# LanceZPF/loongx

Measured on AMD Instinct MI355X. Metric: edited images/s @512x512, 28-step Flux denoise, higher is better.
Workload: dtype bf16

## Files before the change

### include/lx.h

```cpp
#ifndef LX_H_
#define LX_H_
#include <stddef.h>
#include <stdint.h>
#ifdef __cplusplus
extern "C" {
#endif

#define LX_VERSION 404

typedef enum lx_status {
  LX_OK = 0,
  LX_ERR_INVALID = -1,
  LX_ERR_UNSUPPORTED = -2,
  LX_ERR_LAUNCH = -3,
  LX_ERR_NO_DEVICE = -4
} lx_status;

int lx_version(void);
const char* lx_last_error(void);
int lx_device_arch(char* name, size_t n);

enum {
  LX_EPI_STORE_BF16 = 0,
  LX_EPI_STORE_F32 = 1,
  LX_EPI_RESID_F32 = 2,
  LX_EPI_GELU = 0x100,
  LX_W_TILED = 0x200,
  LX_EPI_SPLIT_BF16 = 0x400,
  LX_EPI_STORE_FP8 = 3,
  LX_EPI_QKV = 0x1000,
  LX_OPERANDS_FP8 = 0x800,
  LX_OPERANDS_F16 = 0x2000
};

typedef struct lx_gemm_desc {
  const void* A;
  const void* W;
  const float* bias;
  void* C;
  const float* gate;
  const float* lora_t;
  const float* lora_up;
  int32_t M, N, K;
  int32_t lda, ldw, ldc;
  int32_t rows_per_batch, gate_ld;
  int32_t lora_r, lora_ldt, lora_mod_cols, lora_toff_max;
  int32_t epilogue;
  int32_t gelu_col_start;
  int32_t lora_nsplit;
  int32_t lora_split_stride;
  int32_t k_segs, a_lo_off;
  int32_t c_lo_off;
  float out_scale;
  union {
    const float* col_scale;
    int32_t* f16_ovf;
  };
  const float* qkv_norm_q;
  const float* qkv_norm_k;
  const float* qkv_rope;
  void* qkv_vt;
  void* qkv_k;
  int32_t qkv_d, qkv_vt_ld, qkv_vt_pos0;
  int32_t qkv_k_ld;
  void* qkv_q8;
  void* qkv_k8;
  void* qkv_vt8;
  int32_t qkv_ld8;
  float qkv_q_scale, qkv_k_scale, qkv_v_scale;
} lx_gemm_desc;

#define LX_GEMM_MAX_GROUP 4
int lx_gemm_bf16(const lx_gemm_desc* problems, int n, void* stream);
void lx_gemm_reload_env(void);

size_t lx_gemm_workspace_bytes(void);
int lx_gemm_bf16_ws(const lx_gemm_desc* problems, int n, void* workspace, size_t ws_bytes, void* stream);
int lx_gemm_workspace_status(void* workspace, void* stream);
enum { LX_GEMM_PLAN_NONE = 0, LX_GEMM_PLAN_8WAVE_256 = 1, LX_GEMM_PLAN_8WAVE_128 = 2, LX_GEMM_PLAN_MIXED = 3, LX_GEMM_PLAN_MIXED_2L = 4,
       LX_GEMM_PLAN_G4 = 5, LX_GEMM_PLAN_G4_SPLIT2 = 6, LX_GEMM_PLAN_G4_SPLIT3 = 7 };
int lx_gemm_last_plan(void);

int lx_lora_down(const void* X, int ldx, const void* Adown, float* T, int ldt, int M, int K, int R, int n_split,
                 int split_stride, void* stream);
int lx_lora_down_f16(const void* X, int ldx, const void* Adown, float* T, int ldt, int M, int K, int R, int n_split,
                     int split_stride, void* stream);
int lx_lora_down_terms(const void* const* X, const int* ldx, const void* const* Adown, int n_terms, float* T, int ldt, int M, int K, int R,
                       int slab_stride, void* stream);

int lx_linear_skinny(const float* X, int ldx, const void* W, int ldw, const float* bias, float* Y, int ldy,
                     int M, int N, int K, int act_in, int act_out, int accumulate, void* stream);

int lx_timestep_embed(const float* t, float* out, int B, int dim, void* stream);

int lx_rope_table(const float* ids, int L, int a0, int a1, int a2, double theta, float* cos_t, float* sin_t, void* stream);

int lx_ln_modulate(const float* X, int ldx, const float* shift, const float* scale, int mod_ld, void* Y, int ldy,
                   int M, int D, int rows_per_batch, float eps, void* stream);
typedef struct lx_ln_seg { int32_t row0, n_rows, rows_per_batch, _pad; const float* shift; const float* scale; } lx_ln_seg;
int lx_ln_modulate_segs(const float* X, int ldx, const lx_ln_seg* seg, int n_seg, int mod_ld, void* Y, int ldy, int D,
                        float eps, void* stream);
int lx_ln_modulate_f16_segs(const float* X, int ldx, const lx_ln_seg* seg, int n_seg, int mod_ld, void* Y, int ldy, int D,
                            float eps, int32_t* f16_ovf, void* stream);
int lx_ln_modulate_lora_segs(const float* X, int ldx, const lx_ln_seg* seg, int n_seg, int mod_ld, void* Y, int ldy, int D,
                             float eps, const void* Adown, int R, float* T, int ldt, int lora_row0, int lora_rows, void* stream);
int lx_ln_modulate_lora_f16_segs(const float* X, int ldx, const lx_ln_seg* seg, int n_seg, int mod_ld, void* Y, int ldy, int D,
                                 float eps, const void* Adown, int R, float* T, int ldt, int lora_row0, int lora_rows,
                                 int32_t* f16_ovf, void* stream);

int lx_qkv_prep(void* QKV, int ld, int q_col, int k_col, int v_col, int row0, int n_rows, int rows_per_batch,
                int H, const float* wq, const float* wk, float eps, const float* cos_tab, const float* sin_tab,
                void* VT, int vt_ld, int vt_pos0, void* stream);

typedef struct lx_qkv_seg {
  int32_t row0, rows_per_batch, vt_pos0, _pad;
  const float* wq; const float* wk; const float* cos_tab; const float* sin_tab;
} lx_qkv_seg;
int lx_qkv_prep_segs(void* QKV, int ld, int q_col, int k_col, int v_col, const lx_qkv_seg* seg, int n_seg, int n_batches,
                     int H, float eps, void* VT, int vt_ld, void* stream);
int lx_qkv_prep_f16in_segs(void* QKV, int ld, int q_col, int k_col, int v_col, const lx_qkv_seg* seg, int n_seg, int n_batches,
                           int H, float eps, void* VT, int vt_ld, void* stream);

typedef struct lx_attn_desc {
  const void* Q; const void* K; const void* VT; void* O;
  int32_t ldq, ldk, ldo, vt_ld;
  int32_t q_col, k_col, o_col;
  int32_t B, H;
  int32_t n_seg;
  int32_t seg_row0[3], seg_len[3], seg_vt0[3];
  float bias[3][3];
  float scale;
  int32_t n_qseg;
  int32_t flags;
  int32_t qseg_mask;
  int32_t* f16_ovf;
} lx_attn_desc;
enum { LX_ATTN_Q_LOG2 = 1, LX_ATTN_BOUNDED = 2, LX_ATTN_INVARIANT = 4, LX_ATTN_O_F16 = 8, LX_ATTN_PREFER_4WAVE = 16, LX_ATTN_P_EXP2 = 32 };
int lx_attn_fwd(const lx_attn_desc* d, void* stream);
enum { LX_ATTN_KERNEL_NONE = 0, LX_ATTN_KERNEL_8WAVE = 1, LX_ATTN_KERNEL_4WAVE = 2 };
int lx_attn_last_kernel(void);

enum { LX_ATTN_MASK_BOOL = 0, LX_ATTN_MASK_F32 = 1, LX_ATTN_MASK_BF16 = 2, LX_ATTN_MASK_F16 = 3 };
typedef struct lx_attn_mask_desc {
  const void* mask;
  int32_t dtype;
  int32_t dims[4];
  int32_t _pad;
  int64_t strides[4];
  void* workspace;
  size_t workspace_bytes;
} lx_attn_mask_desc;
int lx_attn_mask_workspace(const lx_attn_desc* d, const lx_attn_mask_desc* m, size_t* bytes);
int lx_attn_mask_prep(const lx_attn_desc* d, const lx_attn_mask_desc* m, void* stream);
int lx_attn_fwd_masked(const lx_attn_desc* d, const lx_attn_mask_desc* m, void* stream);

int lx_qkv_prep_fp8_segs(const void* QKV, int ld, int q_col, int k_col, int v_col, const lx_qkv_seg* seg, int n_seg,
                         int n_batches, int H, float eps, void* Q8, void* K8, int ld8, void* VT8, int vt8_ld,
                         float q_scale, float k_scale, float v_scale, void* stream);
int lx_qkv_prep_fp8_f16in_segs(const void* QKV, int ld, int q_col, int k_col, int v_col, const lx_qkv_seg* seg, int n_seg,
                               int n_batches, int H, float eps, void* Q8, void* K8, int ld8, void* VT8, int vt8_ld,
                               float q_scale, float k_scale, float v_scale, void* stream);
int lx_attn_fwd_fp8(const lx_attn_desc* d, float qk_descale, float v_descale, void* stream);

int lx_split_bf16(const float* src, int lds, void* dst, int ldd, int lo_off, int M, int K, void* stream);
int lx_ln_modulate_split_segs(const float* X, int ldx, const lx_ln_seg* seg, int n_seg, int mod_ld, void* Y, int ldy, int y_lo_off,
                              int D, float eps, void* stream);
int lx_qkv_prep_f32_segs(float* QKV, int ld, int q_col, int k_col, const lx_qkv_seg* seg, int n_seg, int n_batches, int H, float eps,
                         void* stream);
typedef struct lx_attn_f32_desc {
  const float* QKV; int32_t ld, q_col, k_col, v_col;
  void* O; int32_t ldo, o_col, o_lo_off;
  int32_t B, H, n_seg;
  int32_t seg_row0[3], seg_len[3];
  float bias[3][3];
  float scale;
} lx_attn_f32_desc;
int lx_attn_fwd_f32(const lx_attn_f32_desc* d, void* stream);

int lx_qkv_prep_split_segs(const float* QKV, int ld, int q_col, int k_col, int v_col, const lx_qkv_seg* seg, int n_seg, int n_batches, int H,
                           float eps, void* QK2, int ld2, int q2_col, int k2_col, int lo_off, void* VT2, int vt_ld, long long vt_lo_off,
                           void* stream);
int lx_attn_fwd_split(const lx_attn_desc* d, int qk_lo_off, long long vt_lo_off, int o_lo_off, void* stream);

int lx_ln_modulate_fp8_segs(const float* X, int ldx, const lx_ln_seg* seg, int n_seg, int mod_ld, void* Y, int ldy, void* Y8, int ldy8,
                            float y8_scale, int D, float eps, void* stream);
int lx_convert_fp8(const void* src, int src_is_bf16, int lds, void* dst, int ldd, float scale, int M, int K, void* stream);
int lx_lora_down_fp8(const void* X8, int ldx, float x_descale, const void* Adown, float* T, int ldt, int M, int K, int R, int n_split,
                     int split_stride, void* stream);

int lx_euler_step(float* x, const void* v, int v_is_bf16, float dsigma, size_t n, void* stream);
int lx_convert(void* dst, int dst_bf16, const void* src, int src_bf16, size_t n, void* stream);

int lx_s4_scan(const float* u, const double* lam, const double* w, const float* Dskip, float* y,
               int B, int H, int L, int N, void* stream);
int lx_s4_conv(const float* u, const float* Kker, const float* Dskip, float* y, int B, int H, int L, void* stream);
int lx_chanmix(const float* x, const float* W, const float* bias, const float* resid, const float* ln_g,
               const float* ln_b, float* y, int B, int Hin, int Hout, int L, int act, void* stream);
int lx_pyramid_pool(const float* x, float* y, int B, int C, int L, const int* sizes, int n_sizes, int ldy, int y_col0,
                    void* stream);
int lx_layernorm_relu(float* x, const float* g, const float* b, int M, int D, float eps, void* stream);
int lx_linear_f32(const float* X, int ldx, int x_trans, const float* W, int ldw, const float* bias, float* Y, int ldy,
                  int y_trans, int M, int N, int K, int accumulate, void* stream);

int lx_chan_gemm_f32(const float* X, long x_bstride, int ldx, const float* W, int ldw, const float* bias, float* Y, long y_bstride,
                     int ldy, int B, int N, int K, int L, int epilogue, float* part, void* stream);

size_t lx_duan_workspace_bytes(int B, int C, int L, int Hd);
int lx_duan_fwd(const float* x, const float* c, const float* gw1, const float* gb1, const float* gw2, const float* gb2,
                const float* mw1, const float* mb1, const float* mw2, const float* mb2, float* y,
                int B, int C, int L, int Hd, float eps, int keep_k, void* ws, size_t ws_bytes, void* stream);

size_t lx_groupnorm_workspace_bytes(int B, int P, int G);
int lx_groupnorm_silu(const void* x, int x_is_bf16, int B, int P, int C, int G, const float* gamma, const float* beta, float eps,
                      int silu, void* y, void* ws, size_t ws_bytes, void* stream);
int lx_im2col3x3(const void* x, int B, int H, int W, int C, int mode, void* out, int Kpad, void* stream);
int lx_softmax_rows(const float* S, int lds, float scale, void* P, int ldp, int M, int N, void* stream);

#ifdef __cplusplus
}
#endif
#endif
```

### loongx_amd/_lib.py

```python
from __future__ import annotations

import ctypes as C
import os

import torch

_HERE = os.path.dirname(os.path.abspath(__file__))
LIB_PATH = os.environ.get("LX_AMD_LIB", os.path.join(_HERE, "lib", "liblx_amd.so"))

LX_EPI_STORE_BF16, LX_EPI_STORE_F32, LX_EPI_RESID_F32, LX_EPI_GELU, LX_W_TILED, LX_EPI_SPLIT_BF16 = 0, 1, 2, 0x100, 0x200, 0x400
LX_EPI_STORE_FP8, LX_OPERANDS_FP8, LX_EPI_QKV, LX_OPERANDS_F16 = 3, 0x800, 0x1000, 0x2000
LX_GEMM_MAX_GROUP = 4
(LX_GEMM_PLAN_NONE, LX_GEMM_PLAN_8WAVE_256, LX_GEMM_PLAN_8WAVE_128, LX_GEMM_PLAN_MIXED, LX_GEMM_PLAN_MIXED_2L, LX_GEMM_PLAN_G4,
 LX_GEMM_PLAN_G4_SPLIT2, LX_GEMM_PLAN_G4_SPLIT3) = range(8)


class GemmDesc(C.Structure):
    _fields_ = [("A", C.c_void_p), ("W", C.c_void_p), ("bias", C.c_void_p), ("C", C.c_void_p),
                ("gate", C.c_void_p), ("lora_t", C.c_void_p), ("lora_up", C.c_void_p),
                ("M", C.c_int32), ("N", C.c_int32), ("K", C.c_int32),
                ("lda", C.c_int32), ("ldw", C.c_int32), ("ldc", C.c_int32),
                ("rows_per_batch", C.c_int32), ("gate_ld", C.c_int32),
                ("lora_r", C.c_int32), ("lora_ldt", C.c_int32), ("lora_mod_cols", C.c_int32),
                ("lora_toff_max", C.c_int32), ("epilogue", C.c_int32), ("gelu_col_start", C.c_int32),
                ("lora_nsplit", C.c_int32), ("lora_split_stride", C.c_int32),
                ("k_segs", C.c_int32), ("a_lo_off", C.c_int32), ("c_lo_off", C.c_int32), ("out_scale", C.c_float),
                ("col_scale", C.c_void_p),
                ("qkv_norm_q", C.c_void_p), ("qkv_norm_k", C.c_void_p), ("qkv_rope", C.c_void_p), ("qkv_vt", C.c_void_p),
                ("qkv_k", C.c_void_p),
                ("qkv_d", C.c_int32), ("qkv_vt_ld", C.c_int32), ("qkv_vt_pos0", C.c_int32), ("qkv_k_ld", C.c_int32),
                ("qkv_q8", C.c_void_p), ("qkv_k8", C.c_void_p), ("qkv_vt8", C.c_void_p),
                ("qkv_ld8", C.c_int32), ("qkv_q_scale", C.c_float), ("qkv_k_scale", C.c_float), ("qkv_v_scale", C.c_float)]


class AttnDesc(C.Structure):
    _fields_ = [("Q", C.c_void_p), ("K", C.c_void_p), ("VT", C.c_void_p), ("O", C.c_void_p),
                ("ldq", C.c_int32), ("ldk", C.c_int32), ("ldo", C.c_int32), ("vt_ld", C.c_int32),
                ("q_col", C.c_int32), ("k_col", C.c_int32), ("o_col", C.c_int32),
                ("B", C.c_int32), ("H", C.c_int32), ("n_seg", C.c_int32),
                ("seg_row0", C.c_int32 * 3), ("seg_len", C.c_int32 * 3), ("seg_vt0", C.c_int32 * 3),
                ("bias", (C.c_float * 3) * 3), ("scale", C.c_float), ("n_qseg", C.c_int32), ("flags", C.c_int32),
                ("qseg_mask", C.c_int32), ("f16_ovf", C.c_void_p)]


LX_ATTN_Q_LOG2, LX_ATTN_BOUNDED, LX_ATTN_INVARIANT, LX_ATTN_O_F16, LX_ATTN_PREFER_4WAVE, LX_ATTN_P_EXP2 = 1, 2, 4, 8, 16, 32
LX_ATTN_MASK_BOOL, LX_ATTN_MASK_F32, LX_ATTN_MASK_BF16, LX_ATTN_MASK_F16 = 0, 1, 2, 3


class AttnMaskDesc(C.Structure):
    _fields_ = [("mask", C.c_void_p), ("dtype", C.c_int32), ("dims", C.c_int32 * 4), ("_pad", C.c_int32),
                ("strides", C.c_int64 * 4), ("workspace", C.c_void_p), ("workspace_bytes", C.c_size_t)]


class AttnF32Desc(C.Structure):
    _fields_ = [("QKV", C.c_void_p), ("ld", C.c_int32), ("q_col", C.c_int32), ("k_col", C.c_int32), ("v_col", C.c_int32),
                ("O", C.c_void_p), ("ldo", C.c_int32), ("o_col", C.c_int32), ("o_lo_off", C.c_int32),
                ("B", C.c_int32), ("H", C.c_int32), ("n_seg", C.c_int32),
                ("seg_row0", C.c_int32 * 3), ("seg_len", C.c_int32 * 3),
                ("bias", (C.c_float * 3) * 3), ("scale", C.c_float)]


class LnSeg(C.Structure):
    _fields_ = [("row0", C.c_int32), ("n_rows", C.c_int32), ("rows_per_batch", C.c_int32), ("_pad", C.c_int32),
                ("shift", C.c_void_p), ("scale", C.c_void_p)]


class QkvSeg(C.Structure):
    _fields_ = [("row0", C.c_int32), ("rows_per_batch", C.c_int32), ("vt_pos0", C.c_int32), ("_pad", C.c_int32),
                ("wq", C.c_void_p), ("wk", C.c_void_p), ("cos_tab", C.c_void_p), ("sin_tab", C.c_void_p)]


_P, _I, _F, _Z = C.c_void_p, C.c_int, C.c_float, C.c_size_t
_SIGS = {
    "lx_version": (C.c_int, []),
    "lx_last_error": (C.c_char_p, []),
    "lx_device_arch": (C.c_int, [C.c_char_p, _Z]),
    "lx_gemm_bf16": (C.c_int, [C.POINTER(GemmDesc), _I, _P]),
    "lx_gemm_reload_env": (None, []),
    "lx_gemm_workspace_bytes": (_Z, []),
    "lx_gemm_bf16_ws": (C.c_int, [C.POINTER(GemmDesc), _I, _P, _Z, _P]),
    "lx_gemm_workspace_status": (C.c_int, [_P, _P]),
    "lx_gemm_last_plan": (C.c_int, []),
    "lx_lora_down": (C.c_int, [_P, _I, _P, _P, _I, _I, _I, _I, _I, _I, _P]),
    "lx_lora_down_f16": (C.c_int, [_P, _I, _P, _P, _I, _I, _I, _I, _I, _I, _P]),
    "lx_lora_down_terms": (C.c_int, [C.POINTER(C.c_void_p), C.POINTER(C.c_int), C.POINTER(C.c_void_p), _I, _P, _I, _I, _I, _I, _I, _P]),
    "lx_linear_skinny": (C.c_int, [_P, _I, _P, _I, _P, _P, _I, _I, _I, _I, _I, _I, _I, _P]),
    "lx_timestep_embed": (C.c_int, [_P, _P, _I, _I, _P]),
    "lx_rope_table": (C.c_int, [_P, _I, _I, _I, _I, C.c_double, _P, _P, _P]),
    "lx_ln_modulate": (C.c_int, [_P, _I, _P, _P, _I, _P, _I, _I, _I, _I, _F, _P]),
    "lx_ln_modulate_segs": (C.c_int, [_P, _I, C.POINTER(LnSeg), _I, _I, _P, _I, _I, _F, _P]),
    "lx_ln_modulate_f16_segs": (C.c_int, [_P, _I, C.POINTER(LnSeg), _I, _I, _P, _I, _I, _F, _P, _P]),
    "lx_ln_modulate_lora_segs": (C.c_int, [_P, _I, C.POINTER(LnSeg), _I, _I, _P, _I, _I, _F, _P, _I, _P, _I, _I, _I, _P]),
    "lx_ln_modulate_lora_f16_segs": (C.c_int, [_P, _I, C.POINTER(LnSeg), _I, _I, _P, _I, _I, _F, _P, _I, _P, _I, _I, _I, _P, _P]),
    "lx_qkv_prep_segs": (C.c_int, [_P, _I, _I, _I, _I, C.POINTER(QkvSeg), _I, _I, _I, _F, _P, _I, _P]),
    "lx_qkv_prep_f16in_segs": (C.c_int, [_P, _I, _I, _I, _I, C.POINTER(QkvSeg), _I, _I, _I, _F, _P, _I, _P]),
    "lx_qkv_prep": (C.c_int, [_P, _I, _I, _I, _I, _I, _I, _I, _I, _P, _P, _F, _P, _P, _P, _I, _I, _P]),
    "lx_attn_fwd": (C.c_int, [C.POINTER(AttnDesc), _P]),
    "lx_attn_last_kernel": (C.c_int, []),
    "lx_attn_mask_workspace": (C.c_int, [C.POINTER(AttnDesc), C.POINTER(AttnMaskDesc), C.POINTER(C.c_size_t)]),
    "lx_attn_mask_prep": (C.c_int, [C.POINTER(AttnDesc), C.POINTER(AttnMaskDesc), _P]),
    "lx_attn_fwd_masked": (C.c_int, [C.POINTER(AttnDesc), C.POINTER(AttnMaskDesc), _P]),
    "lx_qkv_prep_fp8_segs": (C.c_int, [_P, _I, _I, _I, _I, C.POINTER(QkvSeg), _I, _I, _I, _F, _P, _P, _I, _P, _I, _F, _F, _F, _P]),
    "lx_qkv_prep_fp8_f16in_segs": (C.c_int, [_P, _I, _I, _I, _I, C.POINTER(QkvSeg), _I, _I, _I, _F, _P, _P, _I, _P, _I, _F, _F, _F, _P]),
    "lx_attn_fwd_fp8": (C.c_int, [C.POINTER(AttnDesc), _F, _F, _P]),
    "lx_split_bf16": (C.c_int, [_P, _I, _P, _I, _I, _I, _I, _P]),
    "lx_ln_modulate_split_segs": (C.c_int, [_P, _I, C.POINTER(LnSeg), _I, _I, _P, _I, _I, _I, _F, _P]),
    "lx_qkv_prep_f32_segs": (C.c_int, [_P, _I, _I, _I, C.POINTER(QkvSeg), _I, _I, _I, _F, _P]),
    "lx_attn_fwd_f32": (C.c_int, [C.POINTER(AttnF32Desc), _P]),
    "lx_qkv_prep_split_segs": (C.c_int, [_P, _I, _I, _I, _I, C.POINTER(QkvSeg), _I, _I, _I, _F, _P, _I, _I, _I, _I, _P, _I, C.c_longlong, _P]),
    "lx_attn_fwd_split": (C.c_int, [C.POINTER(AttnDesc), _I, C.c_longlong, _I, _P]),
    "lx_groupnorm_workspace_bytes": (_Z, [_I, _I, _I]),
    "lx_groupnorm_silu": (C.c_int, [_P, _I, _I, _I, _I, _I, _P, _P, _F, _I, _P, _P, _Z, _P]),
    "lx_im2col3x3": (C.c_int, [_P, _I, _I, _I, _I, _I, _P, _I, _P]),
    "lx_softmax_rows": (C.c_int, [_P, _I, _F, _P, _I, _I, _I, _P]),
    "lx_ln_modulate_fp8_segs": (C.c_int, [_P, _I, C.POINTER(LnSeg), _I, _I, _P, _I, _P, _I, _F, _I, _F, _P]),
    "lx_convert_fp8": (C.c_int, [_P, _I, _I, _P, _I, _F, _I, _I, _P]),
    "lx_lora_down_fp8": (C.c_int, [_P, _I, _F, _P, _P, _I, _I, _I, _I, _I, _I, _P]),
    "lx_euler_step": (C.c_int, [_P, _P, _I, _F, _Z, _P]),
    "lx_convert": (C.c_int, [_P, _I, _P, _I, _Z, _P]),
    "lx_s4_scan": (C.c_int, [_P, _P, _P, _P, _P, _I, _I, _I, _I, _P]),
    "lx_s4_conv": (C.c_int, [_P, _P, _P, _P, _I, _I, _I, _P]),
    "lx_chanmix": (C.c_int, [_P, _P, _P, _P, _P, _P, _P, _I, _I, _I, _I, _I, _P]),
    "lx_pyramid_pool": (C.c_int, [_P, _P, _I, _I, _I, C.POINTER(C.c_int), _I, _I, _I, _P]),
    "lx_layernorm_relu": (C.c_int, [_P, _P, _P, _I, _I, _F, _P]),
    "lx_linear_f32": (C.c_int, [_P, _I, _I, _P, _I, _P, _P, _I, _I, _I, _I, _I, _I, _P]),
    "lx_chan_gemm_f32": (C.c_int, [_P, C.c_long, _I, _P, _I, _P, _P, C.c_long, _I, _I, _I, _I, _I, _I, _P, _P]),
    "lx_duan_workspace_bytes": (_Z, [_I, _I, _I, _I]),
    "lx_duan_fwd": (C.c_int, [_P] * 11 + [_I, _I, _I, _I, _F, _I, _P, _Z, _P]),
}

EXPORTS = tuple(_SIGS)


class LxError(RuntimeError):
    pass


def _load():
    if not os.path.exists(LIB_PATH):
        raise ImportError(f"liblx_amd.so not found at {LIB_PATH}: build it with `python -c 'import __graft_entry__ as g; "
                          f"g.build()'` or loongx_amd/csrc/build.sh -- there is no CPU/torch fallback for the hot path")
    lib = C.CDLL(LIB_PATH)
    for name, (res, args) in _SIGS.items():
        fn = getattr(lib, name)
        fn.restype, fn.argtypes = res, args
    return lib


lib = _load()


def check(status: int, what: str = "") -> None:
    if status != 0:
        raise LxError(f"{what or 'lx call'} failed ({status}): {lib.lx_last_error().decode()}")
```

### loongx_amd/csrc/gemm.hip

```cpp
#include "gemm8.h"


static double round_us(int bm, int K) { return bm == 256 ? 15.0 + 1.81 * (K / 64) : 10.5 + 1.06 * (K / 64); }

struct GemmEnv { int bm, g4, sk, g4_fault; };
static int env_int(const char* name, int dflt) {
  const char* s = getenv(name);
  return s ? atoi(s) : dflt;
}
static GemmEnv read_gemm_env() { return GemmEnv{env_int("LX_GEMM_BM", 0), env_int("LX_GEMM4", 1), env_int("LX_GEMM4_SK", 1), env_int("LX_GEMM4_FAULT", 0)}; }
static GemmEnv g_gemm_env = read_gemm_env();
static const GemmEnv& gemm_env() { return g_gemm_env; }
extern "C" void lx_gemm_reload_env(void) { g_gemm_env = read_gemm_env(); }

namespace {
constexpr size_t SK_FLAGS_OFF = (size_t)256 * SK_SLOT_FLOATS * sizeof(float);
constexpr size_t SK_WS_BYTES = SK_FLAGS_OFF + (256 + 64) * sizeof(int);
static_assert(SK_WS_BYTES % 256 == 0, "workspace size keeps the 256-byte alignment contract");
constexpr int SK_MIN_KT_ALL = 96;
constexpr int SK_MAX_ROUNDS = 16;

int device_cus() {
  static int n = -1;
  if (n < 0) {
    int dev = 0;
    hipDeviceProp_t pr;
    n = (hipGetDevice(&dev) == hipSuccess && hipGetDeviceProperties(&pr, dev) == hipSuccess) ? pr.multiProcessorCount : 0;
  }
  return n;
}
}

static long tiles_of(const lx_gemm_desc& p, int bm) { return (long)((p.M + bm - 1) / bm) * ((p.N + BN - 1) / BN); }

static lx_gemm_desc sub_rows(const lx_gemm_desc& p, int r0, int rows) {
  lx_gemm_desc q = p;
  q.A = (const uint16_t*)p.A + (size_t)r0 * p.lda;
  const int epi = p.epilogue & 0xff;
  q.C = epi == LX_EPI_STORE_BF16 ? (void*)((uint16_t*)p.C + (size_t)r0 * p.ldc) : (void*)((float*)p.C + (size_t)r0 * p.ldc);
  if (p.lora_t) q.lora_t = p.lora_t + (size_t)r0 * p.lora_ldt;
  if (p.qkv_k) q.qkv_k = (uint16_t*)p.qkv_k + (size_t)r0 * p.qkv_k_ld;
  if (p.qkv_q8) {
    q.qkv_q8 = (uint8_t*)p.qkv_q8 + (size_t)r0 * p.qkv_ld8;
    q.qkv_k8 = (uint8_t*)p.qkv_k8 + (size_t)r0 * p.qkv_ld8;
  }
  q.M = rows;
  return q;
}

static int launch_plan(const GemmArgs& a, int bm, hipStream_t s, int variant = LX_GV_BF16) {
  if (a.n == 0) return LX_OK;
  if (variant == LX_GV_SPLIT) lx_gemm8_launch_split(bm, a, s);
  else if (variant == LX_GV_F16) lx_gemm8_launch_f16(bm, a, s);
  else if (variant == LX_GV_FP8) lx_gemm8_launch_fp8(bm, a, s);
  else lx_gemm8_launch_bf16(bm, a, s);
  LX_LAUNCH_CHECK("lx_gemm_bf16");
  return LX_OK;
}

void lx_gemm8_launch_bf16(int bm, const GemmArgs& a, hipStream_t s) {
  const int t = a.tile_start[a.n];
  if (bm == 256) hipLaunchKernelGGL((lx_gemm_kernel<256, false>), dim3(t), dim3(NTHREADS), 0, s, a);
  else hipLaunchKernelGGL((lx_gemm_kernel<128, false>), dim3(t), dim3(NTHREADS), 0, s, a);
}
void lx_gemm8_mixed_launch_bf16(const GemmArgs& big, const GemmArgs& tail, int n_big_pad, hipStream_t s) {
  hipLaunchKernelGGL(lx_gemm_mixed_kernel<false>, dim3(n_big_pad + tail.tile_start[tail.n]), dim3(NTHREADS), 0, s, big, tail, n_big_pad);
}

static void plan_add(GemmArgs& a, const lx_gemm_desc& p, int m_base, int bm) {
  a.p[a.n] = p;
  a.m_base[a.n] = m_base;
  a.tile_start[a.n + 1] = a.tile_start[a.n] + (int)tiles_of(p, bm);
  ++a.n;
  for (int i = a.n + 1; i <= MAX_SUB; ++i) a.tile_start[i] = a.tile_start[a.n];
}

static thread_local int lx_gemm_last = LX_GEMM_PLAN_NONE;
extern "C" int lx_gemm_last_plan(void) { return lx_gemm_last; }
static int planned(int rc, int plan) {
  if (rc == LX_OK) lx_gemm_last = plan;
  return rc;
}

extern "C" size_t lx_gemm_workspace_bytes(void) { return SK_WS_BYTES; }

extern "C" int lx_gemm_workspace_status(void* workspace, void* stream) {
  LX_CHECK_ARG(workspace, "lx_gemm_workspace_status: NULL workspace");
  int* err = (int*)((char*)workspace + SK_FLAGS_OFF) + 256;
  int v = 0;
  hipStream_t s = (hipStream_t)stream;
  if (hipMemcpyAsync(&v, err, sizeof(int), hipMemcpyDeviceToHost, s) != hipSuccess || hipStreamSynchronize(s) != hipSuccess) {
    lx_set_error("lx_gemm_workspace_status: reading the error word failed: %s", hipGetErrorString(hipGetLastError()));
    return LX_ERR_LAUNCH;
  }
  if (v == 0) return LX_OK;
  (void)hipMemsetAsync((char*)workspace + SK_FLAGS_OFF, 0, (256 + 64) * sizeof(int), s);
  (void)hipStreamSynchronize(s);
  lx_set_error("lx_gemm_bf16_ws: a split-K pair workgroup timed out waiting for its partner (CUs held by other work?); the results "
               "of that launch are invalid. Re-run with the workspace omitted (lx_gemm_bf16) or LX_GEMM4_SK=0");
  return LX_ERR_LAUNCH;
}

extern "C" int lx_gemm_bf16(const lx_gemm_desc* problems, int n, void* stream) { return lx_gemm_bf16_ws(problems, n, nullptr, 0, stream); }

extern "C" int lx_gemm_bf16_ws(const lx_gemm_desc* problems, int n, void* workspace, size_t ws_bytes, void* stream) {
  LX_CHECK_ARG(problems && n >= 1 && n <= LX_GEMM_MAX_GROUP, "lx_gemm_bf16: n=%d out of range [1,%d]", n, LX_GEMM_MAX_GROUP);
  long t256 = 0, t128 = 0;
  int kmax = 0;
  bool split = false, fp8 = false, f16 = false, qkv = false;
  for (int i = 0; i < n; ++i) fp8 = fp8 || (problems[i].epilogue & LX_OPERANDS_FP8) != 0;
  for (int i = 0; i < n; ++i) f16 = f16 || (problems[i].epilogue & LX_OPERANDS_F16) != 0;
  for (int i = 0; i < n; ++i) {
    const lx_gemm_desc& p = problems[i];
    if (f16) {
      LX_CHECK_ARG((p.epilogue & LX_OPERANDS_F16) != 0 && !(p.epilogue & LX_OPERANDS_FP8) && p.k_segs <= 1 && !(p.epilogue & LX_EPI_SPLIT_BF16),
                   "lx_gemm_bf16[%d]: LX_OPERANDS_F16 must be set on every problem of a launch and excludes the e4m3 and split-bf16 modes", i);
      if (p.f16_ovf) LX_CHECK_ARG(((uintptr_t)p.f16_ovf & 3) == 0, "lx_gemm_bf16[%d]: f16_ovf must be 4-byte aligned", i);
    }
    if (fp8) {
      LX_CHECK_ARG((p.epilogue & LX_OPERANDS_FP8) != 0 && p.k_segs <= 1 && !(p.epilogue & LX_EPI_SPLIT_BF16), "lx_gemm_bf16[%d]: LX_OPERANDS_FP8 must be set on every problem of a launch and excludes the split-bf16 mode", i);
      LX_CHECK_ARG(p.K % 128 == 0 && p.lda % 16 == 0 && p.ldw % 16 == 0, "lx_gemm_bf16[%d]: fp8 operands need K %% 128 == 0 and lda / ldw %% 16 == 0 (K=%d)", i, p.K);
      if (p.col_scale) LX_CHECK_ARG(((uintptr_t)p.col_scale & 15) == 0, "lx_gemm_bf16[%d]: col_scale must be 16-byte aligned", i);
      if (p.lora_t) LX_CHECK_ARG(p.lora_r <= 4 && p.lora_nsplit <= 4, "lx_gemm_bf16[%d]: the fp8 path applies LoRA in the tile prologue only (rank <= 4, <= 4 slabs)", i);
      if ((p.epilogue & 0xff) == LX_EPI_STORE_FP8) LX_CHECK_ARG(p.out_scale > 0.f && p.ldc % 8 == 0, "lx_gemm_bf16[%d]: LX_EPI_STORE_FP8 needs out_scale > 0 and ldc %% 8 == 0", i);
    }
    LX_CHECK_ARG(p.k_segs >= 0 && p.k_segs <= 3, "lx_gemm_bf16[%d]: k_segs=%d must be 0..3", i, p.k_segs);
    const int segs = p.k_segs > 1 ? p.k_segs : 1;
    if (segs > 1 || (p.epilogue & LX_EPI_SPLIT_BF16)) split = true;
    if (segs > 1) LX_CHECK_ARG(p.a_lo_off >= p.K && p.a_lo_off % 8 == 0 && p.lda >= p.a_lo_off + p.K, "lx_gemm_bf16[%d]: a_lo_off=%d needs K <= a_lo_off, a_lo_off + K <= lda, multiple of 8", i, p.a_lo_off);
    if (segs == 3) LX_CHECK_ARG(p.ldw >= 2 * p.K, "lx_gemm_bf16[%d]: k_segs = 3 reads W as [N, 2K] = [W_hi | W_lo]: ldw=%d < 2K", i, p.ldw);
    if (p.epilogue & LX_EPI_SPLIT_BF16) LX_CHECK_ARG((p.epilogue & 0xff) == LX_EPI_STORE_BF16 && p.c_lo_off >= p.N && p.c_lo_off % 8 == 0 && p.ldc >= p.c_lo_off + p.N,
                                                     "lx_gemm_bf16[%d]: LX_EPI_SPLIT_BF16 needs a bf16 store and N <= c_lo_off, c_lo_off + N <= ldc, multiple of 8", i);
    LX_CHECK_ARG(p.A && p.W && p.C, "lx_gemm_bf16[%d]: NULL operand", i);
    LX_CHECK_ARG(p.M > 0 && p.N > 0 && p.K > 0, "lx_gemm_bf16[%d]: bad shape M=%d N=%d K=%d", i, p.M, p.N, p.K);
    LX_CHECK_ARG(p.K % BK == 0, "lx_gemm_bf16[%d]: K=%d must be a multiple of %d", i, p.K, BK);
    LX_CHECK_ARG(p.N % 8 == 0, "lx_gemm_bf16[%d]: N=%d must be a multiple of 8", i, p.N);
    LX_CHECK_ARG(p.lda % 8 == 0 && p.ldw % 8 == 0 && p.lda >= p.K && p.ldw >= p.K, "lx_gemm_bf16[%d]: lda/ldw must be >= K and multiples of 8", i);
    LX_CHECK_ARG(((uintptr_t)p.A & 15) == 0 && ((uintptr_t)p.W & 15) == 0 && ((uintptr_t)p.C & 15) == 0, "lx_gemm_bf16[%d]: operands must be 16-byte aligned", i);
    LX_CHECK_ARG(p.ldc % 8 == 0 && p.ldc >= p.N, "lx_gemm_bf16[%d]: ldc=%d must be >= N and a multiple of 8", i, p.ldc);
    const int epi = p.epilogue & 0xff;
    LX_CHECK_ARG(epi >= LX_EPI_STORE_BF16 && (epi <= LX_EPI_RESID_F32 || (fp8 && epi == LX_EPI_STORE_FP8)), "lx_gemm_bf16[%d]: unknown epilogue %d", i, p.epilogue);
    LX_CHECK_ARG(p.rows_per_batch > 0, "lx_gemm_bf16[%d]: rows_per_batch must be > 0", i);
    if (p.epilogue & LX_W_TILED) LX_CHECK_ARG(p.N % BN == 0 && p.ldw == (segs == 3 ? 2 * p.K : p.K), "lx_gemm_bf16[%d]: LX_W_TILED needs N %% 256 == 0 and ldw == K (2K with k_segs = 3)", i);
    if (p.gate) LX_CHECK_ARG(p.gate_ld >= p.N && p.gate_ld % 4 == 0, "lx_gemm_bf16[%d]: gate_ld=%d", i, p.gate_ld);
    if (p.lora_t) {
      LX_CHECK_ARG(p.lora_up && p.lora_r >= 1 && p.lora_r <= 16, "lx_gemm_bf16[%d]: LoRA needs lora_up and 1 <= r <= 16", i);
      LX_CHECK_ARG(p.lora_mod_cols <= 0 || p.lora_mod_cols % BN == 0, "lx_gemm_bf16[%d]: lora_mod_cols must be a multiple of %d", i, BN);
    }
    if (p.epilogue & LX_EPI_QKV) {
      LX_CHECK_ARG(!fp8 && segs == 1 && !(p.epilogue & LX_EPI_SPLIT_BF16) && epi == LX_EPI_STORE_BF16, "lx_gemm_bf16[%d]: LX_EPI_QKV goes with plain bf16 operands and LX_EPI_STORE_BF16", i);
      LX_CHECK_ARG(p.qkv_d > 0 && p.qkv_d % BN == 0 && (p.N >= 3 * p.qkv_d || p.N % BN == 0), "lx_gemm_bf16[%d]: LX_EPI_QKV needs qkv_d %% 256 == 0 and whole projection tiles (qkv_d=%d N=%d)", i, p.qkv_d, p.N);
      LX_CHECK_ARG(p.rows_per_batch % 32 == 0 && p.M % 32 == 0, "lx_gemm_bf16[%d]: LX_EPI_QKV needs rows_per_batch %% 32 == 0 and M %% 32 == 0 (%d, %d)", i, p.rows_per_batch, p.M);
      const bool q8 = p.qkv_q8 != nullptr;
      LX_CHECK_ARG(p.qkv_norm_q && p.qkv_norm_k && (p.qkv_vt || q8) && p.qkv_rope && ((uintptr_t)p.qkv_norm_q & 15) == 0 && ((uintptr_t)p.qkv_norm_k & 15) == 0 && ((uintptr_t)p.qkv_vt & 15) == 0 &&
                   ((uintptr_t)p.qkv_rope & 15) == 0, "lx_gemm_bf16[%d]: LX_EPI_QKV needs 16-byte aligned qkv_norm_q / qkv_norm_k / qkv_rope / qkv_vt", i);
      if (q8) {
        LX_CHECK_ARG(p.qkv_k8 && p.qkv_vt8 && (((uintptr_t)p.qkv_q8 | (uintptr_t)p.qkv_k8 | (uintptr_t)p.qkv_vt8) & 15) == 0 && p.qkv_ld8 % 16 == 0 && p.qkv_ld8 >= p.qkv_d,
                     "lx_gemm_bf16[%d]: LX_EPI_QKV e4m3 outputs need 16-byte aligned qkv_q8 / qkv_k8 / qkv_vt8 and qkv_ld8 %% 16 == 0, >= qkv_d", i);
        LX_CHECK_ARG(p.qkv_q_scale > 0.f && p.qkv_k_scale > 0.f && p.qkv_v_scale > 0.f && !p.qkv_k, "lx_gemm_bf16[%d]: LX_EPI_QKV e4m3 outputs need positive scales and no separate bf16 key image", i);
      }
      LX_CHECK_ARG(p.qkv_vt_ld > 0 && p.qkv_vt_ld % 64 == 0 && p.qkv_vt_pos0 >= 0 && p.qkv_vt_pos0 % 64 == 0 && p.qkv_vt_pos0 + p.rows_per_batch <= p.qkv_vt_ld,
                   "lx_gemm_bf16[%d]: qkv_vt_ld / qkv_vt_pos0 must be multiples of 64 with the stream inside a V^T row", i);
      if (p.qkv_k) LX_CHECK_ARG(((uintptr_t)p.qkv_k & 15) == 0 && p.qkv_k_ld % 8 == 0 && p.qkv_k_ld >= p.qkv_d, "lx_gemm_bf16[%d]: qkv_k must be 16-byte aligned with qkv_k_ld %% 8 == 0, >= qkv_d", i);
      qkv = true;
    }
    if (p.bias) LX_CHECK_ARG(((uintptr_t)p.bias & 15) == 0, "lx_gemm_bf16[%d]: bias must be 16-byte aligned", i);
    t256 += tiles_of(p, 256);
    t128 += tiles_of(p, 128);
    kmax = p.K * segs > kmax ? p.K * segs : kmax;
  }
  hipStream_t s = (hipStream_t)stream;
  if (fp8) {
    const int ncu = device_cus() > 0 ? device_cus() : 256;
    const double ca = (double)((t256 + ncu - 1) / ncu) * round_us(256, kmax / 4), cb = (double)((t128 + ncu - 1) / ncu) * round_us(128, kmax / 4);
    const int bm = gemm_env().bm ? gemm_env().bm : (cb < ca ? 128 : 256);
    GemmArgs all;
    all.n = 0;
    all.tile_start[0] = 0;
    for (int i = 1; i <= MAX_SUB; ++i) all.tile_start[i] = 0;
    for (int i = 0; i < n; ++i) plan_add(all, problems[i], 0, bm);
    return planned(launch_plan(all, bm, s, LX_GV_FP8), bm == 256 ? LX_GEMM_PLAN_8WAVE_256 : LX_GEMM_PLAN_8WAVE_128);
  }
  const int NCU = device_cus() > 0 ? device_cus() : 256;
  const GemmEnv& env = gemm_env();
  const int forced = env.bm;
  if (env.g4 && forced == 0 && (workspace || env.g4 == 2)) {
    bool ok = true;
    for (int i = 0; i < n; ++i) {
      const lx_gemm_desc& p = problems[i];
      ok = ok && (p.epilogue & 0xff) <= LX_EPI_RESID_F32 && p.K / BK >= 2 && !((p.epilogue & LX_EPI_QKV) && p.qkv_q8);
      if (p.lora_t)
        ok = ok && p.lora_r <= 8 && p.lora_r % 2 == 0 && p.lora_nsplit >= 1 && p.lora_nsplit <= 4 && p.lora_ldt % 2 == 0 && p.lora_split_stride % 2 == 0 &&
             ((((uintptr_t)p.lora_t) | ((uintptr_t)p.lora_up)) & 7) == 0;
    }
    const long rounds = (t256 + NCU - 1) / NCU;
    bool fills = env.g4 == 2 || (t256 >= NCU && (rounds * NCU - t256 <= NCU / 4 || rounds >= 8));
    bool uniform_k4 = true;
    for (int i = 1; i < n; ++i) uniform_k4 = uniform_k4 && problems[i].K == problems[0].K;
    const long tail = t256 % NCU, full = t256 - tail;
    for (int i = 1; i < n; ++i) uniform_k4 = uniform_k4 && problems[i].k_segs == problems[0].k_segs;
    const int kt_all = kmax / BK;
    const bool can_split = env.sk && workspace && ws_bytes >= SK_WS_BYTES && ((uintptr_t)workspace & 255) == 0 && uniform_k4 && kt_all >= 16 &&
                           tail > 0 && tail * 2 <= 256 && tail * 2 <= NCU && rounds <= SK_MAX_ROUNDS;
    bool split_all = can_split && full == 0 && kt_all >= SK_MIN_KT_ALL;
    const int tail_div = !qkv && kt_all >= 96 ? 2 : 3;
    bool split_tail = can_split && full > 0 && tail * tail_div <= NCU;
    int np = 2;
    if (!split && env.sk != 2 && kt_all >= 24 && tail * 3 <= 256 && tail * 3 <= NCU && (split_all || split_tail) && (kt_all >= 96 || tail * 6 <= NCU)) np = 3;
    if (split) {
      const double r4 = 8.9 + 1.31 * kt_all;
      const bool sk_tail = can_split && tail > 0;
      const double c4 = (double)(full / NCU) * r4 + (tail == 0 ? 0.0 : sk_tail ? 8.9 + 1.31 * (kt_all - kt_all / 2) + 6.0 : r4);
      const double c8a = (double)((t256 + NCU - 1) / NCU) * (5.8 + 1.55 * kt_all), c8b = (double)((t128 + NCU - 1) / NCU) * (10.5 + 1.06 * kt_all);
      fills = env.g4 == 2 || c4 < (c8a < c8b ? c8a : c8b);
      split_all = fills && sk_tail && full == 0;
      split_tail = fills && sk_tail && full > 0;
      if (!fills) split_all = split_tail = false;
    }
    if (ok && (fills || split_all || split_tail)) {
      GemmArgs all;
      all.n = 0;
      all.tile_start[0] = 0;
      for (int i = 1; i <= MAX_SUB; ++i) all.tile_start[i] = 0;
      for (int i = 0; i < n; ++i) plan_add(all, problems[i], 0, 256);
      float* slots = nullptr;
      int *flags = nullptr, *err = nullptr;
      unsigned grid = (unsigned)t256;
      int sk_full = (int)t256, sk_parts = 1;
      if (split_all || split_tail) {
        slots = (float*)workspace;
        flags = (int*)((char*)workspace + SK_FLAGS_OFF);
        err = flags + 256;
        grid = (unsigned)(full + np * tail);
        sk_full = (int)full;
        sk_parts = env.g4_fault ? 3 : 2;
      }
      if (split) lx_gemm4_launch_split(all, grid, sk_full, sk_parts, slots, flags, err, s);
      else if (f16) lx_gemm4_launch_f16(all, grid, sk_full, sk_parts, slots, flags, err, s, np);
      else lx_gemm4_launch_bf16(all, grid, sk_full, sk_parts, slots, flags, err, s, np);
      LX_LAUNCH_CHECK("lx_gemm_bf16");
      return planned(LX_OK, !(split_all || split_tail) ? LX_GEMM_PLAN_G4 : np == 3 ? LX_GEMM_PLAN_G4_SPLIT3 : LX_GEMM_PLAN_G4_SPLIT2);
    }
  }
  if (split) {
    const double ca = (double)((t256 + NCU - 1) / NCU) * round_us(256, kmax), cb = (double)((t128 + NCU - 1) / NCU) * round_us(128, kmax);
    const int bm = forced ? forced : (cb < ca ? 128 : 256);
    GemmArgs all;
    all.n = 0;
    all.tile_start[0] = 0;
    for (int i = 1; i <= MAX_SUB; ++i) all.tile_start[i] = 0;
    for (int i = 0; i < n; ++i) plan_add(all, problems[i], 0, bm);
    return planned(launch_plan(all, bm, s, LX_GV_SPLIT), bm == 256 ? LX_GEMM_PLAN_8WAVE_256 : LX_GEMM_PLAN_8WAVE_128);
  }
  if (workspace) LX_CHECK_ARG(ws_bytes >= SK_WS_BYTES && ((uintptr_t)workspace & 255) == 0, "lx_gemm_bf16_ws: workspace needs %zu bytes (lx_gemm_workspace_bytes()), 256-byte aligned", SK_WS_BYTES);
  const int variant = f16 ? LX_GV_F16 : LX_GV_BF16;
  const double c_a = (double)((t256 + NCU - 1) / NCU) * round_us(256, kmax);
  const double c_b = (double)((t128 + NCU - 1) / NCU) * round_us(128, kmax);
  GemmArgs big, tail;
  big.n = tail.n = 0;
  big.tile_start[0] = tail.tile_start[0] = 0;
  for (int i = 1; i <= MAX_SUB; ++i) big.tile_start[i] = tail.tile_start[i] = 0;
  double c_c = 1e30;
  const long full = (t256 / NCU) * NCU;
  if (forced == 0 && full > 0 && t256 > full) {
    long remain = t256;
    int keep_rows[LX_GEMM_MAX_GROUP];
    for (int i = 0; i < n; ++i) keep_rows[i] = problems[i].M;
    for (int i = n - 1; i >= 0 && remain > full; --i) {
      const int tn = (problems[i].N + BN - 1) / BN;
      while (remain > full && keep_rows[i] > 0) {
        const int last_rows = keep_rows[i] % 256 ? keep_rows[i] % 256 : 256;
        keep_rows[i] -= last_rows;
        remain -= tn;
      }
    }
    long tail_tiles = 0;
    for (int i = 0; i < n; ++i) {
      if (keep_rows[i] > 0) plan_add(big, sub_rows(problems[i], 0, keep_rows[i]), 0, 256);
      if (keep_rows[i] < problems[i].M) {
        const lx_gemm_desc q = sub_rows(problems[i], keep_rows[i], problems[i].M - keep_rows[i]);
        plan_add(tail, q, keep_rows[i], 128);
        tail_tiles += tiles_of(q, 128);
      }
    }
    c_c = (double)((remain + NCU - 1) / NCU) * round_us(256, kmax) + (double)((tail_tiles + NCU - 1) / NCU) * round_us(128, kmax) + 2.0;
  }
  int choice = forced == 256 ? 0 : forced == 128 ? 1 : (c_c < c_a && c_c < c_b) ? 2 : (c_b < c_a ? 1 : 0);
  if (choice == 2) {
    if (big.n > 0 && tail.n > 0) {
      const int n_big = big.tile_start[big.n], n_big_pad = (n_big + 7) & ~7;
      if (f16) lx_gemm8_mixed_launch_f16(big, tail, n_big_pad, s);
      else lx_gemm8_mixed_launch_bf16(big, tail, n_big_pad, s);
      LX_LAUNCH_CHECK("lx_gemm_bf16");
      return planned(LX_OK, LX_GEMM_PLAN_MIXED);
    }
    const int rc = launch_plan(big, 256, s, variant);
    if (rc != LX_OK) return rc;
    return planned(launch_plan(tail, 128, s, variant), LX_GEMM_PLAN_MIXED_2L);
  }
  GemmArgs all;
  all.n = 0;
  all.tile_start[0] = 0;
  for (int i = 1; i <= MAX_SUB; ++i) all.tile_start[i] = 0;
  for (int i = 0; i < n; ++i) plan_add(all, problems[i], 0, choice == 0 ? 256 : 128);
  return planned(launch_plan(all, choice == 0 ? 256 : 128, s, variant), choice == 0 ? LX_GEMM_PLAN_8WAVE_256 : LX_GEMM_PLAN_8WAVE_128);
}
```

### loongx_amd/csrc/gemm4.h

```cpp
#pragma once
#include "gemm_common.h"

namespace {

constexpr int G4_STAGE = 256 * BK * 2 + BN * BK * 2;
constexpr int G4_LDS = 2 * G4_STAGE;
constexpr int G4_PLD = 132;
static_assert(G4_LDS <= 160 * 1024 && 4 * 2 * 16 * G4_PLD * 4 <= G4_LDS, "LDS budget / epilogue patches");

#ifdef LX_G4_PROBE
__device__ unsigned long long lx_g4_probe_buf[8192 * 8];
#define G4_STAMP(k) if (threadIdx.x == 0 && blockIdx.x < 8192) { asm volatile("s_waitcnt lgkmcnt(0)" ::: "memory"); lx_g4_probe_buf[blockIdx.x * 8 + (k)] = __builtin_amdgcn_s_memtime(); }
#else
#define G4_STAMP(k)
#endif


template <bool SPLIT, bool F16 = false, int NP = 2>
__global__ __launch_bounds__(G4_THREADS) void lx_gemm4_kernel(const GemmArgs args, const int sk_full, const int sk_parts, float* __restrict__ sk_slots,
                                                              int* __restrict__ sk_flags, int* __restrict__ sk_err) {
#if defined(__HIP_DEVICE_COMPILE__)
  __shared__ __attribute__((aligned(1024))) char smem[G4_LDS];
  constexpr int BM = 256, A_BYTES = BM * BK * 2;
  const int pid = blockIdx.x;
  G4_STAMP(0)
  const int total = args.tile_start[MAX_SUB];
  int lid, part = 0;
  if (pid < sk_full) {
    const int q = sk_full >> 3, r = sk_full & 7;
    const int xcd = pid & 7, inx = pid >> 3;
    lid = (xcd < r ? xcd * (q + 1) : r * (q + 1) + (xcd - r) * q) + inx;
  } else {
    const int r = pid - sk_full;
    lid = sk_full + r / NP;
    part = r % NP;
  }
  (void)total;
  const bool split_tile = pid >= sk_full && sk_parts >= 2;
  const int g = tile_group(args, lid);
  lx_gemm_desc P = args.p[g];
  int tm, tn;
  tile_coords<BM>(P, lid - args.tile_start[g], tm, tn);
  const int tid = threadIdx.x, lane = tid & 63;
  const int wave = __builtin_amdgcn_readfirstlane(tid >> 6);
  const int wm = wave >> 1, wn = wave & 1, l15 = lane & 15, lq = lane >> 4;
  int m0 = tm * BM, n0 = tn * BN;
  int M = P.M, N = P.N;
  const int K = P.K;
  const bool w_tiled = (P.epilogue & LX_W_TILED) != 0;
  const int nk1 = K / BK;
  const int nkt = SPLIT ? nk1 * max(P.k_segs, 1) : nk1;
  const int kt_begin = !split_tile ? 0 : NP == 2 ? (part ? nkt >> 1 : 0) : (part * nkt) / NP;
  const int kt_end = !split_tile ? nkt : NP == 2 ? (part ? nkt : nkt >> 1) : ((part + 1) * nkt) / NP;

  uint32_t aoff[8], woff[8];
  {
    const int rsub = lane >> 3, pslot = lane & 7;
#pragma unroll
    for (int j = 0; j < 8; ++j) {
      const int row = (j * 4 + wave) * 8 + rsub;
      const int lslot = pslot ^ ((row >> 1) & 7);
      aoff[j] = (uint32_t)((min(m0 + row, M - 1) - m0) * P.lda + lslot * 8) * 2u;
      woff[j] = w_tiled ? (uint32_t)((j * 4 + wave) * 512 + lane * 8) * 2u : (uint32_t)((min(n0 + row, N - 1) - n0) * P.ldw + lslot * 8) * 2u;
    }
  }
  const __bf16* a_org = (const __bf16*)P.A + (size_t)m0 * P.lda;
  const int kw_tiles = SPLIT && P.k_segs == 3 ? 2 * nk1 : nk1;
  const __bf16* w_org = w_tiled ? (const __bf16*)P.W + ((size_t)tn * kw_tiles) * (BN * BK) : (const __bf16*)P.W + (size_t)n0 * P.ldw;
  const lx_rsrc_t rs_a = lx_make_rsrc(a_org), rs_w = lx_make_rsrc(w_org);
  const int w_kstride_b = (w_tiled ? BN * BK : BK) * 2;
  const int a_lo_b = SPLIT ? P.a_lo_off * 2 : 0;
  auto a_soff = [&](int t) -> int {
    if constexpr (!SPLIT) return t * (BK * 2);
    else {
      const int seg = t >= 2 * nk1 ? 2 : (t >= nk1 ? 1 : 0);
      return (t - seg * nk1) * (BK * 2) + (seg == 1 ? a_lo_b : 0);
    }
  };
  auto w_soff = [&](int t) -> int {
    if constexpr (!SPLIT) return t * w_kstride_b;
    else {
      const int seg = t >= 2 * nk1 ? 2 : (t >= nk1 ? 1 : 0);
      return (t - seg * nk1 + (seg == 2 ? nk1 : 0)) * w_kstride_b;
    }
  };
  auto piece = [&](int p_, int a_so, int w_so, int stage) {
    if (p_ < 8) lx_buf_to_lds(rs_a, (lptr_t)(smem + stage * G4_STAGE + (p_ * 4 + wave) * 1024), aoff[p_], a_so);
    else lx_buf_to_lds(rs_w, (lptr_t)(smem + stage * G4_STAGE + A_BYTES + ((p_ - 8) * 4 + wave) * 1024), woff[p_ - 8], w_so);
  };
  int a_ad[2], w_ad[2];
  {
    const int ar = wm * 128 + l15, wr = wn * 128 + l15;
#pragma unroll
    for (int ks = 0; ks < 2; ++ks) {
      a_ad[ks] = ar * 128 + (((ks * 4 + lq) ^ ((ar >> 1) & 7)) * 16);
      w_ad[ks] = A_BYTES + wr * 128 + (((ks * 4 + lq) ^ ((wr >> 1) & 7)) * 16);
    }
  }
  f32x4 acc[8][8];
#pragma unroll
  for (int i = 0; i < 8; ++i)
#pragma unroll
    for (int j = 0; j < 8; ++j) acc[i][j] = f32x4{0.f, 0.f, 0.f, 0.f};
  bf16x8 af[2][8], wf[2][8];
  auto rd = [&](int stage, int ks, int idx) {
    const char* base = smem + stage * G4_STAGE;
    if (idx < 8) wf[ks][idx] = *(const bf16x8*)(base + w_ad[ks] + idx * 2048);
    else af[ks][idx - 8] = *(const bf16x8*)(base + a_ad[ks] + (idx - 8) * 2048);
  };
  auto mm = [&](int ks, int n_) {
    const int j = n_ >> 3, i = n_ & 7;
    if constexpr (F16) asm volatile("v_mfma_f32_16x16x32_f16 %0, %1, %2, %0" : "+a"(acc[i][j]) : "v"(wf[ks][j]), "v"(af[ks][i]));
    else asm volatile("v_mfma_f32_16x16x32_bf16 %0, %1, %2, %0" : "+a"(acc[i][j]) : "v"(wf[ks][j]), "v"(af[ks][i]));
  };
#define G4_SB() __builtin_amdgcn_sched_barrier(0)
  const bool has_lora = P.lora_t != nullptr && kt_begin == 0;
  u32x2 lu[8], lt[8][4];
  if (has_lora) {
    const int R = P.lora_r, nsplit = P.lora_nsplit;
    const int toff = R * min(n0 / max(P.lora_mod_cols, 1), P.lora_toff_max);
    const int rk = min(2 * lq, R - 2);
#pragma unroll
    for (int j = 0; j < 8; ++j) lu[j] = *(const u32x2*)(P.lora_up + (size_t)min(n0 + wn * 128 + j * 16 + l15, N - 1) * R + rk);
#pragma unroll
    for (int i = 0; i < 8; ++i) {
      const float* tp = P.lora_t + (size_t)min(m0 + wm * 128 + i * 16 + l15, M - 1) * P.lora_ldt + toff + rk;
#pragma unroll
      for (int q = 0; q < 4; ++q) lt[i][q] = *(const u32x2*)(tp + (size_t)min(q, nsplit - 1) * P.lora_split_stride);
    }
  }
  {
    const int t1 = min(kt_begin + 1, kt_end - 1);
    const int a0 = a_soff(kt_begin), w0 = w_soff(kt_begin), a1 = a_soff(t1), w1 = w_soff(t1);
#pragma unroll
    for (int p_ = 0; p_ < 16; ++p_) piece(p_, a0, w0, 0);
#pragma unroll
    for (int p_ = 0; p_ < 16; ++p_) piece(p_, a1, w1, 1);
  }
  asm volatile("s_waitcnt vmcnt(16)" ::: "memory");
  __builtin_amdgcn_s_barrier();
  G4_SB();
  G4_STAMP(1)
#pragma unroll
  for (int x = 0; x < 16; ++x) rd(0, 0, x);
  if (has_lora) {
    const int R = P.lora_r, nsplit = P.lora_nsplit;
    const bool live = 2 * lq < R;
    auto frag_u = [&](u32x2 v) {
      const float a = live ? __uint_as_float(v[0]) : 0.f, b = live ? __uint_as_float(v[1]) : 0.f;
      const uint16_t ah = f32_to_bf16(a), bh = f32_to_bf16(b);
      const uint16_t al = f32_to_bf16(a - bf16_to_f32(ah)), bl = f32_to_bf16(b - bf16_to_f32(bh));
      const u32x4 w = {(uint32_t)ah * 0x10001u, (uint32_t)al * 0x10001u, (uint32_t)bh * 0x10001u, (uint32_t)bl * 0x10001u};
      return __builtin_bit_cast(bf16x8, w);
    };
    auto frag_t = [&](float a, float b) {
      a = live ? a : 0.f; b = live ? b : 0.f;
      const uint16_t ah = f32_to_bf16(a), bh = f32_to_bf16(b);
      const uint32_t pa = (uint32_t)ah | ((uint32_t)f32_to_bf16(a - bf16_to_f32(ah)) << 16);
      const uint32_t pb = (uint32_t)bh | ((uint32_t)f32_to_bf16(b - bf16_to_f32(bh)) << 16);
      const u32x4 w = {pa, pa, pb, pb};
      return __builtin_bit_cast(bf16x8, w);
    };
    bf16x8 uf[8], tf[8];
#pragma unroll
    for (int j = 0; j < 8; ++j) uf[j] = frag_u(lu[j]);
#pragma unroll
    for (int i = 0; i < 8; ++i) {
      float a = __uint_as_float(lt[i][0][0]), b = __uint_as_float(lt[i][0][1]);
#pragma unroll
      for (int q = 1; q < 4; ++q)
        if (q < nsplit) { a += __uint_as_float(lt[i][q][0]); b += __uint_as_float(lt[i][q][1]); }
      tf[i] = frag_t(a, b);
    }
#pragma unroll
    for (int j = 0; j < 8; ++j)
#pragma unroll
      for (int i = 0; i < 8; ++i) acc[i][j] = __builtin_amdgcn_mfma_f32_16x16x32_bf16(uf[j], tf[i], acc[i][j], 0, 0, 0);
    asm volatile("s_nop 15\n s_nop 7" ::: "memory");
  }
  asm volatile("s_waitcnt lgkmcnt(0)" ::: "memory");
  G4_STAMP(2)
  int c = 0;
  for (int kt = kt_begin; kt < kt_end; ++kt) {
    const int n = c ^ 1;
    const int kt2 = min(kt + 2, kt_end - 1);
    const int a_so2 = a_soff(kt2), w_so2 = w_soff(kt2);
#pragma unroll
    for (int m = 0; m < 64; ++m) {
      if (m == 16) {
        G4_SB();
        asm volatile("s_waitcnt lgkmcnt(0)" ::: "memory");
        __builtin_amdgcn_s_barrier();
        G4_SB();
      }
      mm(0, m); G4_SB();
      if (m < 16) { rd(c, 1, m); G4_SB(); }
      if (m >= 16 && (m - 16) % 6 == 0) { piece((m - 16) / 6, a_so2, w_so2, c); G4_SB(); }
    }
#pragma unroll
    for (int m = 0; m < 64; ++m) {
      if (m == 43) {
        G4_SB();
        asm volatile("s_waitcnt vmcnt(16)" ::: "memory");
        __builtin_amdgcn_s_barrier();
        G4_SB();
      }
      mm(1, m); G4_SB();
      if (m < 40 && m % 5 == 0) { piece(8 + m / 5, a_so2, w_so2, c); G4_SB(); }
      if (m >= 43 && m < 59) { rd(n, 0, m - 43); G4_SB(); }
    }
    asm volatile("s_waitcnt lgkmcnt(0)" ::: "memory");
    c = n;
  }
#undef G4_SB
  G4_STAMP(3)
  asm volatile("s_nop 15\n s_nop 7\n s_waitcnt vmcnt(0)" ::: "memory");
  __syncthreads();
  G4_STAMP(4)

  const float* partner = nullptr;
  const float* partner2 = nullptr;
  float* my_slot = nullptr;
  if (split_tile) {
    my_slot = sk_slots + (size_t)(pid - sk_full) * SK_SLOT_FLOATS;
    if constexpr (NP == 2) {
      partner = sk_slots + (size_t)((pid - sk_full) ^ 1) * SK_SLOT_FLOATS;
    } else {
      const int gb = (pid - sk_full) - part;
      partner = sk_slots + (size_t)(gb + (part + 1) % NP) * SK_SLOT_FLOATS;
      partner2 = sk_slots + (size_t)(gb + (part + 2) % NP) * SK_SLOT_FLOATS;
    }
  }
  auto pld4 = [&](size_t off_floats, const float* from) {
    const u32x4 v = __builtin_amdgcn_raw_buffer_load_b128(lx_make_rsrc(from), (int)(off_floats * 4), 0, PAIR_AUX_SC1);
    return f32x4{__uint_as_float(v[0]), __uint_as_float(v[1]), __uint_as_float(v[2]), __uint_as_float(v[3])};
  };
  const int lm0 = wm * 128, ln0 = wn * 128;
  auto exchange = [&]() {
    asm volatile("s_waitcnt vmcnt(0)" ::: "memory");
    __syncthreads();
    __builtin_amdgcn_fence(__ATOMIC_RELEASE, "workgroup");
    if (tid == 0) {
      const int me = pid - sk_full, other = NP == 2 ? (me ^ 1) : (me - part + (part + 1) % NP), other2 = me - part + (part + 2) % NP;
      bool ok = __hip_atomic_load(sk_err, __ATOMIC_RELAXED, __HIP_MEMORY_SCOPE_AGENT) == 0;
      if (ok) {
        if (!(sk_parts == 3 && part == 1))
          __hip_atomic_store(sk_flags + me, NP - 1, __ATOMIC_RELAXED, __HIP_MEMORY_SCOPE_AGENT);
        int spins = 0;
        while (__hip_atomic_load(sk_flags + other, __ATOMIC_RELAXED, __HIP_MEMORY_SCOPE_AGENT) == 0) {
          __builtin_amdgcn_s_sleep(1);
          if (++spins > (1 << 20)) { ok = false; break; }
        }
        if constexpr (NP == 3) {
          while (ok && __hip_atomic_load(sk_flags + other2, __ATOMIC_RELAXED, __HIP_MEMORY_SCOPE_AGENT) == 0) {
            __builtin_amdgcn_s_sleep(1);
            if (++spins > (1 << 20)) { ok = false; break; }
          }
        }
        if (ok) {
          if constexpr (NP == 2) __hip_atomic_store(sk_flags + other, 0, __ATOMIC_RELAXED, __HIP_MEMORY_SCOPE_AGENT);
          else {
            __hip_atomic_fetch_add(sk_flags + other, -1, __ATOMIC_RELAXED, __HIP_MEMORY_SCOPE_AGENT);
            __hip_atomic_fetch_add(sk_flags + other2, -1, __ATOMIC_RELAXED, __HIP_MEMORY_SCOPE_AGENT);
          }
        } else __hip_atomic_store(sk_err, 1, __ATOMIC_RELAXED, __HIP_MEMORY_SCOPE_AGENT);
      }
    }
    __syncthreads();
    G4_STAMP(6)
    __builtin_amdgcn_fence(__ATOMIC_ACQUIRE, "workgroup");
  };

  const int epi = P.epilogue & 0xff;
  const bool do_gelu = (P.epilogue & LX_EPI_GELU) != 0;
  const int mw0 = m0 + wm * 128, nw0 = n0 + wn * 128;
  float* patch = (float*)smem + wave * (2 * 16 * G4_PLD);
  const bool bf16_out = epi == LX_EPI_STORE_BF16;
  const int c8 = (lane & 15) * 8, c4 = (lane & 31) * 4;
  const int ncol = nw0 + (bf16_out ? c8 : c4);
  const bool col_ok = ncol < N;
  f32x4 bias0 = {0.f, 0.f, 0.f, 0.f}, bias1 = {0.f, 0.f, 0.f, 0.f};
  if (P.bias && col_ok) {
    bias0 = *(const f32x4*)(P.bias + ncol);
    if (bf16_out) bias1 = *(const f32x4*)(P.bias + ncol + 4);
  }
  asm volatile("s_waitcnt vmcnt(0)" : "+v"(bias0), "+v"(bias1)::"memory");
  const bool gelu0 = do_gelu && ncol >= P.gelu_col_start;
  const int m_base = args.m_base[g];
  static_assert(!(F16 && SPLIT), "fp16 operands exclude the split-bf16 mode");
  float f16_mx = 0.f;
  const bool qkv_tile = (P.epilogue & LX_EPI_QKV) != 0 && n0 < 3 * P.qkv_d;
  const int qkind = qkv_tile ? n0 / P.qkv_d : -1;
  f32x4 nw0v = {1.f, 1.f, 1.f, 1.f}, nw1v = {1.f, 1.f, 1.f, 1.f};
  if (qkv_tile && qkind != 1) {
    const float* nwp = (qkind == 2 ? P.qkv_norm_q : P.qkv_norm_k) + c8;
    nw0v = *(const f32x4*)nwp; nw1v = *(const f32x4*)(nwp + 4);
    asm volatile("s_waitcnt vmcnt(0)" : "+v"(nw0v), "+v"(nw1v)::"memory");
  }
  auto put = [&](auto ic_) {
    constexpr int i = decltype(ic_)::value;
    float* pt = patch + (i & 1) * (16 * G4_PLD);
    asm volatile("" : "+a"(acc[i][0]), "+a"(acc[i][1]), "+a"(acc[i][2]), "+a"(acc[i][3]), "+a"(acc[i][4]), "+a"(acc[i][5]), "+a"(acc[i][6]), "+a"(acc[i][7]));
#pragma unroll
    for (int j = 0; j < 8; ++j) *(f32x4*)(pt + l15 * G4_PLD + j * 16 + 4 * lq) = acc[i][j];
  };
  auto park = [&](auto ic_, auto nx_) {
    constexpr int i = decltype(ic_)::value, nx = decltype(nx_)::value;
    const float* pt = patch + (i & 1) * (16 * G4_PLD);
    __builtin_amdgcn_wave_barrier();
    if constexpr (nx >= 0) { if (mw0 + nx * 16 < M) put(std::integral_constant<int, nx>{}); }
    __builtin_amdgcn_sched_barrier(0);
    if (mw0 + i * 16 >= M) return;
    const lx_rsrc_t rs_slot = lx_make_rsrc(my_slot);
#pragma unroll
    for (int t = 0; t < 8; ++t) {
      const int row = t * 2 + (lane >> 5);
      const f32x4 v = *(const f32x4*)(pt + row * G4_PLD + c4);
      __builtin_amdgcn_raw_buffer_store_b128(u32x4{__float_as_uint(v[0]), __float_as_uint(v[1]), __float_as_uint(v[2]), __float_as_uint(v[3])}, rs_slot,
                                             (int)(((size_t)(wm * 128 + i * 16 + row) * 256 + wn * 128 + c4) * 4), 0, PAIR_AUX_SC1);
    }
  };
  auto block = [&](auto ic_, auto nx_) {
    constexpr int i = decltype(ic_)::value, nx = decltype(nx_)::value;
    const int mb = mw0 + i * 16;
    if (mb >= M) return;
    const float* pt = patch + (i & 1) * (16 * G4_PLD);
    f32x4 res[8], gat[8];
    if (epi == LX_EPI_RESID_F32 && !qkv_tile) {
      const int rpb = P.rows_per_batch;
#pragma unroll
      for (int t = 0; t < 8; ++t) {
        const int m = mb + t * 2 + (lane >> 5);
        if (m < M && col_ok) {
          res[t] = *(const f32x4*)((const float*)P.C + (size_t)m * P.ldc + ncol);
          if (P.gate) gat[t] = *(const f32x4*)(P.gate + (size_t)((m_base + m) / rpb) * P.gate_ld + ncol);
        }
      }
    }
    __builtin_amdgcn_wave_barrier();
    if constexpr (nx >= 0) { if (mw0 + nx * 16 < M) put(std::integral_constant<int, nx>{}); }
    __builtin_amdgcn_sched_barrier(0);
    if (partner) {
      f32x4 pa[4][2], pb[4][2];
#pragma unroll
      for (int t = 0; t < 4; ++t) {
        const size_t po = (size_t)(lm0 + i * 16 + t * 4 + (lane >> 4)) * 256 + ln0 + c8;
        pa[t][0] = pld4(po, partner); pa[t][1] = pld4(po + 4, partner);
        if constexpr (NP == 3) { pb[t][0] = pld4(po, partner2); pb[t][1] = pld4(po + 4, partner2); }
      }
      float* pw = patch + (i & 1) * (16 * G4_PLD);
#pragma unroll
      for (int t = 0; t < 4; ++t) {
        float* q_ = pw + (t * 4 + (lane >> 4)) * G4_PLD + c8;
        f32x4 v0 = *(const f32x4*)q_, v1 = *(const f32x4*)(q_ + 4);
#pragma unroll
        for (int c_ = 0; c_ < 4; ++c_) { v0[c_] += pa[t][0][c_]; v1[c_] += pa[t][1][c_]; }
        if constexpr (NP == 3) {
#pragma unroll
          for (int c_ = 0; c_ < 4; ++c_) { v0[c_] += pb[t][0][c_]; v1[c_] += pb[t][1][c_]; }
        }
        *(f32x4*)q_ = v0; *(f32x4*)(q_ + 4) = v1;
      }
      __builtin_amdgcn_wave_barrier();
    }
    if (qkv_tile) {
      const int D = P.qkv_d, L = P.rows_per_batch, H = D >> 7;
      const int gm = m_base + mb, b = gm / L, p0 = gm - b * L;
      const int h = (nw0 - qkind * D) >> 7;
      if (qkind == 1) {
        const int gk = lane & 1;
        float e[4][8];
#pragma unroll
        for (int t = 0; t < 4; ++t)
#pragma unroll
          for (int k = 0; k < 8; ++k) {
            const int rk = qkv_vt_interleave(gk * 8 + k), dk = t * 32 + (lane >> 1);
            e[t][k] = pt[rk * G4_PLD + dk];
          }
#pragma unroll
        for (int t = 0; t < 4; ++t) {
          const int d = t * 32 + (lane >> 1);
          const float bd = P.bias ? P.bias[nw0 + d] : 0.f;
          u32x4 o = {pack_bf16x2(e[t][0] + bd, e[t][1] + bd), pack_bf16x2(e[t][2] + bd, e[t][3] + bd), pack_bf16x2(e[t][4] + bd, e[t][5] + bd),
                     pack_bf16x2(e[t][6] + bd, e[t][7] + bd)};
          *(u32x4*)((uint16_t*)P.qkv_vt + ((size_t)(b * H + h) * 128 + d) * P.qkv_vt_ld + P.qkv_vt_pos0 + p0 + gk * 8) = o;
        }
      } else {
        uint16_t* const out = (qkind == 0 && P.qkv_k) ? (uint16_t*)P.qkv_k : (uint16_t*)P.C;
        const int out_ld = (qkind == 0 && P.qkv_k) ? P.qkv_k_ld : P.ldc;
        f32x4 cs[4][2], pv[4][2];
#pragma unroll
        for (int t = 0; t < 4; ++t) {
          const float* rp = P.qkv_rope + (size_t)(p0 + t * 4 + (lane >> 4)) * 128 + c8;
          cs[t][0] = *(const f32x4*)rp; cs[t][1] = *(const f32x4*)(rp + 4);
        }
#pragma unroll
        for (int t = 0; t < 4; ++t) {
          const int row = t * 4 + (lane >> 4);
          pv[t][0] = *(const f32x4*)(pt + row * G4_PLD + c8); pv[t][1] = *(const f32x4*)(pt + row * G4_PLD + c8 + 4);
        }
        float yy[4][8];
#pragma unroll
        for (int t = 0; t < 4; ++t) {
          f32x4 v0 = pv[t][0], v1 = pv[t][1];
          float ss = 0.f;
#pragma unroll
          for (int c_ = 0; c_ < 4; ++c_) { v0[c_] += bias0[c_]; v1[c_] += bias1[c_]; ss = __builtin_fmaf(v0[c_], v0[c_], ss); ss = __builtin_fmaf(v1[c_], v1[c_], ss); }
#ifdef LX_G4_ROW16_SHFL
          ss += __shfl_xor(ss, 1, 64); ss += __shfl_xor(ss, 2, 64); ss += __shfl_xor(ss, 4, 64); ss += __shfl_xor(ss, 8, 64);
#else
          ss = row16_sum(ss);
#endif
          const float r = rsqrtf(ss * (1.0f / 128.0f) + 1e-6f);
          float x[8];
          float (&y)[8] = yy[t];
#pragma unroll
          for (int c_ = 0; c_ < 4; ++c_) { x[c_] = v0[c_] * r * nw0v[c_]; x[4 + c_] = v1[c_] * r * nw1v[c_]; }
#pragma unroll
          for (int q = 0; q < 4; ++q) {
            const float co = q < 2 ? cs[t][0][2 * q] : cs[t][1][2 * q - 4], si = q < 2 ? cs[t][0][2 * q + 1] : cs[t][1][2 * q - 3];
            y[2 * q] = x[2 * q] * co - x[2 * q + 1] * si;
            y[2 * q + 1] = x[2 * q + 1] * co + x[2 * q] * si;
          }
        }
#pragma unroll
        for (int t = 0; t < 4; ++t) {
          const int m = mb + t * 4 + (lane >> 4);
          const float (&y)[8] = yy[t];
          u32x4 o = {pack_bf16x2(y[0], y[1]), pack_bf16x2(y[2], y[3]), pack_bf16x2(y[4], y[5]), pack_bf16x2(y[6], y[7])};
          if (m < M) *(u32x4*)(out + (size_t)m * out_ld + ncol) = o;
        }
      }
      return;
    }
    if (bf16_out) {
      f32x4 pv[4][2];
#pragma unroll
      for (int t = 0; t < 4; ++t) {
        const int row = t * 4 + (lane >> 4);
        pv[t][0] = *(const f32x4*)(pt + row * G4_PLD + c8); pv[t][1] = *(const f32x4*)(pt + row * G4_PLD + c8 + 4);
      }
#pragma unroll
      for (int t = 0; t < 4; ++t) {
        const int row = t * 4 + (lane >> 4), m = mb + row;
        f32x4 v0 = pv[t][0], v1 = pv[t][1];
        if (m < M && col_ok) {
#pragma unroll
          for (int c_ = 0; c_ < 4; ++c_) { v0[c_] += bias0[c_]; v1[c_] += bias1[c_]; }
          if (gelu0) { v0 = gelu_tanh4(v0); v1 = gelu_tanh4(v1); }
          u32x4 o = {pack_op16x2<F16>(v0[0], v0[1], f16_mx), pack_op16x2<F16>(v0[2], v0[3], f16_mx), pack_op16x2<F16>(v1[0], v1[1], f16_mx),
                     pack_op16x2<F16>(v1[2], v1[3], f16_mx)};
          *(u32x4*)((uint16_t*)P.C + (size_t)m * P.ldc + ncol) = o;
          if constexpr (SPLIT) {
            if (P.epilogue & LX_EPI_SPLIT_BF16) {
              float r[8];
#pragma unroll
              for (int c_ = 0; c_ < 4; ++c_) {
                r[c_] = v0[c_] - bf16_to_f32(f32_to_bf16(v0[c_]));
                r[4 + c_] = v1[c_] - bf16_to_f32(f32_to_bf16(v1[c_]));
              }
              u32x4 ol = {pack_bf16x2(r[0], r[1]), pack_bf16x2(r[2], r[3]), pack_bf16x2(r[4], r[5]), pack_bf16x2(r[6], r[7])};
              *(u32x4*)((uint16_t*)P.C + (size_t)m * P.ldc + ncol + P.c_lo_off) = ol;
            }
          }
        }
      }
    } else {
      f32x4 pv[8];
#pragma unroll
      for (int t = 0; t < 8; ++t) pv[t] = *(const f32x4*)(pt + (t * 2 + (lane >> 5)) * G4_PLD + c4);
      if (epi == LX_EPI_RESID_F32) {
        asm volatile("s_waitcnt vmcnt(0)" ::: "memory");
#pragma unroll
        for (int t = 0; t < 8; ++t) asm volatile("" : "+v"(res[t]), "+v"(gat[t]));
      }
#pragma unroll
      for (int t = 0; t < 8; ++t) {
        const int row = t * 2 + (lane >> 5), m = mb + row;
        f32x4 v = pv[t];
        if (m < M && col_ok) {
#pragma unroll
          for (int c_ = 0; c_ < 4; ++c_) v[c_] += bias0[c_];
          if (gelu0) v = gelu_tanh4(v);
          if (epi == LX_EPI_RESID_F32) {
            f32x4 o = res[t];
            if (P.gate) {
#pragma unroll
              for (int c_ = 0; c_ < 4; ++c_) o[c_] = __builtin_fmaf(gat[t][c_], v[c_], o[c_]);
            } else {
#pragma unroll
              for (int c_ = 0; c_ < 4; ++c_) o[c_] += v[c_];
            }
            v = o;
          }
          *(f32x4*)((float*)P.C + (size_t)m * P.ldc + ncol) = v;
        }
      }
    }
  };
#define G4_B(I, NX) block(std::integral_constant<int, I>{}, std::integral_constant<int, NX>{})
#define G4_K(I, NX) park(std::integral_constant<int, I>{}, std::integral_constant<int, NX>{})
  if (!split_tile) {
    if (mw0 < M) put(std::integral_constant<int, 0>{});
    G4_B(0, 1); G4_B(1, 2); G4_B(2, 3); G4_B(3, 4); G4_B(4, 5); G4_B(5, 6); G4_B(6, 7); G4_B(7, -1);
  } else if constexpr (NP == 2) {
    if (part == 0) {
      if (mw0 + 64 < M) put(std::integral_constant<int, 4>{});
      G4_K(4, 5); G4_K(5, 6); G4_K(6, 7); G4_K(7, 0);
      exchange();
      G4_B(0, 1); G4_B(1, 2); G4_B(2, 3); G4_B(3, -1);
    } else {
      if (mw0 < M) put(std::integral_constant<int, 0>{});
      G4_K(0, 1); G4_K(1, 2); G4_K(2, 3); G4_K(3, 4);
      exchange();
      G4_B(4, 5); G4_B(5, 6); G4_B(6, 7); G4_B(7, -1);
    }
  } else {
    if (part == 0) {
      if (mw0 + 48 < M) put(std::integral_constant<int, 3>{});
      G4_K(3, 4); G4_K(4, 5); G4_K(5, 6); G4_K(6, 7); G4_K(7, 0);
      exchange();
      G4_B(0, 1); G4_B(1, 2); G4_B(2, -1);
    } else if (part == 1) {
      if (mw0 < M) put(std::integral_constant<int, 0>{});
      G4_K(0, 1); G4_K(1, 2); G4_K(2, 7); G4_K(7, 6); G4_K(6, 3);
      exchange();
      G4_B(3, 4); G4_B(4, 5); G4_B(5, -1);
    } else {
      if (mw0 < M) put(std::integral_constant<int, 0>{});
      G4_K(0, 1); G4_K(1, 2); G4_K(2, 3); G4_K(3, 4); G4_K(4, 5); G4_K(5, 6);
      exchange();
      G4_B(6, 7); G4_B(7, -1);
    }
  }
#undef G4_B
#undef G4_K
  if constexpr (F16) { if (bf16_out && !qkv_tile) report_f16_overflow(f16_mx, P.f16_ovf); }
  asm volatile("s_waitcnt vmcnt(0)" ::: "memory");
  G4_STAMP(5)
#endif
}


}
```

### loongx_amd/csrc/gemm_common.h

```cpp
#pragma once
#include "common.h"
#include <type_traits>

constexpr int MAX_SUB = 2 * LX_GEMM_MAX_GROUP;

struct GemmArgs {
  lx_gemm_desc p[MAX_SUB];
  int tile_start[MAX_SUB + 1];
  int m_base[MAX_SUB];
  int n;
};
static_assert(2 * sizeof(GemmArgs) + 16 <= 4096, "lx_gemm_mixed_kernel takes two plans by value: the kernarg segment is 4 KiB");

namespace {

constexpr int BN = 256;
constexpr int BK = 64;
constexpr int NTHREADS = 512;
#ifndef LX_GROUP_M
#define LX_GROUP_M 4
#endif
constexpr int GROUP_M = LX_GROUP_M;

typedef const __attribute__((address_space(1))) void* gptr_t;
typedef __attribute__((address_space(3))) void* lptr_t;

constexpr int PAIR_AUX_SC1 = 16;

__device__ __forceinline__ float clamp_e4m3(float x) { return fminf(fmaxf(x, -448.f), 448.f); }
__device__ __forceinline__ uint32_t pack_fp8x4(float a, float b, float c, float d) {
  int w = __builtin_amdgcn_cvt_pk_fp8_f32(clamp_e4m3(a), clamp_e4m3(b), 0, false);
  w = __builtin_amdgcn_cvt_pk_fp8_f32(clamp_e4m3(c), clamp_e4m3(d), w, true);
  return (uint32_t)w;
}

__device__ __forceinline__ int qkv_vt_interleave(int key) {
  return (key & ~15) | (((key >> 2) & 1) << 3) | (((key >> 3) & 1) << 2) | (key & 3);
}

__device__ __forceinline__ int tile_group(const GemmArgs& args, const int lid) {
  int g = 0;
#pragma unroll
  for (int i = 1; i < MAX_SUB; ++i)
    if (lid >= args.tile_start[i]) g = i;
  return g;
}

template <int BM>
__device__ __forceinline__ void tile_coords(const lx_gemm_desc& P, const int local, int& tm, int& tn) {
  const int tiles_m = (P.M + BM - 1) / BM;
  const int tiles_n = (P.N + BN - 1) / BN;
  const int gs = GROUP_M * tiles_n;
  const int gi = local / gs, in_g = local - gi * gs;
  const int first_m = gi * GROUP_M;
  const int gm = min(tiles_m - first_m, GROUP_M);
  tm = first_m + in_g % gm;
  tn = in_g / gm;
}

constexpr int G4_THREADS = 256;
constexpr int SK_SLOT_FLOATS = 256 * 256;

}

enum { LX_GV_BF16 = 0, LX_GV_F16 = 1, LX_GV_SPLIT = 2, LX_GV_FP8 = 3 };

void lx_gemm8_launch_bf16(int bm, const GemmArgs& a, hipStream_t s);
void lx_gemm8_launch_f16(int bm, const GemmArgs& a, hipStream_t s);
void lx_gemm8_launch_split(int bm, const GemmArgs& a, hipStream_t s);
void lx_gemm8_launch_fp8(int bm, const GemmArgs& a, hipStream_t s);
void lx_gemm8_mixed_launch_bf16(const GemmArgs& big, const GemmArgs& tail, int n_big_pad, hipStream_t s);
void lx_gemm8_mixed_launch_f16(const GemmArgs& big, const GemmArgs& tail, int n_big_pad, hipStream_t s);
void lx_gemm4_launch_bf16(const GemmArgs& a, unsigned grid, int sk_full, int sk_parts, float* slots, int* flags, int* err, hipStream_t s, int np = 2);
void lx_gemm4_launch_f16(const GemmArgs& a, unsigned grid, int sk_full, int sk_parts, float* slots, int* flags, int* err, hipStream_t s, int np = 2);
void lx_gemm4_launch_split(const GemmArgs& a, unsigned grid, int sk_full, int sk_parts, float* slots, int* flags, int* err, hipStream_t s);
```

### loongx_amd/flux/engine.py

```python
from __future__ import annotations

import math
import os
from typing import Dict, List, Optional, Sequence

import torch

from .. import ops
from ..ops import LX_EPI_GELU, LX_EPI_RESID_F32, LX_EPI_STORE_BF16, LX_EPI_STORE_F32
from .weights import FluxConfig, PackedWeights

NEG_INF = float("-inf")


def _pad64(n: int) -> int:
    return (n + 63) // 64 * 64


def mask_argument(attention_mask) -> None:
    if not isinstance(attention_mask, torch.Tensor) or attention_mask.dim() < 2:
        raise NotImplementedError("attention_mask must be a tensor of rank 2..4 over the concatenated [text | image | condition] sequence")


def refuse_masked_modes(model_config: Optional[Dict], precise_default: bool) -> None:
    mc = model_config or {}
    if bool(mc.get("precise", precise_default)):
        raise NotImplementedError("attention_mask is not supported in precise mode")
    if mc.get("attn_fp8", False):
        raise NotImplementedError("attention_mask is not supported in attn_fp8 mode")


class DiTEngine:
    def __init__(self, weights: PackedWeights, device="cuda"):
        self.w = weights
        self.cfg: FluxConfig = weights.cfg
        self.device = torch.device(device)
        if self.cfg.attention_head_dim != 128:
            raise ValueError("the gfx950 attention kernel is specialised for head_dim 128 (FLUX.1)")
        self.shape = None
        self.cond_ready = False
        self.sched = None
        self.graphs: Dict = {}
        self._warmed = set()
        import os
        self.use_graph = os.environ.get("LX_GRAPH", "1") != "0"
        self.qkv_epilogue = True
        self.ln_lora = True
        self.model_config: Dict = {}
        self.c_factor: Optional[float] = None
        self.attn_mask: Optional[torch.Tensor] = None
        self.cond_mask: Optional[torch.Tensor] = None
        self._mask_ws: Optional[torch.Tensor] = None
        self.pair_plan = os.environ.get("LX_PAIR_PLAN", "1") != "0"
        self.lora_scale = 1.0
        self.precise_default = False
        self.attn_nomax = False
        self.precise = False
        self.gemm_fp8 = False
        self.w8: Dict[str, torch.Tensor] = {}
        self.operands_default = "bf16"
        self.f16 = False
        self.w16: Dict[str, torch.Tensor] = {}
        self.f16_ovf: Optional[torch.Tensor] = None
        self._gemm_ws: Optional[torch.Tensor] = None
        self.cond_cache_enabled = os.environ.get("LX_COND_CACHE", "1") != "0"
        self.cond_cache = False
        self.cond_cached = False
        self.cond_skip = False
        self.KC = self.VTC = None

    def setup(self, B: int, T: int, N: int, C: int) -> None:
        if self.shape == (B, T, N, C):
            return
        cfg, dev = self.cfg, self.device
        D, H = cfg.inner_dim, cfg.num_attention_heads
        self.B, self.T, self.N, self.C = B, T, N, C
        self.r_txt, self.r_img, self.r_cond = 0, B * T, B * (T + N)
        self.M = B * (T + N + C)
        M = self.M
        f32, bf16 = torch.float32, torch.bfloat16
        self.X = torch.zeros(M, D, dtype=f32, device=dev)
        self.XN = torch.zeros(M, D, dtype=bf16, device=dev)
        self.Y = torch.zeros(M, 7 * D, dtype=bf16, device=dev)
        self.XN16, self.Y16 = self.XN.view(torch.float16), self.Y.view(torch.float16)
        self.vt0 = {"txt": 0, "img": _pad64(T), "cond": _pad64(T) + _pad64(N)}
        self.VT = torch.zeros(B, H, 128, _pad64(T) + _pad64(N) + _pad64(C), dtype=bf16, device=dev)
        self.Q8 = self.K8 = self.VT8 = None
        self.TL_SPLIT = 4
        self.TLs = torch.zeros(max(self.TL_SPLIT, 3), M, 16, dtype=f32, device=dev)
        self.TL = self.TLs[0]
        self.lat16 = torch.zeros(B * N, cfg.in_channels, dtype=bf16, device=dev)
        self.lat16h = self.lat16.view(torch.float16)
        self.out = torch.zeros(B * N, cfg.in_channels, dtype=f32, device=dev)
        self.temb = torch.zeros(B, D, dtype=f32, device=dev)
        self.temb_base = torch.zeros(B, D, dtype=f32, device=dev)
        self.cond_temb = torch.zeros(B, D, dtype=f32, device=dev)
        self.tproj = torch.zeros(B, 256, dtype=f32, device=dev)
        self.thid = torch.zeros(B, D, dtype=f32, device=dev)
        self.t1000 = torch.zeros(B, dtype=f32, device=dev)
        self.mods = torch.zeros(B, cfg.n_mod, dtype=f32, device=dev)
        self.cmods = torch.zeros(B, cfg.n_mod, dtype=f32, device=dev)
        nb = cfg.num_layers + cfg.num_single_layers
        self.tmod = torch.zeros(B, max(nb * cfg.lora_r, 4), dtype=f32, device=dev)
        self.X_txt_init = torch.zeros(max(B * T, 1), D, dtype=f32, device=dev)
        self.X_cond_init = torch.zeros(max(B * C, 1), D, dtype=f32, device=dev)
        rd = sum(cfg.axes_dims_rope)
        self.rope_main = torch.zeros(2, T + N, rd, dtype=f32, device=dev)
        self.rope_cond = torch.zeros(2, max(C, 1), rd, dtype=f32, device=dev)
        self.rope_cs_main = torch.zeros(T + N, rd, dtype=f32, device=dev)
        self.rope_cs_cond = torch.zeros(max(C, 1), rd, dtype=f32, device=dev)
        self.qkv_fused = False
        self.g_lat = torch.zeros(B, N, cfg.in_channels, dtype=f32, device=dev)
        self.g_t = torch.zeros(B, dtype=f32, device=dev)
        self.graphs = {}
        self.shape = (B, T, N, C)
        self.cond_ready = False
        self.KC = self.VTC = None
        self.cond_cache = self.cond_cached = False
        self.XN2 = self.Y32 = self.YA = self.lat2 = None
        self.XN8 = self.Y8 = None

    def _setup_precise(self) -> None:
        if self.XN2 is not None:
            return
        if not self.w.precise_ready:
            raise ValueError("precise mode needs weights packed with precise=True (pack_state_dict / LxFluxTransformer.from_state_dict): "
                             "the bf16 rounding residuals of the weights were not kept")
        D, dev, bf16 = self.cfg.inner_dim, self.device, torch.bfloat16
        self.XN2 = torch.zeros(self.M, 2 * D, dtype=bf16, device=dev)
        self.Y32 = torch.zeros(self.M, 3 * D, dtype=torch.float32, device=dev)
        self.YA = torch.zeros(self.M, 10 * D, dtype=bf16, device=dev)
        self.lat2 = torch.zeros(self.B * self.N, 2 * self.cfg.in_channels, dtype=bf16, device=dev)
        self.precise_attn_split = os.environ.get("LX_PRECISE_ATTN", "split") != "f32"
        if self.precise_attn_split:
            self.QK2 = torch.zeros(self.M, 4 * D, dtype=bf16, device=dev)
            self.VT2 = torch.zeros((2,) + tuple(self.VT.shape), dtype=bf16, device=dev)

    def _fp8_images(self) -> None:
        if self.Q8 is None:
            u8, D = torch.uint8, self.cfg.inner_dim
            self.Q8 = torch.zeros(self.M, D, dtype=u8, device=self.device)
            self.K8 = torch.zeros(self.M, D, dtype=u8, device=self.device)
            self.VT8 = torch.zeros(self.VT.shape, dtype=u8, device=self.device)

    def _setup_f16(self) -> None:
        if self.f16_ovf is None:
            self.f16_ovf = torch.zeros(1, dtype=torch.int32, device=self.device)
        key = (id(self.w), getattr(self.w, "weights_version", 0), getattr(self.w, "lora_version", 0), len(self.w.lora))
        if self.w16 and self._w16_key == key:
            return
        self.w16 = {}
        self._w16_gen = getattr(self, "_w16_gen", 0) + 1
        stat = torch.zeros(2, dtype=torch.int64, device=self.device)
        total = 0

        def image(W):
            h = W.float().clamp_(-65504.0, 65504.0).to(torch.float16)
            back = h.to(W.dtype)
            stat[0] += (back != W).sum()
            stat[1] += (W.float().abs() > 65504.0).sum()
            return h

        for name, W in self.w.t.items():
            if not name.endswith(".w") or name.startswith("mod.") or name.startswith("tte.") or W.dtype != torch.bfloat16:
                continue
            h = image(W)
            if getattr(W, "lx_tiled", False):
                h.lx_tiled = True
            total += W.numel()
            self.w16[name[:-2]] = h
        for name, lo in self.w.lora.items():
            self.w16[name + ".down"] = image(lo.down)
        lost, clipped = (int(v) for v in stat.tolist())
        self.w16_inexact_share = lost / max(total, 1)
        self.w16_clipped = clipped
        self._w16_key = key

    def f16_overflow_count(self, reset: bool = True) -> int:
        if self.f16_ovf is None:
            return 0
        n = int(self.f16_ovf.item())
        if reset:
            self._ovf_event, self._ovf_seen = None, 0
            if n:
                self.f16_ovf.zero_()
        return n

    def f16_overflow_poll(self, sync: bool = False) -> int:
        if not self.f16 or self.f16_ovf is None:
            return 0
        wclip = int(getattr(self, "w16_clipped", 0))
        if sync:
            return self.f16_overflow_count(reset=True) + wclip
        if getattr(self, "_ovf_host", None) is None:
            self._ovf_host = torch.zeros(1, dtype=torch.int32).pin_memory()
            self._ovf_event, self._ovf_seen = None, 0
        n = 0
        if self._ovf_event is not None and self._ovf_event.query():
            self._ovf_event = None
            total = int(self._ovf_host[0])
            n, self._ovf_seen = max(total - self._ovf_seen, 0), total
        if self._ovf_event is None:
            self._ovf_host.copy_(self.f16_ovf, non_blocking=True)
            self._ovf_event = torch.cuda.Event()
            self._ovf_event.record()
        return n + wclip

    def set_lora_scale(self, s: float) -> None:
        s = float(s)
        if s != self.lora_scale:
            self.lora_scale = s
            self.graphs = {}
            self.cond_ready = False
            self.sched = None

    def gemm_ws(self) -> Optional[torch.Tensor]:
        if not self.pair_plan:
            return None
        if self._gemm_ws is None:
            if torch.cuda.is_current_stream_capturing():
                return None
            self._gemm_ws = ops.gemm_workspace(self.device)
        return self._gemm_ws

    def check_status(self, sync: bool = True) -> None:
        if self._gemm_ws is None:
            return
        if sync:
            try:
                ops.gemm_workspace_status(self._gemm_ws)
            except Exception:
                self.pair_plan, self.graphs, self._err_event = False, {}, None
                raise
            return
        n = self._gemm_ws.numel()
        if getattr(self, "_err_host", None) is None:
            self._err_host = torch.zeros(1, dtype=torch.int32).pin_memory()
            self._err_event = None
        if self._err_event is not None and self._err_event.query():
            self._err_event = None
            if int(self._err_host[0]) != 0:
                self.check_status(sync=True)
        if self._err_event is None:
            word = self._gemm_ws[n - 64 * 4: n - 63 * 4].view(torch.int32)
            self._err_host.copy_(word, non_blocking=True)
            self._err_event = torch.cuda.Event()
            self._err_event.record()

    def rows(self, buf: torch.Tensor, stream: str) -> torch.Tensor:
        if stream == "txt":
            return buf[self.r_txt:self.r_img]
        if stream == "img":
            return buf[self.r_img:self.r_cond]
        return buf[self.r_cond:self.M]

    def _streams(self):
        return [(n, l) for n, l in (("txt", self.T), ("img", self.N), ("cond", 0 if self.cond_skip else self.C)) if l > 0]

    def _all_streams(self):
        return [(n, l) for n, l in (("txt", self.T), ("img", self.N), ("cond", self.C)) if l > 0]

    def _lin_skinny(self, x, name, out, act_in=0, act_out=0, accumulate=False):
        lo = self.w.t.get(name + ".w_lo") if self.precise else None
        if lo is None:
            ops.linear_skinny(x, self.w.t[name + ".w"], self.w.t[name + ".b"], out, act_in=act_in, act_out=act_out,
                              accumulate=accumulate)
            return
        ops.linear_skinny(x, self.w.t[name + ".w"], self.w.t[name + ".b"], out, act_in=act_in, accumulate=accumulate)
        ops.linear_skinny(x, lo, None, out, act_in=act_in, accumulate=True)
        if act_out == 1:
            torch.nn.functional.silu(out, inplace=True)

    def _time_text_embed(self, t1000: torch.Tensor, out: torch.Tensor, base: torch.Tensor) -> None:
        ops.timestep_embed(t1000, self.tproj)
        self._lin_skinny(self.tproj, "tte.timestep_embedder.linear_1", self.thid, act_out=1)
        out.copy_(base)
        self._lin_skinny(self.thid, "tte.timestep_embedder.linear_2", out, accumulate=True)

    def _compute_mods(self, temb: torch.Tensor, out: torch.Tensor, lora: bool, lora_only: bool = False) -> None:
        w = self.w
        if not lora_only:
            ops.linear_skinny(temb, w.t["mod.w"], w.t["mod.b"], out, act_in=1)
            if self.precise and "mod.w_lo" in w.t:
                ops.linear_skinny(temb, w.t["mod.w_lo"], None, out, act_in=1, accumulate=True)
        if lora and "mod.lora_down" in w.t and self.lora_scale != 0.0:
            cfg, r, D = self.cfg, self.cfg.lora_r, self.cfg.inner_dim
            nb = cfg.num_layers + cfg.num_single_layers
            rows = temb.shape[0]
            tm = self.tmod[:, : nb * r] if rows == self.B else torch.zeros(rows, nb * r, dtype=torch.float32, device=self.device)
            ops.linear_skinny(temb, w.t["mod.lora_down"], None, tm, act_in=1)
            if self.precise and "mod.lora_down_lo" in w.t:
                ops.linear_skinny(temb, w.t["mod.lora_down_lo"], None, tm, act_in=1, accumulate=True)
            if self.lora_scale != 1.0:
                tm.mul_(self.lora_scale)
            for idx in range(nb):
                if idx < cfg.num_layers:
                    base, width = cfg.mod_base_double(idx), 6 * D
                else:
                    base, width = cfg.mod_base_single(idx - cfg.num_layers), 3 * D
                ops.linear_f32(tm[:, idx * r:], w.t[f"mod.lora_up.{idx}"], None, out[:, base:], M=rows, N=width, K=r,
                               ldx=tm.stride(0), ldy=out.stride(0), accumulate=True)

    def prepare_schedule(self, t_sched) -> None:
        if not self.cond_ready:
            raise RuntimeError("call set_conditioning() before prepare_schedule()")
        cfg, dev, f32 = self.cfg, self.device, torch.float32
        host = None if isinstance(t_sched, torch.Tensor) and t_sched.is_cuda else tuple(float(v) for v in torch.as_tensor(t_sched, dtype=f32).reshape(-1).tolist())
        t = torch.as_tensor(t_sched, dtype=f32).reshape(-1).to(dev)
        n, B, D = t.numel(), self.B, cfg.inner_dim
        if n * B * cfg.n_mod * 4 > (4 << 30):
            self.sched = None
            return
        t1000 = torch.mul(t, 1000.0).repeat_interleave(B).contiguous()
        tproj = torch.empty(n * B, 256, dtype=f32, device=dev)
        thid = torch.empty(n * B, D, dtype=f32, device=dev)
        temb_all = self.temb_base.repeat(n, 1).contiguous()
        ops.timestep_embed(t1000, tproj)
        self._lin_skinny(tproj, "tte.timestep_embedder.linear_1", thid, act_out=1)
        self._lin_skinny(thid, "tte.timestep_embedder.linear_2", temb_all, accumulate=True)
        xs = torch.nn.functional.silu(temb_all)
        hi = xs.to(torch.bfloat16)
        lo = (xs - hi.float()).to(torch.bfloat16)
        acc2 = torch.empty(2 * n * B, cfg.n_mod, dtype=f32, device=dev)
        ops.gemm([ops.gemm_desc(torch.cat([hi, lo], 0).contiguous(), self.w.t["mod.w"], acc2, epilogue=LX_EPI_STORE_F32)])
        mods_all = acc2[: n * B]
        mods_all += acc2[n * B:]
        if self.precise and "mod.w_lo" in self.w.t:
            acc3 = torch.empty(n * B, cfg.n_mod, dtype=f32, device=dev)
            ops.gemm([ops.gemm_desc(hi.contiguous(), self.w.t["mod.w_lo"], acc3, epilogue=LX_EPI_STORE_F32)])
            mods_all += acc3
        mods_all += self.w.t["mod.b"]
        if self.latent_lora and "mod.lora_down" in self.w.t:
            self._compute_mods(temb_all, mods_all, lora=True, lora_only=True)
        self.sched = (host if host is not None else tuple(float(v) for v in t.tolist()), mods_all.view(n, B, cfg.n_mod))

    def _setup_nomax(self) -> None:
        self.attn_nomax = False
        if self.model_config.get("attn_fp8", False) and not self.precise:
            return
        if (self.precise and not getattr(self, "precise_attn_split", False)) or os.environ.get("LX_ATTN_NOMAX", "1") == "0":
            return
        w = self.w
        tab = getattr(w, "q_log2", None)
        if tab is None:
            layers = []
            for n in w.t:
                if n.endswith(".wq"):
                    p = n[:-3]
                    layers.append((w.t[n], w.t[p + ".wk"], w.t.get(p + ".wq_txt", w.t[n]), w.t.get(p + ".wk_txt", w.t[p + ".wk"])))
            if not layers:
                return
            mx = torch.stack([torch.stack([torch.maximum(a.abs().max(), c.abs().max()), torch.maximum(b.abs().max(), d.abs().max())])
                              for a, b, c, d in layers]).tolist()
            tab = {}
            for (a, b, c, d), (qm, km) in zip(layers, mx):
                tab[a.data_ptr()] = {"wq": a, "wk": b, "wq_txt": c, "wk_txt": d, "bound": 128.0 * ops.Q_LOG2_FACTOR * qm * km,
                                     "scaled": {a.data_ptr(): (a * ops.Q_LOG2_FACTOR).contiguous(), c.data_ptr(): (c * ops.Q_LOG2_FACTOR).contiguous()}}
            w.q_log2 = tab
            w.q_log2_version = getattr(w, "q_log2_version", 0)
        fin = [abs(v) for row in self.attn_bias.values() for v in row.values() if v > -1e37]
        self._nomax_room = 100.0 - max(fin, default=0.0) * 1.4426950408889634
        self.attn_nomax = any(e["bound"] <= self._nomax_room for e in tab.values())

    def _layer_nomax(self, wq: torch.Tensor) -> bool:
        if not self.attn_nomax:
            return False
        e = getattr(self.w, "q_log2", {}).get(wq.data_ptr())
        return e is not None and e["wq"] is wq and e["bound"] <= self._nomax_room

    def _qn(self, w_q: torch.Tensor, wq: torch.Tensor) -> torch.Tensor:
        return self.w.q_log2[wq.data_ptr()]["scaled"][w_q.data_ptr()] if self._layer_nomax(wq) else w_q

    def _attn_bias(self) -> Dict[str, Dict[str, float]]:
        names = ("txt", "img", "cond")
        b = {q: {k: 0.0 for k in names} for q in names}
        mc = self.model_config
        if self.C:
            if not mc.get("union_cond_attn", True):
                for o in ("txt", "img"):
                    b[o]["cond"] = NEG_INF
                    b["cond"][o] = NEG_INF
            elif mc.get("independent_condition", False):
                b["cond"]["txt"] = b["cond"]["img"] = NEG_INF
            if self.c_factor is not None:
                lb = math.log(self.c_factor)
                b = {q: {k: 0.0 for k in names} for q in names}
                for o in ("txt", "img"):
                    b[o]["cond"] = lb
                    b["cond"][o] = lb
        return b

    def user_mask(self, mask: torch.Tensor, B: int, S: int, C: int, model_config, c_factor: Optional[float]) -> Optional[torch.Tensor]:
        mc = model_config or {}
        if c_factor is not None or (C and (not mc.get("union_cond_attn", True) or mc.get("independent_condition", False))):
            return None
        if mask.dim() > 4:
            raise ValueError(f"attention_mask: rank {mask.dim()} (expected 2..4)")
        if mask.device.type != self.device.type or (self.device.index is not None and mask.device.index != self.device.index):
            raise ValueError(f"attention_mask: on {mask.device}, the engine runs on {self.device}")
        if mask.dtype not in (torch.bool, torch.float32, torch.bfloat16, torch.float16):
            raise ValueError(f"attention_mask: dtype {mask.dtype} (expected bool, float32, bfloat16 or float16)")
        m = mask
        while m.dim() < 4:
            m = m.unsqueeze(0)
        H = self.cfg.num_attention_heads
        if m.shape[0] not in (1, B) or m.shape[1] not in (1, H) or m.shape[2] not in (1, S) or m.shape[3] != S:
            raise ValueError(f"attention_mask: shape {tuple(mask.shape)} does not broadcast to [B={B}, H={H}, S={S}, S={S}] "
                             "over the concatenated [text | image | condition] sequence")
        return m

    def _mask_segments(self):
        streams = self._all_streams()
        bias = [[0.0] * 3 for _ in range(3)]
        for qi, (qs, _) in enumerate(streams):
            for ki, (ks, _) in enumerate(streams):
                bias[qi][ki] = self.attn_bias[qs][ks]
        return [L for _, L in streams], [self.vt0[s] for s, _ in streams], bias

    def _prep_cond_mask(self) -> None:
        seg_len, seg_vt0, bias = self._mask_segments()
        kw = dict(B=self.B, H=self.cfg.num_attention_heads, seg_len=seg_len, seg_vt0=seg_vt0, bias=bias)
        need = ops.attn_mask_workspace_bytes(self.cond_mask, **kw)
        if self._mask_ws is None or self._mask_ws.numel() < need:
            self._mask_ws = torch.empty(max(need, 1), dtype=torch.uint8, device=self.device)
        ops.attn_mask_prep(self.cond_mask, self._mask_ws, **kw)

    def set_conditioning(self, prompt_embeds, pooled, guidance, txt_ids, img_ids, condition_latents=None,
                         condition_ids=None, c_t: float = 0.0, model_config: Optional[Dict] = None,
                         c_factor: Optional[float] = None, attention_mask: Optional[torch.Tensor] = None) -> None:
        cfg, w, dev = self.cfg, self.w, self.device
        B, T = prompt_embeds.shape[0], prompt_embeds.shape[1]
        N = img_ids.shape[0]
        C = 0 if condition_latents is None else condition_latents.shape[1]
        self.cond_mask, self.cond_ready = None, False
        mask = None
        if attention_mask is not None:
            mask_argument(attention_mask)
            refuse_masked_modes(model_config, self.precise_default)
            mask = self.user_mask(attention_mask, B, T + N + C, C, model_config, c_factor)
        self.setup(B, T, N, C)
        self.gemm_ws()
        self.model_config = dict(model_config or {})
        self.c_factor = c_factor
        self.latent_lora = bool(self.model_config.get("latent_lora", False))
        self.precise = bool(self.model_config.get("precise", self.precise_default))
        if self.precise:
            self._setup_precise()
        self.gemm_fp8 = bool(self.model_config.get("gemm_fp8", False)) and not self.precise
        if self.gemm_fp8:
            self._setup_fp8()
        self._pick_operands()
        if self.model_config.get("attn_fp8", False) and not self.precise:
            self._fp8_images()
        if self.model_config.get("add_cond_attn", False) and C and C != N:
            raise ValueError("add_cond_attn adds the condition attention output onto the image stream: needs C == N")
        f32, bf16 = torch.float32, torch.bfloat16
        if self.precise:
            self._embed_p(prompt_embeds.reshape(B * T, -1), "context_embedder", self.X_txt_init, lora=False)
            if C:
                self._embed_p(condition_latents.reshape(B * C, -1), "x_embedder", self.X_cond_init, lora=True)
        else:
            pe = prompt_embeds.to(device=dev, dtype=self._op_dtype()).reshape(B * T, -1).contiguous()
            ops.gemm([ops.gemm_desc(pe, self._W("context_embedder"), self.X_txt_init, bias=w.t["context_embedder.b"],
                                    epilogue=LX_EPI_STORE_F32, **self._f16_kw())])
        if C and not self.precise:
            cl = condition_latents.to(device=dev, dtype=self._op_dtype()).reshape(B * C, -1).contiguous()
            lo = w.lora.get("x_embedder") if self.lora_scale != 0.0 else None
            tl = None
            if lo is not None:
                tl = self.TL[: B * C, : cfg.lora_r]
                ops.lora_down(cl, self._down("x_embedder", lo), tl)
                if self.lora_scale != 1.0:
                    tl.mul_(self.lora_scale)
            ops.gemm([ops.gemm_desc(cl, self._W("x_embedder"), self.X_cond_init, bias=w.t["x_embedder.b"], epilogue=LX_EPI_STORE_F32,
                                    lora_t=tl, lora_up=lo.up if lo is not None else None, **self._f16_kw())])
        ids = torch.cat([txt_ids.to(dev, f32).reshape(-1, 3), img_ids.to(dev, f32).reshape(-1, 3)], 0)
        self.cos_main, self.sin_main = ops.rope_table(ids, cfg.axes_dims_rope, out=(self.rope_main[0], self.rope_main[1]))
        if C:
            self.cos_cond, self.sin_cond = ops.rope_table(condition_ids.to(dev, f32).reshape(-1, 3), cfg.axes_dims_rope,
                                                          out=(self.rope_cond[0], self.rope_cond[1]))
        self._rope_pairs(check=False)
        pooled = pooled.to(device=dev, dtype=f32).contiguous()
        self._lin_skinny(pooled, "tte.text_embedder.linear_1", self.thid, act_out=1)
        self._lin_skinny(self.thid, "tte.text_embedder.linear_2", self.temb_base)
        if cfg.guidance_embeds:
            if guidance is None:
                raise ValueError("this transformer has guidance_embeds=True: pass `guidance`")
            g1000 = (guidance.to(device=dev, dtype=f32) * 1000.0).contiguous()
            ops.timestep_embed(g1000, self.tproj)
            self._lin_skinny(self.tproj, "tte.guidance_embedder.linear_1", self.thid, act_out=1)
            self._lin_skinny(self.thid, "tte.guidance_embedder.linear_2", self.temb_base, accumulate=True)
        if C:
            ct = torch.full((B,), float(c_t) * 1000.0, dtype=f32, device=dev)
            self._time_text_embed(ct, self.cond_temb, self.temb_base)
            self._compute_mods(self.cond_temb, self.cmods, lora=True)
        self.attn_bias = self._attn_bias()
        self._setup_nomax()
        if mask is not None:
            self.cond_mask = mask
            self._prep_cond_mask()
        self.cond_ready = True
        self.cond_cached = False
        self.sched = None

    def _pick_operands(self) -> None:
        fmt = str(self.model_config.get("operands", self.operands_default)).lower()
        if fmt not in ("bf16", "fp16", "f16", "float16", "bfloat16"):
            raise ValueError(f'model_config["operands"] = {fmt!r}: "bf16" or "fp16"')
        self.f16 = fmt in ("fp16", "f16", "float16") and not self.precise and not self.gemm_fp8
        if self.f16:
            self._setup_f16()
        elif self.w16:
            self.w16, self.graphs = {}, {}

    def _op_dtype(self):
        return torch.float16 if self.f16 else torch.bfloat16

    def _op(self, t: torch.Tensor) -> torch.Tensor:
        return t.view(torch.float16) if self.f16 else t

    def _W(self, name: str) -> torch.Tensor:
        return self.w16[name] if self.f16 else self.w.t[name + ".w"]

    def _down(self, name: str, lo) -> torch.Tensor:
        return self.w16[name + ".down"] if self.f16 else lo.down

    def _f16_kw(self) -> Dict:
        return dict(f16=True, f16_ovf=self.f16_ovf) if self.f16 else {}

    def _ln(self, base_by_stream: Dict[str, int], shift_off: int, scale_off: int, lora_for: Optional[str] = None,
            include_txt: bool = False):
        row0 = {"txt": self.r_txt, "img": self.r_img, "cond": self.r_cond}
        segs = []
        for s, L in self._streams():
            mods = self.cmods if s == "cond" else self.mods
            b0 = base_by_stream[s]
            segs.append((row0[s], self.B * L, L, mods[:, b0 + shift_off:], mods[:, b0 + scale_off:]))
        lora, ready = None, None
        lo = self.w.lora.get(lora_for) if lora_for is not None else None
        if (lo is not None and self.ln_lora and (self.C > 0 or self.latent_lora) and self.lora_scale == 1.0 and lo.down.shape[0] <= 16
                and self.cfg.inner_dim in (3072, 256) and self._lora_rows(include_txt) is not None):
            r0, n = self._lora_rows(include_txt)
            lora = (self._down(lora_for, lo), self.TL[r0:r0 + n, : lo.down.shape[0]], r0, n)
            ready = (lo, r0)
        if self.f16:
            ops.ln_modulate_segs(self.X, segs, self.XN16, self.mods.stride(0), f16_ovf=self.f16_ovf, lora=lora)
        else:
            ops.ln_modulate_segs(self.X, segs, self.XN, self.mods.stride(0), lora=lora)
        return ready

    def _lora_rows(self, include_txt: bool):
        end = self.r_cond if self.cond_skip else self.M
        if self.latent_lora:
            r0 = self.r_txt if include_txt else self.r_img
            return r0, end - r0
        if self.cond_skip:
            return None
        return self.r_cond, self.M - self.r_cond

    def _lora_t(self, A: torch.Tensor, name: str, include_txt: bool = False):
        lo = self.w.lora.get(name)
        if lo is None or (self.C == 0 and not self.latent_lora) or self.lora_scale == 0.0 or self._lora_rows(include_txt) is None:
            return None, None
        r0, n = self._lora_rows(include_txt)
        t = self.TL[r0:r0 + n, : lo.down.shape[0]]
        ops.lora_down(self._op(A[r0:r0 + n]), self._down(name, lo), t, n_split=self.TL_SPLIT, split_stride=self.TLs.stride(0))
        if self.lora_scale != 1.0:
            self.TLs[:, r0:r0 + n, : lo.down.shape[0]].mul_(self.lora_scale)
        return lo, r0

    def _gemm_streams(self, A: torch.Tensor, Cbuf: torch.Tensor, main: str, txt: Optional[str], *, epilogue: int,
                      gate_off: Optional[Dict[str, int]] = None, lora_mod_cols: int = 0, lora_toff_max: int = 0,
                      gelu_col_start: int = 0, only: Optional[Sequence[str]] = None, ncols: Optional[Dict[str, int]] = None,
                      qkv=None, lora_ready=None) -> None:
        w = self.w
        lora_needed = only is None or "cond" in only or self.latent_lora
        nsplit = self.TL_SPLIT
        if lora_ready is not None:
            (lo, lr0), nsplit = lora_ready, 1
        else:
            lo, lr0 = self._lora_t(A, main, include_txt=txt is None) if lora_needed else (None, None)
        probs = []
        for s, L in self._streams():
            if only is not None and s not in only:
                continue
            name = txt if (s == "txt" and txt is not None) else main
            a, c = self._op(self.rows(A, s)), self.rows(Cbuf, s)
            W, bias = self._W(name), w.t[name + ".b"]
            if self.f16 and (epilogue & 0xff) == LX_EPI_STORE_BF16 and qkv is None:
                c = c.view(torch.float16)
            n_out = ncols.get(s) if ncols else None
            if n_out is not None and n_out < W.shape[0]:
                tiled = getattr(W, "lx_tiled", False)
                W, bias, c = W[:n_out], bias[:n_out], c[:, :n_out]
                if tiled:
                    W.lx_tiled = True
            kw = dict(bias=bias, epilogue=epilogue, rows_per_batch=L, gelu_col_start=gelu_col_start, **self._f16_kw())
            if qkv is not None:
                rope = self.rope_cs_cond if s == "cond" else (self.rope_cs_main[: self.T] if s == "txt" else self.rope_cs_main[self.T:])
                kw["qkv"] = dict(norm_q=self._qn(qkv[2] if s == "txt" else qkv[0], qkv[0]), norm_k=qkv[3] if s == "txt" else qkv[1], rope=rope,
                                 vt=self.VT, vt_pos0=self.vt0[s], d=self.cfg.inner_dim)
                if self.model_config.get("attn_fp8", False):
                    self._fp8_images()
                    kw["qkv"].update(q8=self.rows(self.Q8, s), k8=self.rows(self.K8, s), vt=self.VT8)
                elif self.cond_cache and len(qkv) > 4:
                    kw["qkv"].update(k=self.rows(self.KC[qkv[4]], s), vt=self.VTC[qkv[4]])
            if gate_off is not None:
                mods = self.cmods if s == "cond" else self.mods
                kw["gate"] = mods[:, gate_off[s]:]
            if lo is not None and name == main and (s == "cond" or (s == "img" and self.latent_lora) or
                                                    (s == "txt" and self.latent_lora and txt is None)):
                row0 = {"txt": self.r_txt, "img": self.r_img, "cond": self.r_cond}[s]
                if row0 >= lr0:
                    kw.update(lora_t=self.TL[row0:row0 + a.shape[0]], lora_up=lo.up[: W.shape[0]], lora_mod_cols=lora_mod_cols,
                              lora_toff_max=lora_toff_max, lora_nsplit=nsplit, lora_split_stride=self.TLs.stride(0))
            probs.append(ops.gemm_desc(a, W, c, **kw))
        ops.gemm(probs, self.gemm_ws())

    def _rope_pairs(self, check: bool) -> None:
        D, rd = self.cfg.inner_dim, sum(self.cfg.axes_dims_rope)
        ok = (self.qkv_epilogue and D % 256 == 0 and rd == 128 and self.cos_main is not None
              and all(L % 32 == 0 for _, L in self._all_streams()) and (self.C == 0 or self.cos_cond is not None)
              and self.cos_main.shape[0] == self.T + self.N)
        if ok:
            pairs = [(self.rope_cs_main, self.cos_main, self.sin_main)]
            if self.C:
                pairs.append((self.rope_cs_cond, self.cos_cond, self.sin_cond))
            for dst, cos, sin in pairs:
                if check and not (torch.equal(cos[:, 0::2], cos[:, 1::2]) and torch.equal(sin[:, 0::2], sin[:, 1::2])):
                    ok = False
                    break
                dst[:, 0::2].copy_(cos[:, 0::2])
                dst[:, 1::2].copy_(sin[:, 0::2])
        self.qkv_fused = bool(ok)

    def _qkv_epilogue(self) -> bool:
        if not self.qkv_fused or self.precise or self.gemm_fp8:
            return False
        return True

    def _attention(self, wq, wk, wq_txt, wk_txt, prepped: bool = False, layer: Optional[int] = None, img_only: bool = False) -> None:
        cfg = self.cfg
        D, H, B = cfg.inner_dim, cfg.num_attention_heads, self.B
        Y = self.Y
        seg_row0, seg_len, seg_vt0, qsegs = [], [], [], []
        off = 0
        cached = self.cond_cache and layer is not None and prepped
        streams = self._all_streams() if cached else self._streams()
        bias = [[0.0] * 3 for _ in range(3)]
        for qi, (qs, _) in enumerate(streams):
            for ki, (ks, _) in enumerate(streams):
                bias[qi][ki] = self.attn_bias[qs][ks]
        for s, L in streams:
            row0 = {"txt": self.r_txt, "img": self.r_img, "cond": self.r_cond}[s]
            if s == "cond":
                cos, sin = self.cos_cond, self.sin_cond
            elif self.cos_main is None:
                cos = sin = None
            else:
                cos, sin = self.cos_main[off:off + L], self.sin_main[off:off + L]
                off += L
            qsegs.append((row0, L, self.vt0[s], self._qn(wq_txt if s == "txt" else wq, wq), wk_txt if s == "txt" else wk, cos, sin))
            seg_row0.append(row0); seg_len.append(L); seg_vt0.append(self.vt0[s])
        flags = (ops.ATTN_Q_LOG2 | ops.ATTN_BOUNDED) if self._layer_nomax(wq) else 0
        if not self.pair_plan:
            flags |= ops.ATTN_INVARIANT
        okw = dict(f16_ovf=self.f16_ovf) if self.f16 else {}
        if img_only:
            okw["qseg_mask"] = 1 << [s for s, _ in streams].index("img")
        if self.f16:
            flags |= ops.ATTN_O_F16
        mask, mask_ws = (self.attn_mask, None) if self.attn_mask is not None else (self.cond_mask, self._mask_ws)
        if mask is not None:
            if self.model_config.get("attn_fp8", False):
                raise NotImplementedError("attention_mask is not supported in attn_fp8 mode")
            if cached:
                raise NotImplementedError("attention_mask is not supported on condition-cached forwards")
            if not prepped:
                ops.qkv_prep_segs(Y, 2 * D, 0, D, qsegs, B, H, self.VT, in_f16=self.f16)
            mflags = (ops.ATTN_Q_LOG2 if self._layer_nomax(wq) else 0) | (ops.ATTN_O_F16 if self.f16 else 0)
            ops.attn_fwd_masked(Y, Y, self.VT, Y, mask, q_col=2 * D, k_col=0, o_col=2 * D, B=B, H=H, seg_row0=seg_row0,
                                seg_len=seg_len, seg_vt0=seg_vt0, bias=bias, flags=mflags, workspace=mask_ws, prepped=mask_ws is not None,
                                **okw)
            return
        if self.model_config.get("attn_fp8", False):
            self._fp8_images()
            if not prepped:
                ops.qkv_prep_fp8_segs(Y, 2 * D, 0, D, qsegs, B, H, self.Q8, self.K8, self.VT8, in_f16=self.f16)
            f8 = (ops.ATTN_O_F16 if self.f16 else 0) | (ops.ATTN_P_EXP2 if self.model_config.get("attn_fp8_exp2", False) else 0)
            ops.attn_fwd_fp8(self.Q8, self.K8, self.VT8, Y, o_col=2 * D, B=B, H=H, seg_row0=seg_row0, seg_len=seg_len,
                             seg_vt0=seg_vt0, bias=bias, flags=f8, **okw)
            return
        if cached:
            ops.attn_fwd(Y, self.KC[layer], self.VTC[layer], Y, q_col=2 * D, k_col=0, o_col=2 * D, B=B, H=H, seg_row0=seg_row0,
                         seg_len=seg_len, seg_vt0=seg_vt0, bias=bias, n_qseg=(len(self._streams()) if self.cond_skip else 0) if not img_only else 0,
                         flags=flags, **okw)
            return
        if not prepped:
            ops.qkv_prep_segs(Y, 2 * D, 0, D, qsegs, B, H, self.VT, in_f16=self.f16)
        ops.attn_fwd(Y, Y, self.VT, Y, q_col=2 * D, k_col=0, o_col=2 * D, B=B, H=H, seg_row0=seg_row0, seg_len=seg_len,
                     seg_vt0=seg_vt0, bias=bias, flags=flags, **okw)

    def double_block(self, i: int) -> None:
        if self.precise:
            return self._double_block_p(i)
        if self.gemm_fp8:
            return self._double_block_8(i)
        cfg, w = self.cfg, self.w
        D = cfg.inner_dim
        b = cfg.mod_base_double(i)
        base = {"img": b, "cond": b, "txt": b + 6 * D}
        p = f"d{i}"
        Yq, Ya, Yf = self.Y[:, : 3 * D], self.Y[:, 2 * D: 3 * D], self.Y[:, 3 * D:]
        ready = self._ln(base, 0, D, lora_for=p + ".qkv")
        nw = (w.t[p + ".wq"], w.t[p + ".wk"], w.t[p + ".wq_txt"], w.t[p + ".wk_txt"])
        fused = self._qkv_epilogue()
        self._gemm_streams(self.XN, Yq, p + ".qkv", p + ".qkv_txt", epilogue=LX_EPI_STORE_BF16, lora_mod_cols=D, lora_toff_max=2,
                           qkv=nw + (i,) if fused else None, lora_ready=ready)
        self._attention(*nw, prepped=fused, layer=i)
        gate = {s: base[s] + 2 * D for s in base}
        self._gemm_streams(Ya, self.X, p + ".out", p + ".out_txt", epilogue=LX_EPI_RESID_F32, gate_off=gate)
        if self.C and self.model_config.get("add_cond_attn", False):
            lo = w.lora.get(p + ".out") if self.lora_scale != 0.0 else None
            a = self.rows(Ya, "cond")
            kw = dict(lora_t=self.rows(self.TL, "cond"), lora_up=lo.up, lora_nsplit=self.TL_SPLIT,
                      lora_split_stride=self.TLs.stride(0)) if lo is not None else {}
            ops.gemm([ops.gemm_desc(self._op(a), self._W(p + ".out"), self.rows(self.X, "img"), bias=w.t[p + ".out.b"], epilogue=LX_EPI_RESID_F32,
                                    rows_per_batch=self.C, gate=self.cmods[:, gate["cond"]:], **kw, **self._f16_kw())])
        ready = self._ln(base, 3 * D, 4 * D, lora_for=p + ".ff1")
        self._gemm_streams(self.XN, Yf, p + ".ff1", p + ".ff1_txt", epilogue=LX_EPI_STORE_BF16 | LX_EPI_GELU, lora_ready=ready)
        gate = {s: base[s] + 5 * D for s in base}
        self._gemm_streams(Yf, self.X, p + ".ff2", p + ".ff2_txt", epilogue=LX_EPI_RESID_F32, gate_off=gate)

    def single_block(self, j: int, image_out_only: bool = False) -> None:
        if self.precise:
            return self._single_block_p(j, image_out_only)
        if self.gemm_fp8:
            return self._single_block_8(j, image_out_only)
        cfg, w = self.cfg, self.w
        D = cfg.inner_dim
        b = cfg.mod_base_single(j)
        base = {"img": b, "cond": b, "txt": b}
        p = f"s{j}"
        ready = self._ln(base, 0, D, lora_for=p + ".fused", include_txt=True)
        kv_only = {"txt": 2 * D, "cond": 2 * D} if image_out_only else None
        nw = (w.t[p + ".wq"], w.t[p + ".wk"], w.t[p + ".wq"], w.t[p + ".wk"])
        fused = self._qkv_epilogue()
        self._gemm_streams(self.XN, self.Y, p + ".fused", None, epilogue=LX_EPI_STORE_BF16 | LX_EPI_GELU, gelu_col_start=3 * D,
                           lora_mod_cols=D, lora_toff_max=3, ncols=kv_only, qkv=nw + (cfg.num_layers + j,) if fused else None,
                           lora_ready=ready)
        self._attention(*nw, prepped=fused, layer=cfg.num_layers + j, img_only=image_out_only)
        gate = {s: b + 2 * D for s in base}
        self._gemm_streams(self.Y[:, 2 * D:], self.X, p + ".out", None, epilogue=LX_EPI_RESID_F32, gate_off=gate,
                           only=("img",) if image_out_only else None)

    S_X8, S_Y8 = 16.0, 16.0

    def _setup_fp8(self) -> None:
        if self.XN8 is None:
            D = self.cfg.inner_dim
            self.XN8 = torch.zeros(self.M, D, dtype=torch.uint8, device=self.device)
            self.Y8 = torch.zeros(self.M, 5 * D, dtype=torch.uint8, device=self.device)
        if self.w8:
            return
        names = []
        for i in range(self.cfg.num_layers):
            names += [f"d{i}.{n}" for n in ("qkv", "qkv_txt", "out", "out_txt", "ff1", "ff1_txt", "ff2", "ff2_txt")]
        for j in range(self.cfg.num_single_layers):
            names += [f"s{j}.fused", f"s{j}.out"]
        for n in names:
            W = self.w.t[n + ".w"]
            W = ops.untile_weight(W) if getattr(W, "lx_tiled", False) else W
            W8, rs = ops.quantize_weight_fp8(W)
            self.w8[n] = ops.tile_weight(W8) if (W8.shape[0] % 256 == 0 and W8.shape[1] % 128 == 0) else W8
            self.w8[n + ".rs"] = rs

    def _cs(self, name: str, act_scale: float, rows: Optional[slice] = None) -> torch.Tensor:
        key = f"{name}.cs{act_scale:g}"
        t = self.w8.get(key)
        if t is None:
            t = self.w8[key] = (self.w8[name + ".rs"] / act_scale).contiguous()
        return t if rows is None else t[rows]

    def _gemm_streams_8(self, A8: torch.Tensor, act_scale: float, Cbuf: torch.Tensor, main: str, txt: Optional[str], *, epilogue: int,
                        w_rows: Optional[slice] = None, t_col0: int = 0, gate_off: Optional[Dict[str, int]] = None, lora_mod_cols: int = 0,
                        lora_toff_max: int = 0, gelu: bool = False, only: Optional[Sequence[str]] = None, lora=None, out_scale: float = 0.0):
        w = self.w
        row0 = {"txt": self.r_txt, "img": self.r_img, "cond": self.r_cond}
        lo, lr0 = lora if lora is not None else (None, 0)
        probs = []
        for s_, L in self._streams():
            if only is not None and s_ not in only:
                continue
            name = txt if (s_ == "txt" and txt is not None) else main
            a, c = self.rows(A8, s_), self.rows(Cbuf, s_)
            W8, bias = self.w8[name], w.t[name + ".b"]
            if w_rows is not None:
                tiled = getattr(W8, "lx_tiled", False)
                W8, bias = W8[w_rows], bias[w_rows]
                if tiled:
                    W8.lx_tiled = True
            kw = dict(bias=bias, epilogue=epilogue | (LX_EPI_GELU if gelu else 0), rows_per_batch=L, fp8=True, col_scale=self._cs(name, act_scale, w_rows),
                      out_scale=out_scale)
            if gate_off is not None:
                mods = self.cmods if s_ == "cond" else self.mods
                kw["gate"] = mods[:, gate_off[s_]:]
            if lo is not None and name == main and row0[s_] >= lr0 and (s_ == "cond" or (s_ == "img" and self.latent_lora) or
                                                                         (s_ == "txt" and self.latent_lora and txt is None)):
                up = lo.up[w_rows] if w_rows is not None else lo.up
                kw.update(lora_t=self.TL[row0[s_]:row0[s_] + a.shape[0], t_col0:], lora_up=up, lora_mod_cols=lora_mod_cols,
                          lora_toff_max=lora_toff_max, lora_nsplit=self.TL_SPLIT, lora_split_stride=self.TLs.stride(0))
            probs.append(ops.gemm_desc(a, W8, c, **kw))
        ops.gemm(probs)

    def _lora_t8(self, X8: torch.Tensor, act_scale: float, name: str, include_txt: bool = False):
        lo = self.w.lora.get(name)
        if lo is None or (self.C == 0 and not self.latent_lora) or self.lora_scale == 0.0 or self._lora_rows(include_txt) is None:
            return None
        r0, n = self._lora_rows(include_txt)
        t = self.TL[r0:r0 + n, : lo.down.shape[0]]
        ops.lora_down_fp8(X8[r0:r0 + n], self.lora_scale / act_scale, lo.down, t, n_split=self.TL_SPLIT, split_stride=self.TLs.stride(0))
        return lo, r0

    def _ln8(self, base_by_stream: Dict[str, int], shift_off: int, scale_off: int) -> None:
        row0 = {"txt": self.r_txt, "img": self.r_img, "cond": self.r_cond}
        segs = []
        for s_, L in self._streams():
            mods = self.cmods if s_ == "cond" else self.mods
            b0 = base_by_stream[s_]
            segs.append((row0[s_], self.B * L, L, mods[:, b0 + shift_off:], mods[:, b0 + scale_off:]))
        ops.ln_modulate_fp8_segs(self.X, segs, self.XN, self.XN8, self.mods.stride(0), self.S_X8)

    def _lora_pair(self, A: torch.Tensor, name: str, include_txt: bool = False):
        lo, r0 = self._lora_t(A, name, include_txt=include_txt)
        return None if lo is None else (lo, r0)

    def _double_block_8(self, i: int) -> None:
        cfg, w = self.cfg, self.w
        D = cfg.inner_dim
        b = cfg.mod_base_double(i)
        base = {"img": b, "cond": b, "txt": b + 6 * D}
        p = f"d{i}"
        Y, Y8 = self.Y, self.Y8
        self._ln8(base, 0, D)
        self._gemm_streams_8(self.XN8, self.S_X8, Y[:, : 3 * D], p + ".qkv", p + ".qkv_txt", epilogue=LX_EPI_STORE_BF16, lora_mod_cols=D,
                             lora_toff_max=2, lora=self._lora_pair(self.XN, p + ".qkv"))
        self._attention(w.t[p + ".wq"], w.t[p + ".wk"], w.t[p + ".wq_txt"], w.t[p + ".wk_txt"])
        Ya = Y[:, 2 * D: 3 * D]
        ops.convert_fp8(Ya, Y8[:, :D], self.S_Y8)
        gate = {s_: base[s_] + 2 * D for s_ in base}
        self._gemm_streams_8(Y8[:, :D], self.S_Y8, self.X, p + ".out", p + ".out_txt", epilogue=LX_EPI_RESID_F32, gate_off=gate,
                             lora=self._lora_pair(Ya, p + ".out"))
        if self.C and self.model_config.get("add_cond_attn", False):
            raise NotImplementedError("add_cond_attn is not wired into the fp8 GEMM path (use the bf16 or the precise mode)")
        self._ln8(base, 3 * D, 4 * D)
        self._gemm_streams_8(self.XN8, self.S_X8, Y8[:, D:], p + ".ff1", p + ".ff1_txt", epilogue=ops.LX_EPI_STORE_FP8, gelu=True, out_scale=self.S_Y8)
        gate = {s_: base[s_] + 5 * D for s_ in base}
        self._gemm_streams_8(Y8[:, D:], self.S_Y8, self.X, p + ".ff2", p + ".ff2_txt", epilogue=LX_EPI_RESID_F32, gate_off=gate,
                             lora=self._lora_t8(Y8[:, D:], self.S_Y8, p + ".ff2"))

    def _single_block_8(self, j: int, image_out_only: bool = False) -> None:
        cfg, w = self.cfg, self.w
        D, r = cfg.inner_dim, cfg.lora_r
        b = cfg.mod_base_single(j)
        base = {"img": b, "cond": b, "txt": b}
        p = f"s{j}"
        Y, Y8 = self.Y, self.Y8
        self._ln8(base, 0, D)
        lora = self._lora_pair(self.XN, p + ".fused", include_txt=True)
        only = ("img",) if image_out_only else None
        self._gemm_streams_8(self.XN8, self.S_X8, Y[:, : 3 * D], p + ".fused", None, epilogue=LX_EPI_STORE_BF16, w_rows=slice(0, 3 * D),
                             lora_mod_cols=D, lora_toff_max=2, lora=lora)
        self._gemm_streams_8(self.XN8, self.S_X8, Y8[:, D:], p + ".fused", None, epilogue=ops.LX_EPI_STORE_FP8, gelu=True, out_scale=self.S_Y8,
                             w_rows=slice(3 * D, 7 * D), t_col0=3 * r, only=only, lora=lora)
        self._attention(w.t[p + ".wq"], w.t[p + ".wk"], w.t[p + ".wq"], w.t[p + ".wk"])
        ops.convert_fp8(Y[:, 2 * D: 3 * D], Y8[:, :D], self.S_Y8)
        gate = {s_: b + 2 * D for s_ in base}
        self._gemm_streams_8(Y8, self.S_Y8, self.X, p + ".out", None, epilogue=LX_EPI_RESID_F32, gate_off=gate, only=only,
                             lora=self._lora_t8(Y8, self.S_Y8, p + ".out", include_txt=True))

    def _desc_p(self, A2: torch.Tensor, name: str, Cbuf: torch.Tensor, *, K: int, a_lo_off: int, w_rows: Optional[slice] = None, **kw):
        w2 = self.w.t.get(name + ".w2")
        W = w2 if w2 is not None else self.w.t[name + ".w"]
        if w_rows is not None:
            tiled = getattr(W, "lx_tiled", False)
            W = W[w_rows]
            if tiled:
                W.lx_tiled = True
        return ops.gemm_desc(A2, W, Cbuf, K=K, N=W.shape[0], k_segs=3 if w2 is not None else 2, a_lo_off=a_lo_off, **kw)

    def _lora_t_p(self, A2: torch.Tensor, name: str, K: int, a_lo_off: int, r0: int, n: int):
        lo = self.w.lora.get(name)
        if lo is None or self.lora_scale == 0.0:
            return None, 0
        R = lo.down.shape[0]
        terms = [(A2[r0:r0 + n, :K], lo.down), (A2[r0:r0 + n, a_lo_off:a_lo_off + K], lo.down)]
        if lo.down_lo is not None:
            terms.append((A2[r0:r0 + n, :K], lo.down_lo))
        ops.lora_down_terms(terms, self.TLs[0, r0:r0 + n, :R], self.TLs.stride(0))
        if self.lora_scale != 1.0:
            self.TLs[: len(terms), r0:r0 + n, :R].mul_(self.lora_scale)
        return lo, len(terms)

    def _embed_p(self, x32: torch.Tensor, name: str, out: torch.Tensor, lora: bool, pair: Optional[torch.Tensor] = None) -> None:
        x32 = x32.to(device=self.device, dtype=torch.float32).contiguous()
        rows, K = x32.shape
        if pair is None:
            pair = torch.empty(rows, 2 * K, dtype=torch.bfloat16, device=self.device)
        ops.split_bf16(x32, pair, K)
        kw = {}
        if lora:
            lo, ns = self._lora_t_p(pair, name, K, K, 0, rows) if rows <= self.TLs.shape[1] else (None, 0)
            if lo is not None:
                kw = dict(lora_t=self.TL[:rows], lora_up=lo.up, lora_nsplit=ns, lora_split_stride=self.TLs.stride(0))
        ops.gemm([self._desc_p(pair, name, out, K=K, a_lo_off=K, bias=self.w.t[name + ".b"], epilogue=LX_EPI_STORE_F32, **kw)], self.gemm_ws())

    def _ln_p(self, base_by_stream: Dict[str, int], shift_off: int, scale_off: int) -> None:
        row0 = {"txt": self.r_txt, "img": self.r_img, "cond": self.r_cond}
        segs = []
# ... 310 lines not shown
```

### loongx_amd/ops.py

```python
from __future__ import annotations

import ctypes as C
import math
from typing import Optional, Sequence

import torch

from . import _lib as L
from ._lib import (LX_EPI_QKV, LX_EPI_GELU, LX_EPI_RESID_F32, LX_EPI_SPLIT_BF16, LX_EPI_STORE_BF16, LX_EPI_STORE_F32, LX_EPI_STORE_FP8, LX_OPERANDS_F16, LX_OPERANDS_FP8, LX_W_TILED,
                   AttnDesc, GemmDesc, check, lib)


def _stream() -> int:
    return torch.cuda.current_stream().cuda_stream


def _p(t: Optional[torch.Tensor]) -> Optional[int]:
    return None if t is None else t.data_ptr()


def _req(t: torch.Tensor, dtype, name: str):
    if t.dtype != dtype:
        raise TypeError(f"{name}: expected {dtype}, got {t.dtype}")
    if not t.is_cuda:
        raise ValueError(f"{name}: must live on the GPU (the hot path has no CPU fallback)")


def tile_weight(W: torch.Tensor) -> torch.Tensor:
    N, K = W.shape
    e = 16 // W.element_size()
    assert W.dtype in (torch.bfloat16, torch.float16, torch.uint8) and N % 256 == 0 and K % (8 * e) == 0
    t = W.reshape(N // 256, 256, K // (8 * e), 8, e).permute(0, 2, 1, 3, 4)
    r = torch.arange(256, device=W.device)
    src = torch.arange(8, device=W.device)[None, :] ^ ((r >> 1) & 7)[:, None]
    t = t[:, :, r[:, None], src]
    out = t.contiguous().reshape(N, K)
    out.lx_tiled = True
    return out


def untile_weight(Wt: torch.Tensor) -> torch.Tensor:
    N, K = Wt.shape
    e = 16 // Wt.element_size()
    t = Wt.reshape(N // 256, K // (8 * e), 256, 8, e)
    r = torch.arange(256, device=Wt.device)
    src = torch.arange(8, device=Wt.device)[None, :] ^ ((r >> 1) & 7)[:, None]
    return t[:, :, r[:, None], src].permute(0, 2, 1, 3, 4).contiguous().reshape(N, K)


def quantize_weight_fp8(W: torch.Tensor):
    Wf = W.float()
    amax = Wf.abs().amax(dim=1).clamp_min(1e-12)
    s = 448.0 / amax
    W8 = (Wf * s[:, None]).clamp(-448.0, 448.0).to(torch.float8_e4m3fn).view(torch.uint8).contiguous()
    return W8, (1.0 / s).contiguous()


def gemm_desc(A: torch.Tensor, W: torch.Tensor, C_: torch.Tensor, *, bias=None, epilogue=LX_EPI_STORE_BF16,
              gate=None, rows_per_batch=None, lora_t=None, lora_up=None, lora_mod_cols=0, lora_toff_max=0,
              gelu_col_start=0, M=None, N=None, K=None, lora_nsplit=1, lora_split_stride=0, k_segs=0, a_lo_off=0,
              c_lo_off=0, fp8=False, col_scale=None, out_scale=0.0, qkv=None, f16=False, f16_ovf=None) -> GemmDesc:
    if fp8:
        _req(A, torch.uint8, "A"); _req(W, torch.uint8, "W")
        epilogue |= LX_OPERANDS_FP8
    elif f16:
        _req(A, torch.float16, "A"); _req(W, torch.float16, "W")
        assert col_scale is None and not k_segs and not c_lo_off
        epilogue |= LX_OPERANDS_F16
        if f16_ovf is not None:
            _req(f16_ovf, torch.int32, "f16_ovf")
            col_scale = f16_ovf
    else:
        _req(A, torch.bfloat16, "A"); _req(W, torch.bfloat16, "W")
    d = GemmDesc()
    d.A, d.W, d.C = A.data_ptr(), W.data_ptr(), C_.data_ptr()
    d.bias = _p(bias)
    d.M = A.shape[0] if M is None else M
    d.K = A.shape[1] if K is None else K
    d.N = W.shape[0] if N is None else N
    d.lda, d.ldw, d.ldc = A.stride(0), W.stride(0), C_.stride(0)
    d.rows_per_batch = d.M if rows_per_batch is None else rows_per_batch
    d.gate = _p(gate)
    d.gate_ld = gate.stride(0) if gate is not None else 0
    d.lora_t, d.lora_up = _p(lora_t), _p(lora_up)
    if lora_t is not None:
        d.lora_r, d.lora_ldt = lora_up.shape[1], lora_t.stride(0)
    d.lora_mod_cols, d.lora_toff_max = lora_mod_cols, lora_toff_max
    d.lora_nsplit, d.lora_split_stride = lora_nsplit, lora_split_stride
    d.k_segs, d.a_lo_off, d.c_lo_off = k_segs, a_lo_off, c_lo_off
    if c_lo_off:
        epilogue |= LX_EPI_SPLIT_BF16
    if getattr(W, "lx_tiled", False):
        epilogue |= LX_W_TILED
    d.epilogue, d.gelu_col_start = epilogue, gelu_col_start
    d.col_scale, d.out_scale = _p(col_scale), float(out_scale)
    if qkv is not None:
        _req(qkv["norm_q"], torch.float32, "qkv.norm_q"); _req(qkv["norm_k"], torch.float32, "qkv.norm_k")
        f8 = qkv.get("q8") is not None
        _req(qkv["vt"], torch.uint8 if f8 else torch.bfloat16, "qkv.vt")
        rope = qkv["rope"]
        _req(rope, torch.float32, "qkv.rope")
        assert rope.is_contiguous() and rope.shape == (d.rows_per_batch, 128), (rope.shape, d.rows_per_batch)
        assert qkv["vt"].is_contiguous()
        d.qkv_norm_q, d.qkv_norm_k, d.qkv_rope = _p(qkv["norm_q"]), _p(qkv["norm_k"]), _p(rope)
        d.qkv_d, d.qkv_vt_ld, d.qkv_vt_pos0 = int(qkv["d"]), qkv["vt"].shape[-1], int(qkv["vt_pos0"])
        if f8:
            q8, k8 = qkv["q8"], qkv["k8"]
            _req(q8, torch.uint8, "qkv.q8"); _req(k8, torch.uint8, "qkv.k8")
            assert q8.shape[0] == d.M and k8.shape[0] == d.M and q8.stride(0) == k8.stride(0) and q8.stride(1) == 1 and k8.stride(1) == 1
            d.qkv_q8, d.qkv_k8, d.qkv_vt8, d.qkv_ld8 = q8.data_ptr(), k8.data_ptr(), qkv["vt"].data_ptr(), q8.stride(0)
            d.qkv_q_scale, d.qkv_k_scale, d.qkv_v_scale = FP8_Q_SCALE, FP8_K_SCALE, FP8_V_SCALE
        else:
            d.qkv_vt = _p(qkv["vt"])
        d.epilogue = epilogue = epilogue | LX_EPI_QKV
        kimg = qkv.get("k")
        if kimg is not None:
            _req(kimg, torch.bfloat16, "qkv.k")
            assert kimg.shape[0] == d.M and kimg.stride(1) == 1
            d.qkv_k, d.qkv_k_ld = kimg.data_ptr(), kimg.stride(0)
        d._keep = (qkv["norm_q"], qkv["norm_k"], rope, qkv["vt"], kimg, qkv.get("q8"), qkv.get("k8"))
    kind = epilogue & 0xff
    want = torch.bfloat16 if kind == LX_EPI_STORE_BF16 else (torch.uint8 if kind == LX_EPI_STORE_FP8 else torch.float32)
    if f16 and kind == LX_EPI_STORE_BF16 and qkv is None:
        want = torch.float16
    if not (f16 and qkv is not None and kind == LX_EPI_STORE_BF16 and C_.dtype in (torch.float16, torch.bfloat16)):
        _req(C_, want, "C")
    return d


class LaunchTimer:

    def __init__(self, only_calls=None):
        self.records = {}
        self.bytes = {}
        self.only_calls = None if only_calls is None else set(only_calls)
        self.calls = 0
        self.active = only_calls is None

    def next_call(self) -> bool:
        self.active = self.only_calls is None or self.calls in self.only_calls
        self.calls += 1
        return self.active

    def bracket(self, kind: str, flops: float, nbytes: float = 0.0):
        s, e = torch.cuda.Event(enable_timing=True), torch.cuda.Event(enable_timing=True)
        self.records.setdefault(kind, []).append((s, e, flops))
        self.bytes[kind] = self.bytes.get(kind, 0.0) + nbytes
        return s, e

    def summary(self):
        out = {}
        for kind, recs in self.records.items():
            ms = sum(s.elapsed_time(e) for s, e, _ in recs)
            out[kind] = dict(launches=len(recs), flops=sum(f for _, _, f in recs), ms=ms, bytes=self.bytes.get(kind, 0.0))
        return out


TIMER: Optional[LaunchTimer] = None


def gemm_workspace(device) -> torch.Tensor:
    return torch.zeros(lib.lx_gemm_workspace_bytes(), dtype=torch.uint8, device=device)


def gemm_workspace_status(ws: torch.Tensor) -> None:
    check(lib.lx_gemm_workspace_status(ws.data_ptr(), _stream()), "lx_gemm_workspace_status")


def gemm(problems: Sequence[GemmDesc], workspace: Optional[torch.Tensor] = None) -> None:
    n = len(problems)
    arr = (GemmDesc * n)(*problems)
    if workspace is not None:
        call = lambda: check(lib.lx_gemm_bf16_ws(arr, n, workspace.data_ptr(), workspace.numel(), _stream()), "lx_gemm_bf16_ws")
    else:
        call = lambda: check(lib.lx_gemm_bf16(arr, n, _stream()), "lx_gemm_bf16")
    if TIMER is not None and TIMER.active:
        def _bytes(p):
            epi = p.epilogue & 0xff
            out_b = 2 if epi == LX_EPI_STORE_BF16 else (8 if epi == LX_EPI_RESID_F32 else 4)
            return 2.0 * p.M * p.K + 2.0 * p.N * p.K + float(out_b) * p.M * p.N
        s, e = TIMER.bracket("gemm", sum(2.0 * p.M * p.N * p.K for p in problems), sum(_bytes(p) for p in problems))
        s.record()
        call()
        e.record()
        return
    call()


def gemm_last_plan() -> int:
    return lib.lx_gemm_last_plan()


def lora_down(X: torch.Tensor, Adown: torch.Tensor, T: torch.Tensor, n_split: int = 1, split_stride: int = 0) -> None:
    _req(T, torch.float32, "T")
    if X.dtype == torch.float16:
        _req(Adown, torch.float16, "Adown")
        if not X.is_cuda:
            raise ValueError("X: must live on the GPU (the hot path has no CPU fallback)")
        check(lib.lx_lora_down_f16(X.data_ptr(), X.stride(0), Adown.data_ptr(), T.data_ptr(), T.stride(0), X.shape[0], X.shape[1],
                                   Adown.shape[0], n_split, split_stride, _stream()), "lx_lora_down_f16")
        return
    _req(X, torch.bfloat16, "X"); _req(Adown, torch.bfloat16, "Adown")
    check(lib.lx_lora_down(X.data_ptr(), X.stride(0), Adown.data_ptr(), T.data_ptr(), T.stride(0), X.shape[0], X.shape[1],
                           Adown.shape[0], n_split, split_stride, _stream()), "lx_lora_down")


def lora_down_terms(terms, T: torch.Tensor, slab_stride: int) -> None:
    n = len(terms)
    M, K = terms[0][0].shape
    R = terms[0][1].shape[0]
    xs, ls, as_ = (C.c_void_p * n)(), (C.c_int * n)(), (C.c_void_p * n)()
    for i, (x, a) in enumerate(terms):
        _req(x, torch.bfloat16, "X"); _req(a, torch.bfloat16, "Adown")
        assert x.shape == (M, K) and a.shape == (R, K) and a.is_contiguous() and x.stride(1) == 1
        xs[i], ls[i], as_[i] = x.data_ptr(), x.stride(0), a.data_ptr()
    _req(T, torch.float32, "T")
    check(lib.lx_lora_down_terms(xs, ls, as_, n, T.data_ptr(), T.stride(0), M, K, R, slab_stride, _stream()), "lx_lora_down_terms")


def linear_skinny(X, W, bias, Y, act_in=0, act_out=0, accumulate=False) -> None:
    _req(X, torch.float32, "X"); _req(W, torch.bfloat16, "W"); _req(Y, torch.float32, "Y")
    check(lib.lx_linear_skinny(X.data_ptr(), X.stride(0), W.data_ptr(), W.stride(0), _p(bias), Y.data_ptr(), Y.stride(0),
                               X.shape[0], W.shape[0], W.shape[1], act_in, act_out, int(accumulate), _stream()), "lx_linear_skinny")


def timestep_embed(t: torch.Tensor, out: torch.Tensor) -> None:
    _req(t, torch.float32, "t"); _req(out, torch.float32, "out")
    check(lib.lx_timestep_embed(t.data_ptr(), out.data_ptr(), out.shape[0], out.shape[1], _stream()), "lx_timestep_embed")


def rope_table(ids: torch.Tensor, axes=(16, 56, 56), theta: float = 10000.0, out=None):
    _req(ids, torch.float32, "ids")
    ids = ids.contiguous()
    Lq, tot = ids.shape[0], sum(axes)
    if out is None:
        cos = torch.empty(Lq, tot, dtype=torch.float32, device=ids.device)
        sin = torch.empty_like(cos)
    else:
        cos, sin = out
        assert cos.shape == (Lq, tot) and sin.shape == (Lq, tot) and cos.is_contiguous() and sin.is_contiguous()
    check(lib.lx_rope_table(ids.data_ptr(), Lq, axes[0], axes[1], axes[2], float(theta), cos.data_ptr(), sin.data_ptr(), _stream()), "lx_rope_table")
    return cos, sin


def ln_modulate(X, shift, scale, Y, rows_per_batch, eps=1e-6, mod_ld=None, f16_ovf=None) -> None:
    _req(X, torch.float32, "X"); _req(shift, torch.float32, "shift"); _req(scale, torch.float32, "scale")
    if Y.dtype == torch.float16:
        return ln_modulate_segs(X, [(0, X.shape[0], rows_per_batch, shift, scale)], Y, shift.stride(0) if mod_ld is None else mod_ld, eps, f16_ovf=f16_ovf)
    _req(Y, torch.bfloat16, "Y")
    check(lib.lx_ln_modulate(X.data_ptr(), X.stride(0), shift.data_ptr(), scale.data_ptr(),
                             shift.stride(0) if mod_ld is None else mod_ld, Y.data_ptr(), Y.stride(0), X.shape[0], X.shape[1],
                             rows_per_batch, eps, _stream()), "lx_ln_modulate")


def qkv_prep(QKV, q_col, k_col, v_col, row0, n_rows, rows_per_batch, H, wq, wk, cos, sin, VT, vt_pos0, eps=1e-6) -> None:
    _req(QKV, torch.bfloat16, "QKV")
    check(lib.lx_qkv_prep(QKV.data_ptr(), QKV.stride(0), q_col, k_col, v_col, row0, n_rows, rows_per_batch, H, _p(wq), _p(wk), eps,
                          _p(cos), _p(sin), _p(VT), VT.shape[-1] if VT is not None else 0, vt_pos0, _stream()), "lx_qkv_prep")


def ln_modulate_segs(X, segs, Y, mod_ld, eps=1e-6, lora=None, f16_ovf=None) -> None:
    n = len(segs)
    arr = (L.LnSeg * n)()
    for i, (row0, n_rows, rpb, sh, sc) in enumerate(segs):
        arr[i].row0, arr[i].n_rows, arr[i].rows_per_batch = row0, n_rows, rpb
        arr[i].shift, arr[i].scale = sh.data_ptr(), sc.data_ptr()
    if Y.dtype == torch.float16 and lora is not None:
        A, T, r0, cnt = lora
        _req(A, torch.float16, "Adown"); _req(T, torch.float32, "T")
        assert A.is_contiguous() and A.shape[1] == X.shape[1] and T.shape[0] >= cnt and T.stride(1) == 1
        check(lib.lx_ln_modulate_lora_f16_segs(X.data_ptr(), X.stride(0), arr, n, mod_ld, Y.data_ptr(), Y.stride(0), X.shape[1], eps,
                                               A.data_ptr(), A.shape[0], T.data_ptr(), T.stride(0), r0, cnt, _p(f16_ovf), _stream()),
              "lx_ln_modulate_lora_f16_segs")
        return
    if Y.dtype == torch.float16:
        check(lib.lx_ln_modulate_f16_segs(X.data_ptr(), X.stride(0), arr, n, mod_ld, Y.data_ptr(), Y.stride(0), X.shape[1], eps, _p(f16_ovf),
                                          _stream()), "lx_ln_modulate_f16_segs")
        return
    if lora is not None:
        A, T, r0, cnt = lora
        _req(A, torch.bfloat16, "Adown"); _req(T, torch.float32, "T")
        assert A.is_contiguous() and A.shape[1] == X.shape[1] and T.shape[0] >= cnt and T.stride(1) == 1
        check(lib.lx_ln_modulate_lora_segs(X.data_ptr(), X.stride(0), arr, n, mod_ld, Y.data_ptr(), Y.stride(0), X.shape[1], eps,
                                           A.data_ptr(), A.shape[0], T.data_ptr(), T.stride(0), r0, cnt, _stream()), "lx_ln_modulate_lora_segs")
        return
    check(lib.lx_ln_modulate_segs(X.data_ptr(), X.stride(0), arr, n, mod_ld, Y.data_ptr(), Y.stride(0), X.shape[1], eps, _stream()),
          "lx_ln_modulate_segs")


def qkv_prep_segs(QKV, q_col, k_col, v_col, segs, n_batches, H, VT, eps=1e-6, in_f16=False) -> None:
    n = len(segs)
    arr = (L.QkvSeg * n)()
    for i, (row0, rpb, vt0, wq, wk, cos, sin) in enumerate(segs):
        arr[i].row0, arr[i].rows_per_batch, arr[i].vt_pos0 = row0, rpb, vt0
        arr[i].wq, arr[i].wk, arr[i].cos_tab, arr[i].sin_tab = _p(wq), _p(wk), _p(cos), _p(sin)
    fn, nm = (lib.lx_qkv_prep_f16in_segs, "lx_qkv_prep_f16in_segs") if in_f16 else (lib.lx_qkv_prep_segs, "lx_qkv_prep_segs")
    check(fn(QKV.data_ptr(), QKV.stride(0), q_col, k_col, v_col, arr, n, n_batches, H, eps, _p(VT), VT.shape[-1] if VT is not None else 0, _stream()), nm)


def _attn_desc(Q, K, VT, O, q_col, k_col, o_col, B, H, seg_row0, seg_len, seg_vt0, bias, scale):
    d = AttnDesc()
    d.Q, d.K, d.VT, d.O = Q.data_ptr(), K.data_ptr(), VT.data_ptr(), O.data_ptr()
    d.ldq, d.ldk, d.ldo, d.vt_ld = Q.stride(0), K.stride(0), O.stride(0), VT.shape[-1]
    d.q_col, d.k_col, d.o_col, d.B, d.H, d.n_seg = q_col, k_col, o_col, B, H, len(seg_len)
    for i in range(len(seg_len)):
        d.seg_row0[i], d.seg_len[i], d.seg_vt0[i] = seg_row0[i], seg_len[i], seg_vt0[i]
    for i in range(3):
        for j in range(3):
            d.bias[i][j] = 0.0 if bias is None else float(bias[i][j])
    d.scale = (1.0 / math.sqrt(128.0)) if scale is None else scale
    return d


ATTN_Q_LOG2, ATTN_BOUNDED, ATTN_INVARIANT, ATTN_O_F16, ATTN_PREFER_4WAVE, ATTN_P_EXP2 = (L.LX_ATTN_Q_LOG2, L.LX_ATTN_BOUNDED, L.LX_ATTN_INVARIANT, L.LX_ATTN_O_F16,
                                                                                         L.LX_ATTN_PREFER_4WAVE, L.LX_ATTN_P_EXP2)
Q_LOG2_FACTOR = (1.0 / math.sqrt(128.0)) * 1.4426950408889634


def _q_rows(seg_len, n_qseg, qseg_mask):
    if qseg_mask:
        return sum(L_ for i, L_ in enumerate(seg_len) if (qseg_mask >> i) & 1)
    return sum(seg_len[:n_qseg]) if n_qseg else sum(seg_len)


def attn_fwd(Q, K, VT, O, *, q_col, k_col, o_col, B, H, seg_row0, seg_len, seg_vt0, bias=None, scale=None, n_qseg=0, flags=0, f16_ovf=None,
             qseg_mask=0) -> None:
    d = _attn_desc(Q, K, VT, O, q_col, k_col, o_col, B, H, seg_row0, seg_len, seg_vt0, bias, scale)
    d.n_qseg = n_qseg
    d.flags = flags
    d.qseg_mask = qseg_mask
    d.f16_ovf = _p(f16_ovf)
    if TIMER is not None:
        S = sum(seg_len)
        Sq = _q_rows(seg_len, n_qseg, qseg_mask)
        s, e = TIMER.bracket("attn", 4.0 * B * H * Sq * S * 128)
        s.record()
        check(lib.lx_attn_fwd(C.byref(d), _stream()), "lx_attn_fwd")
        e.record()
        return
    check(lib.lx_attn_fwd(C.byref(d), _stream()), "lx_attn_fwd")


_MASK_DTYPES = {torch.bool: L.LX_ATTN_MASK_BOOL, torch.float32: L.LX_ATTN_MASK_F32, torch.bfloat16: L.LX_ATTN_MASK_BF16,
                torch.float16: L.LX_ATTN_MASK_F16}


def _mask_desc(mask: torch.Tensor, workspace: Optional[torch.Tensor]) -> "L.AttnMaskDesc":
    if mask.dtype not in _MASK_DTYPES:
        raise TypeError(f"attention mask: dtype {mask.dtype} is not one of bool, float32, bfloat16, float16")
    if not mask.is_cuda:
        raise ValueError("attention mask: must live on the GPU (the hot path has no CPU fallback)")
    if not 2 <= mask.dim() <= 4:
        raise ValueError(f"attention mask: rank {mask.dim()} (expected 2..4)")
    while mask.dim() < 4:
        mask = mask.unsqueeze(0)
    m = L.AttnMaskDesc()
    m.mask, m.dtype = mask.data_ptr(), _MASK_DTYPES[mask.dtype]
    for i in range(4):
        m.dims[i], m.strides[i] = mask.shape[i], mask.stride(i)
    if workspace is not None:
        m.workspace, m.workspace_bytes = workspace.data_ptr(), workspace.numel() * workspace.element_size()
    return m


def _seg_desc(B, H, seg_len, seg_vt0, bias) -> AttnDesc:
    d = AttnDesc()
    d.B, d.H, d.n_seg = B, H, len(seg_len)
    for i in range(len(seg_len)):
        d.seg_len[i], d.seg_vt0[i] = seg_len[i], seg_vt0[i]
    for i in range(3):
        for j in range(3):
            d.bias[i][j] = 0.0 if bias is None else float(bias[i][j])
    return d


def attn_mask_workspace_bytes(mask, *, B, H, seg_len, seg_vt0, bias=None) -> int:
    d, m = _seg_desc(B, H, seg_len, seg_vt0, bias), _mask_desc(mask, None)
    n = C.c_size_t(0)
    check(lib.lx_attn_mask_workspace(C.byref(d), C.byref(m), C.byref(n)), "lx_attn_mask_workspace")
    return int(n.value)


def attn_mask_workspace(mask, *, B, H, seg_len, seg_vt0, bias=None, device=None) -> torch.Tensor:
    n = attn_mask_workspace_bytes(mask, B=B, H=H, seg_len=seg_len, seg_vt0=seg_vt0, bias=bias)
    return torch.empty(max(n, 1), dtype=torch.uint8, device=device if device is not None else mask.device)


def attn_mask_prep(mask, workspace, *, B, H, seg_len, seg_vt0, bias=None) -> None:
    d, m = _seg_desc(B, H, seg_len, seg_vt0, bias), _mask_desc(mask, workspace)
    check(lib.lx_attn_mask_prep(C.byref(d), C.byref(m), _stream()), "lx_attn_mask_prep")


def attn_fwd_masked(Q, K, VT, O, mask, *, q_col, k_col, o_col, B, H, seg_row0, seg_len, seg_vt0, bias=None, scale=None, flags=0,
                    f16_ovf=None, workspace=None, prepped=False, n_qseg=0, qseg_mask=0) -> torch.Tensor:
    if workspace is None:
        workspace = attn_mask_workspace(mask, B=B, H=H, seg_len=seg_len, seg_vt0=seg_vt0, bias=bias, device=Q.device)
    d = _attn_desc(Q, K, VT, O, q_col, k_col, o_col, B, H, seg_row0, seg_len, seg_vt0, bias, scale)
    d.flags, d.f16_ovf, d.n_qseg, d.qseg_mask = flags, _p(f16_ovf), n_qseg, qseg_mask
    m = _mask_desc(mask, workspace)
    if not prepped:
        check(lib.lx_attn_mask_prep(C.byref(d), C.byref(m), _stream()), "lx_attn_mask_prep")
    if TIMER is not None and TIMER.active:
        S = sum(seg_len)
        s, e = TIMER.bracket("attn", 4.0 * B * H * _q_rows(seg_len, n_qseg, qseg_mask) * S * 128)
        s.record()
        check(lib.lx_attn_fwd_masked(C.byref(d), C.byref(m), _stream()), "lx_attn_fwd_masked")
        e.record()
        return workspace
    check(lib.lx_attn_fwd_masked(C.byref(d), C.byref(m), _stream()), "lx_attn_fwd_masked")
    return workspace


FP8_K_SCALE, FP8_V_SCALE = 16.0, 1.0
FP8_Q_SCALE = 2048.0 * (1.0 / math.sqrt(128.0)) * 1.4426950408889634 / FP8_K_SCALE


def qkv_prep_fp8_segs(QKV, q_col, k_col, v_col, segs, n_batches, H, Q8, K8, VT8, eps=1e-6, in_f16=False) -> None:
    n = len(segs)
    arr = (L.QkvSeg * n)()
    for i, (row0, rpb, vt0, wq, wk, cos, sin) in enumerate(segs):
        arr[i].row0, arr[i].rows_per_batch, arr[i].vt_pos0 = row0, rpb, vt0
        arr[i].wq, arr[i].wk, arr[i].cos_tab, arr[i].sin_tab = _p(wq), _p(wk), _p(cos), _p(sin)
    fn, nm = (lib.lx_qkv_prep_fp8_f16in_segs, "lx_qkv_prep_fp8_f16in_segs") if in_f16 else (lib.lx_qkv_prep_fp8_segs, "lx_qkv_prep_fp8_segs")
    check(fn(QKV.data_ptr(), QKV.stride(0), q_col, k_col, v_col, arr, n, n_batches, H, eps, Q8.data_ptr(), K8.data_ptr(), Q8.stride(0),
             VT8.data_ptr(), VT8.shape[-1], FP8_Q_SCALE, FP8_K_SCALE, FP8_V_SCALE, _stream()), nm)


def attn_fwd_fp8(Q8, K8, VT8, O, *, o_col, B, H, seg_row0, seg_len, seg_vt0, bias=None, scale=None, flags=0, f16_ovf=None, qseg_mask=0) -> None:
    d = _attn_desc(Q8, K8, VT8, O, 0, 0, o_col, B, H, seg_row0, seg_len, seg_vt0, bias, scale)
    d.flags, d.f16_ovf, d.qseg_mask = flags, _p(f16_ovf), qseg_mask
    args = (C.byref(d), 1.0 / (FP8_Q_SCALE * FP8_K_SCALE), 1.0 / FP8_V_SCALE, _stream())
    if TIMER is not None:
        S = sum(seg_len)
        s, e = TIMER.bracket("attn", 4.0 * B * H * _q_rows(seg_len, 0, qseg_mask) * S * 128)
        s.record()
        check(lib.lx_attn_fwd_fp8(*args), "lx_attn_fwd_fp8")
        e.record()
        return
    check(lib.lx_attn_fwd_fp8(*args), "lx_attn_fwd_fp8")


def ln_modulate_fp8_segs(X, segs, Y, Y8, mod_ld, y8_scale, eps=1e-6) -> None:
    n = len(segs)
    arr = (L.LnSeg * n)()
    for i, (row0, n_rows, rpb, sh, sc) in enumerate(segs):
        arr[i].row0, arr[i].n_rows, arr[i].rows_per_batch = row0, n_rows, rpb
        arr[i].shift, arr[i].scale = sh.data_ptr(), sc.data_ptr()
    check(lib.lx_ln_modulate_fp8_segs(X.data_ptr(), X.stride(0), arr, n, mod_ld, _p(Y), Y.stride(0) if Y is not None else 0, Y8.data_ptr(),
                                      Y8.stride(0), float(y8_scale), X.shape[1], eps, _stream()), "lx_ln_modulate_fp8_segs")


def convert_fp8(src: torch.Tensor, dst: torch.Tensor, scale: float) -> None:
    _req(dst, torch.uint8, "dst")
    check(lib.lx_convert_fp8(src.data_ptr(), int(src.dtype == torch.bfloat16), src.stride(0), dst.data_ptr(), dst.stride(0), float(scale),
                             src.shape[0], src.shape[1], _stream()), "lx_convert_fp8")


def lora_down_fp8(X8: torch.Tensor, x_descale: float, Adown: torch.Tensor, T: torch.Tensor, n_split: int = 1, split_stride: int = 0) -> None:
    _req(X8, torch.uint8, "X8"); _req(Adown, torch.bfloat16, "Adown"); _req(T, torch.float32, "T")
    check(lib.lx_lora_down_fp8(X8.data_ptr(), X8.stride(0), float(x_descale), Adown.data_ptr(), T.data_ptr(), T.stride(0), X8.shape[0], X8.shape[1],
                               Adown.shape[0], n_split, split_stride, _stream()), "lx_lora_down_fp8")


def split_bf16(src: torch.Tensor, dst: torch.Tensor, lo_off: int) -> None:
    _req(src, torch.float32, "src"); _req(dst, torch.bfloat16, "dst")
    check(lib.lx_split_bf16(src.data_ptr(), src.stride(0), dst.data_ptr(), dst.stride(0), lo_off, src.shape[0], src.shape[1], _stream()),
          "lx_split_bf16")


def ln_modulate_split_segs(X, segs, Y, mod_ld, y_lo_off, eps=1e-6) -> None:
    n = len(segs)
    arr = (L.LnSeg * n)()
    for i, (row0, n_rows, rpb, sh, sc) in enumerate(segs):
        arr[i].row0, arr[i].n_rows, arr[i].rows_per_batch = row0, n_rows, rpb
        arr[i].shift, arr[i].scale = sh.data_ptr(), sc.data_ptr()
    check(lib.lx_ln_modulate_split_segs(X.data_ptr(), X.stride(0), arr, n, mod_ld, Y.data_ptr(), Y.stride(0), y_lo_off, X.shape[1], eps,
                                        _stream()), "lx_ln_modulate_split_segs")


def qkv_prep_f32_segs(QKV, q_col, k_col, segs, n_batches, H, eps=1e-6) -> None:
    _req(QKV, torch.float32, "QKV")
    n = len(segs)
    arr = (L.QkvSeg * n)()
    for i, (row0, rpb, vt0, wq, wk, cos, sin) in enumerate(segs):
        arr[i].row0, arr[i].rows_per_batch, arr[i].vt_pos0 = row0, rpb, 0
        arr[i].wq, arr[i].wk, arr[i].cos_tab, arr[i].sin_tab = _p(wq), _p(wk), _p(cos), _p(sin)
    check(lib.lx_qkv_prep_f32_segs(QKV.data_ptr(), QKV.stride(0), q_col, k_col, arr, n, n_batches, H, eps, _stream()), "lx_qkv_prep_f32_segs")


def attn_fwd_f32(QKV, O, *, q_col, k_col, v_col, o_col, o_lo_off, B, H, seg_row0, seg_len, bias=None, scale=None) -> None:
    _req(QKV, torch.float32, "QKV"); _req(O, torch.bfloat16, "O")
# ... 127 lines not shown
```

Baseline: 1.068.

## Compute LoRA down-projection inside the gemm4 grid with helper workgroups

Adds helper workgroups to the gemm4 launch that compute the LoRA down-projection (X·Adown) into the T buffer. The tile workgroups wait on per-tile-row arrival counters kept in the workspace, then add T·Up in the epilogue using LDS. This removes the separate lora_down kernel launch and its serialization before the main GEMM. In exchange it adds spin-wait synchronization across workgroups, a host-side dry-run plan preview, and a fallback to the old path when the plan cannot inline.

Result: no change. 1.065 (-0.3%).

```diff
diff --git a/include/lx.h b/include/lx.h
--- a/include/lx.h
+++ b/include/lx.h
@@ -65,9 +65,11 @@
   int32_t qkv_k_ld;
   void* qkv_q8;
   void* qkv_k8;
-  void* qkv_vt8;
-  int32_t qkv_ld8;
-  float qkv_q_scale, qkv_k_scale, qkv_v_scale;
+  union { void* qkv_vt8; const void* lora_down; };
+  union { int32_t qkv_ld8; int32_t lora_down_ld; };
+  union { float qkv_q_scale; int32_t lora_row0; };
+  union { float qkv_k_scale; int32_t lora_rows; };
+  float qkv_v_scale;
 } lx_gemm_desc;
 
 #define LX_GEMM_MAX_GROUP 4
@@ -78,8 +80,10 @@
 int lx_gemm_bf16_ws(const lx_gemm_desc* problems, int n, void* workspace, size_t ws_bytes, void* stream);
 int lx_gemm_workspace_status(void* workspace, void* stream);
 enum { LX_GEMM_PLAN_NONE = 0, LX_GEMM_PLAN_8WAVE_256 = 1, LX_GEMM_PLAN_8WAVE_128 = 2, LX_GEMM_PLAN_MIXED = 3, LX_GEMM_PLAN_MIXED_2L = 4,
-       LX_GEMM_PLAN_G4 = 5, LX_GEMM_PLAN_G4_SPLIT2 = 6, LX_GEMM_PLAN_G4_SPLIT3 = 7 };
+       LX_GEMM_PLAN_G4 = 5, LX_GEMM_PLAN_G4_SPLIT2 = 6, LX_GEMM_PLAN_G4_SPLIT3 = 7,
+       LX_GEMM_PLAN_LORA_INLINE = 0x100  };
 int lx_gemm_last_plan(void);
+int lx_gemm_plan_preview(const lx_gemm_desc* problems, int n, void* workspace, size_t ws_bytes);
 
 int lx_lora_down(const void* X, int ldx, const void* Adown, float* T, int ldt, int M, int K, int R, int n_split,
                  int split_stride, void* stream);
diff --git a/loongx_amd/_lib.py b/loongx_amd/_lib.py
--- a/loongx_amd/_lib.py
+++ b/loongx_amd/_lib.py
@@ -13,9 +13,27 @@
 LX_GEMM_MAX_GROUP = 4
 (LX_GEMM_PLAN_NONE, LX_GEMM_PLAN_8WAVE_256, LX_GEMM_PLAN_8WAVE_128, LX_GEMM_PLAN_MIXED, LX_GEMM_PLAN_MIXED_2L, LX_GEMM_PLAN_G4,
  LX_GEMM_PLAN_G4_SPLIT2, LX_GEMM_PLAN_G4_SPLIT3) = range(8)
+LX_GEMM_PLAN_LORA_INLINE = 0x100
+
+
+class _VtOrDown(C.Union):
+    _fields_ = [("qkv_vt8", C.c_void_p), ("lora_down", C.c_void_p)]
+
+
+class _Ld8OrDownLd(C.Union):
+    _fields_ = [("qkv_ld8", C.c_int32), ("lora_down_ld", C.c_int32)]
+
+
+class _QScaleOrRow0(C.Union):
+    _fields_ = [("qkv_q_scale", C.c_float), ("lora_row0", C.c_int32)]
+
+
+class _KScaleOrRows(C.Union):
+    _fields_ = [("qkv_k_scale", C.c_float), ("lora_rows", C.c_int32)]
 
 
 class GemmDesc(C.Structure):
+    _anonymous_ = ("_u0", "_u1", "_u2", "_u3")
     _fields_ = [("A", C.c_void_p), ("W", C.c_void_p), ("bias", C.c_void_p), ("C", C.c_void_p),
                 ("gate", C.c_void_p), ("lora_t", C.c_void_p), ("lora_up", C.c_void_p),
                 ("M", C.c_int32), ("N", C.c_int32), ("K", C.c_int32),
@@ -29,8 +47,8 @@
                 ("qkv_norm_q", C.c_void_p), ("qkv_norm_k", C.c_void_p), ("qkv_rope", C.c_void_p), ("qkv_vt", C.c_void_p),
                 ("qkv_k", C.c_void_p),
                 ("qkv_d", C.c_int32), ("qkv_vt_ld", C.c_int32), ("qkv_vt_pos0", C.c_int32), ("qkv_k_ld", C.c_int32),
-                ("qkv_q8", C.c_void_p), ("qkv_k8", C.c_void_p), ("qkv_vt8", C.c_void_p),
-                ("qkv_ld8", C.c_int32), ("qkv_q_scale", C.c_float), ("qkv_k_scale", C.c_float), ("qkv_v_scale", C.c_float)]
+                ("qkv_q8", C.c_void_p), ("qkv_k8", C.c_void_p), ("_u0", _VtOrDown),
+                ("_u1", _Ld8OrDownLd), ("_u2", _QScaleOrRow0), ("_u3", _KScaleOrRows), ("qkv_v_scale", C.c_float)]
 
 
 class AttnDesc(C.Structure):
@@ -81,6 +99,7 @@
     "lx_gemm_bf16_ws": (C.c_int, [C.POINTER(GemmDesc), _I, _P, _Z, _P]),
     "lx_gemm_workspace_status": (C.c_int, [_P, _P]),
     "lx_gemm_last_plan": (C.c_int, []),
+    "lx_gemm_plan_preview": (C.c_int, [C.POINTER(GemmDesc), _I, _P, _Z]),
     "lx_lora_down": (C.c_int, [_P, _I, _P, _P, _I, _I, _I, _I, _I, _I, _P]),
     "lx_lora_down_f16": (C.c_int, [_P, _I, _P, _P, _I, _I, _I, _I, _I, _I, _P]),
     "lx_lora_down_terms": (C.c_int, [C.POINTER(C.c_void_p), C.POINTER(C.c_int), C.POINTER(C.c_void_p), _I, _P, _I, _I, _I, _I, _I, _P]),
diff --git a/loongx_amd/csrc/gemm.hip b/loongx_amd/csrc/gemm.hip
--- a/loongx_amd/csrc/gemm.hip
+++ b/loongx_amd/csrc/gemm.hip
@@ -3,12 +3,12 @@
 
 static double round_us(int bm, int K) { return bm == 256 ? 15.0 + 1.81 * (K / 64) : 10.5 + 1.06 * (K / 64); }
 
-struct GemmEnv { int bm, g4, sk, g4_fault; };
+struct GemmEnv { int bm, g4, sk, g4_fault, lora_inline; };
 static int env_int(const char* name, int dflt) {
   const char* s = getenv(name);
   return s ? atoi(s) : dflt;
 }
-static GemmEnv read_gemm_env() { return GemmEnv{env_int("LX_GEMM_BM", 0), env_int("LX_GEMM4", 1), env_int("LX_GEMM4_SK", 1), env_int("LX_GEMM4_FAULT", 0)}; }
+static GemmEnv read_gemm_env() { return GemmEnv{env_int("LX_GEMM_BM", 0), env_int("LX_GEMM4", 1), env_int("LX_GEMM4_SK", 1), env_int("LX_GEMM4_FAULT", 0), env_int("LX_GEMM_LORA_INLINE", 1)}; }
 static GemmEnv g_gemm_env = read_gemm_env();
 static const GemmEnv& gemm_env() { return g_gemm_env; }
 extern "C" void lx_gemm_reload_env(void) { g_gemm_env = read_gemm_env(); }
@@ -48,8 +48,11 @@
   return q;
 }
 
+static thread_local bool t_dry = false;
+static thread_local int t_plan = LX_GEMM_PLAN_NONE;
+
 static int launch_plan(const GemmArgs& a, int bm, hipStream_t s, int variant = LX_GV_BF16) {
-  if (a.n == 0) return LX_OK;
+  if (a.n == 0 || t_dry) return LX_OK;
   if (variant == LX_GV_SPLIT) lx_gemm8_launch_split(bm, a, s);
   else if (variant == LX_GV_F16) lx_gemm8_launch_f16(bm, a, s);
   else if (variant == LX_GV_FP8) lx_gemm8_launch_fp8(bm, a, s);
@@ -67,8 +70,9 @@
   hipLaunchKernelGGL(lx_gemm_mixed_kernel<false>, dim3(n_big_pad + tail.tile_start[tail.n]), dim3(NTHREADS), 0, s, big, tail, n_big_pad);
 }
 
-static void plan_add(GemmArgs& a, const lx_gemm_desc& p, int m_base, int bm) {
+static void plan_add(GemmArgs& a, const lx_gemm_desc& p, int m_base, int bm, bool lora_inline = false) {
   a.p[a.n] = p;
+  if (!lora_inline && !(p.epilogue & LX_EPI_QKV)) a.p[a.n].lora_down = nullptr;
   a.m_base[a.n] = m_base;
   a.tile_start[a.n + 1] = a.tile_start[a.n] + (int)tiles_of(p, bm);
   ++a.n;
@@ -78,9 +82,10 @@
 static thread_local int lx_gemm_last = LX_GEMM_PLAN_NONE;
 extern "C" int lx_gemm_last_plan(void) { return lx_gemm_last; }
 static int planned(int rc, int plan) {
-  if (rc == LX_OK) lx_gemm_last = plan;
+  if (rc == LX_OK) t_plan = plan;
   return rc;
 }
+static int gemm_plan_and_launch(const lx_gemm_desc* problems, int n, void* workspace, size_t ws_bytes, void* stream);
 
 extern "C" size_t lx_gemm_workspace_bytes(void) { return SK_WS_BYTES; }
 
@@ -104,6 +109,20 @@
 extern "C" int lx_gemm_bf16(const lx_gemm_desc* problems, int n, void* stream) { return lx_gemm_bf16_ws(problems, n, nullptr, 0, stream); }
 
 extern "C" int lx_gemm_bf16_ws(const lx_gemm_desc* problems, int n, void* workspace, size_t ws_bytes, void* stream) {
+  t_dry = false;
+  const int rc = gemm_plan_and_launch(problems, n, workspace, ws_bytes, stream);
+  if (rc == LX_OK) lx_gemm_last = t_plan;
+  return rc;
+}
+
+extern "C" int lx_gemm_plan_preview(const lx_gemm_desc* problems, int n, void* workspace, size_t ws_bytes) {
+  t_dry = true;
+  const int rc = gemm_plan_and_launch(problems, n, workspace, ws_bytes, nullptr);
+  t_dry = false;
+  return rc == LX_OK ? t_plan : rc;
+}
+
+static int gemm_plan_and_launch(const lx_gemm_desc* problems, int n, void* workspace, size_t ws_bytes, void* stream) {
   LX_CHECK_ARG(problems && n >= 1 && n <= LX_GEMM_MAX_GROUP, "lx_gemm_bf16: n=%d out of range [1,%d]", n, LX_GEMM_MAX_GROUP);
   long t256 = 0, t128 = 0;
   int kmax = 0;
@@ -147,6 +166,10 @@
       LX_CHECK_ARG(p.lora_up && p.lora_r >= 1 && p.lora_r <= 16, "lx_gemm_bf16[%d]: LoRA needs lora_up and 1 <= r <= 16", i);
       LX_CHECK_ARG(p.lora_mod_cols <= 0 || p.lora_mod_cols % BN == 0, "lx_gemm_bf16[%d]: lora_mod_cols must be a multiple of %d", i, BN);
     }
+    if (p.lora_down && !(p.epilogue & LX_EPI_QKV))
+      LX_CHECK_ARG(p.lora_t && ((uintptr_t)p.lora_down & 15) == 0 && p.lora_down_ld >= p.K && p.lora_down_ld % 8 == 0 && p.lora_row0 >= 0 && p.lora_rows > 0 &&
+                   (long)p.lora_row0 + p.lora_rows <= p.M, "lx_gemm_bf16[%d]: lora_down needs lora_t, 16-byte alignment, lora_down_ld %% 8 == 0, >= K and adapter rows inside the problem (row0=%d rows=%d)",
+                   i, p.lora_row0, p.lora_rows);
     if (p.epilogue & LX_EPI_QKV) {
       LX_CHECK_ARG(!fp8 && segs == 1 && !(p.epilogue & LX_EPI_SPLIT_BF16) && epi == LX_EPI_STORE_BF16, "lx_gemm_bf16[%d]: LX_EPI_QKV goes with plain bf16 operands and LX_EPI_STORE_BF16", i);
       LX_CHECK_ARG(p.qkv_d > 0 && p.qkv_d % BN == 0 && (p.N >= 3 * p.qkv_d || p.N % BN == 0), "lx_gemm_bf16[%d]: LX_EPI_QKV needs qkv_d %% 256 == 0 and whole projection tiles (qkv_d=%d N=%d)", i, p.qkv_d, p.N);
@@ -218,11 +241,24 @@
       if (!fills) split_all = split_tail = false;
     }
     if (ok && (fills || split_all || split_tail)) {
+      const long grid_tiles = (split_all || split_tail) ? full + np * tail : t256;
+      bool inl = env.lora_inline && !split && !split_tail && workspace && ws_bytes >= SK_WS_BYTES && ((uintptr_t)workspace & 255) == 0 &&
+                 grid_tiles + LI_HELPERS <= NCU;
+      bool inl_any = false;
+      long trows = 0;
+      for (int i = 0; i < n; ++i) {
+        const lx_gemm_desc& p = problems[i];
+        trows += (p.M + 255) / 256;
+        if (!p.lora_down || (p.epilogue & LX_EPI_QKV)) continue;
+        inl_any = true;
+        inl = inl && (p.lora_mod_cols <= 0 || p.lora_toff_max == 0);
+      }
+      inl = inl && inl_any && trows <= LI_MAX_TROWS;
       GemmArgs all;
       all.n = 0;
       all.tile_start[0] = 0;
       for (int i = 1; i <= MAX_SUB; ++i) all.tile_start[i] = 0;
-      for (int i = 0; i < n; ++i) plan_add(all, problems[i], 0, 256);
+      for (int i = 0; i < n; ++i) plan_add(all, problems[i], 0, 256, inl);
       float* slots = nullptr;
       int *flags = nullptr, *err = nullptr;
       unsigned grid = (unsigned)t256;
@@ -235,11 +271,18 @@
         sk_full = (int)full;
         sk_parts = env.g4_fault ? 3 : 2;
       }
+      if (inl) {
+        flags = (int*)((char*)workspace + SK_FLAGS_OFF);
+        err = flags + 256;
+        grid += LI_HELPERS;
+      }
+      const int plan = (!(split_all || split_tail) ? LX_GEMM_PLAN_G4 : np == 3 ? LX_GEMM_PLAN_G4_SPLIT3 : LX_GEMM_PLAN_G4_SPLIT2) | (inl ? LX_GEMM_PLAN_LORA_INLINE : 0);
+      if (t_dry) return planned(LX_OK, plan);
       if (split) lx_gemm4_launch_split(all, grid, sk_full, sk_parts, slots, flags, err, s);
       else if (f16) lx_gemm4_launch_f16(all, grid, sk_full, sk_parts, slots, flags, err, s, np);
       else lx_gemm4_launch_bf16(all, grid, sk_full, sk_parts, slots, flags, err, s, np);
       LX_LAUNCH_CHECK("lx_gemm_bf16");
-      return planned(LX_OK, !(split_all || split_tail) ? LX_GEMM_PLAN_G4 : np == 3 ? LX_GEMM_PLAN_G4_SPLIT3 : LX_GEMM_PLAN_G4_SPLIT2);
+      return planned(LX_OK, plan);
     }
   }
   if (split) {
@@ -289,6 +332,7 @@
   if (choice == 2) {
     if (big.n > 0 && tail.n > 0) {
       const int n_big = big.tile_start[big.n], n_big_pad = (n_big + 7) & ~7;
+      if (t_dry) return planned(LX_OK, LX_GEMM_PLAN_MIXED);
       if (f16) lx_gemm8_mixed_launch_f16(big, tail, n_big_pad, s);
       else lx_gemm8_mixed_launch_bf16(big, tail, n_big_pad, s);
       LX_LAUNCH_CHECK("lx_gemm_bf16");
diff --git a/loongx_amd/csrc/gemm4.h b/loongx_amd/csrc/gemm4.h
--- a/loongx_amd/csrc/gemm4.h
+++ b/loongx_amd/csrc/gemm4.h
@@ -7,6 +7,9 @@
 constexpr int G4_LDS = 2 * G4_STAGE;
 constexpr int G4_PLD = 132;
 static_assert(G4_LDS <= 160 * 1024 && 4 * 2 * 16 * G4_PLD * 4 <= G4_LDS, "LDS budget / epilogue patches");
+constexpr int G4_LI_UP = 72 * 1024;
+constexpr int G4_LI_T = 80 * 1024;
+static_assert(4 * 2 * 16 * G4_PLD * 4 <= G4_LI_UP && G4_LI_T + 4 * 512 <= G4_LDS, "in-grid LoRA areas lie behind the patches");
 
 #ifdef LX_G4_PROBE
 __device__ unsigned long long lx_g4_probe_buf[8192 * 8];
@@ -14,6 +17,68 @@
 #else
 #define G4_STAMP(k)
 #endif
+
+template <bool F16>
+__device__ __forceinline__ void g4_lora_helper(const GemmArgs& args, const int h, const int helpers, int* __restrict__ li_flags) {
+#if defined(__HIP_DEVICE_COMPILE__)
+  const int tid = threadIdx.x, lane = tid & 63, l15 = lane & 15, kq = lane >> 4;
+  const int wave = __builtin_amdgcn_readfirstlane(tid >> 6);
+  int nb_all, tr_all;
+  li_base(args, args.n, nb_all, tr_all);
+  const int per = li_per_helper(nb_all, helpers);
+  const int b0 = h * per, b1 = min(nb_all, b0 + per);
+  for (int b = b0 + wave; b < b1; b += 4) {
+    int g = 0, base = 0;
+    while (b >= base + li_nblocks(args.p[g])) { base += li_nblocks(args.p[g]); ++g; }
+    const lx_gemm_desc& P = args.p[g];
+    const int R = P.lora_r, K = P.K;
+    const int rf = P.lora_row0 + (b - base) * 16, rl = P.lora_row0 + P.lora_rows - 1;
+    const uint16_t* xp = (const uint16_t*)P.A + (size_t)min(rf + l15, rl) * P.lda + kq * 8;
+    const uint16_t* ap = (const uint16_t*)P.lora_down + (size_t)min(l15, R - 1) * P.lora_down_ld + kq * 8;
+    f32x4 acc = {0.f, 0.f, 0.f, 0.f};
+    const bf16x8 zero = {};
+    for (int k = 0; k < K; k += 16 * 32) {
+      bf16x8 af[16], xf[16];
+#pragma unroll
+      for (int u = 0; u < 16; ++u) {
+        const bool in = k + u * 32 < K;
+        af[u] = in ? *(const bf16x8*)(ap + k + u * 32) : zero;
+        xf[u] = in ? *(const bf16x8*)(xp + k + u * 32) : zero;
+      }
+#pragma unroll
+      for (int u = 0; u < 16; ++u) {
+        if constexpr (F16) acc = __builtin_amdgcn_mfma_f32_16x16x32_f16(__builtin_bit_cast(f16x8, af[u]), __builtin_bit_cast(f16x8, xf[u]), acc, 0, 0, 0);
+        else acc = __builtin_amdgcn_mfma_f32_16x16x32_bf16(af[u], xf[u], acc, 0, 0, 0);
+      }
+    }
+    const int m = rf + l15, r0 = 4 * kq;
+    if (m <= rl) {
+      const lx_rsrc_t rs_t = lx_make_rsrc(P.lora_t);
+#pragma unroll
+      for (int j = 0; j < 4; ++j)
+        if (r0 + j < R) __builtin_amdgcn_raw_buffer_store_b32(__float_as_uint(acc[j]), rs_t, (int)(((size_t)m * P.lora_ldt + r0 + j) * 4), 0, PAIR_AUX_SC1);
+    }
+  }
+  asm volatile("s_waitcnt vmcnt(0)" ::: "memory");
+  __syncthreads();
+  __builtin_amdgcn_fence(__ATOMIC_RELEASE, "workgroup");
+  if (tid == 0) {
+    int last = -1;
+    for (int b = b0; b < b1; ++b) {
+      int g = 0, base = 0;
+      while (b >= base + li_nblocks(args.p[g])) { base += li_nblocks(args.p[g]); ++g; }
+      int blk_g, tr_g;
+      li_base(args, g, blk_g, tr_g);
+      const int rf = args.p[g].lora_row0 + (b - base) * 16, re = min(rf + 15, args.p[g].lora_row0 + args.p[g].lora_rows - 1);
+      for (int tm = rf >> 8; tm <= re >> 8; ++tm)
+        if (tr_g + tm != last) {
+          last = tr_g + tm;
+          __hip_atomic_fetch_add(li_flags + last, 1, __ATOMIC_RELAXED, __HIP_MEMORY_SCOPE_AGENT);
+        }
+    }
+  }
+#endif
+}
 
 
 template <bool SPLIT, bool F16 = false, int NP = 2>
@@ -25,6 +90,13 @@
   const int pid = blockIdx.x;
   G4_STAMP(0)
   const int total = args.tile_start[MAX_SUB];
+  if constexpr (!SPLIT) {
+    const int n_tile_wg = sk_parts >= 2 ? sk_full + NP * (total - sk_full) : total;
+    if (pid >= n_tile_wg) {
+      g4_lora_helper<F16>(args, pid - n_tile_wg, (int)gridDim.x - n_tile_wg, sk_flags + LI_FLAGS_OFF);
+      return;
+    }
+  }
   int lid, part = 0;
   if (pid < sk_full) {
     const int q = sk_full >> 3, r = sk_full & 7;
@@ -114,7 +186,7 @@
     else asm volatile("v_mfma_f32_16x16x32_bf16 %0, %1, %2, %0" : "+a"(acc[i][j]) : "v"(wf[ks][j]), "v"(af[ks][i]));
   };
 #define G4_SB() __builtin_amdgcn_sched_barrier(0)
-  const bool has_lora = P.lora_t != nullptr && kt_begin == 0;
+  const bool has_lora = P.lora_t != nullptr && kt_begin == 0 && !li_on(P);
   u32x2 lu[8], lt[8][4];
   if (has_lora) {
     const int R = P.lora_r, nsplit = P.lora_nsplit;
@@ -218,6 +290,50 @@
   __syncthreads();
   G4_STAMP(4)
 
+  const bool li_tile = !SPLIT && li_on(P) && m0 < P.lora_row0 + P.lora_rows && m0 + BM > P.lora_row0;
+  const int li_r0 = P.lora_row0, li_r1 = P.lora_row0 + P.lora_rows;
+  float* const li_up = (float*)(smem + G4_LI_UP);
+  float* const li_t = (float*)(smem + G4_LI_T) + wave * 128;
+  if (li_tile) {
+    const int R = P.lora_r;
+    const float* up = P.lora_up + (size_t)min(n0 + tid, N - 1) * R;
+#pragma unroll
+    for (int r = 0; r < 8; r += 2) {
+      f32x2 v = {0.f, 0.f};
+      if (r < R) v = *(const f32x2*)(up + r);
+      li_up[r * 256 + tid] = v[0];
+      li_up[(r + 1) * 256 + tid] = v[1];
+    }
+    if (tid == 0) {
+      int blk_g, tr_g, nb_all, tr_all;
+      li_base(args, g, blk_g, tr_g);
+      li_base(args, args.n, nb_all, tr_all);
+      const int n_tile_wg = sk_parts >= 2 ? sk_full + NP * (total - sk_full) : total;
+      const int per = li_per_helper(nb_all, (int)gridDim.x - n_tile_wg);
+      const int j_lo = (max(m0, li_r0) - li_r0) >> 4, j_hi = (min(m0 + BM, li_r1) - 1 - li_r0) >> 4;
+      const int helpers_here = (blk_g + j_hi) / per - (blk_g + j_lo) / per + 1;
+      const int readers = ((N + BN - 1) / BN) * (split_tile ? NP : 1);
+      int* arrive = sk_flags + LI_FLAGS_OFF + tr_g + tm;
+      int* done = arrive + LI_MAX_TROWS;
+      bool ok = __hip_atomic_load(sk_err, __ATOMIC_RELAXED, __HIP_MEMORY_SCOPE_AGENT) == 0;
+      if (ok) {
+        int spins = 0;
+        while (__hip_atomic_load(arrive, __ATOMIC_RELAXED, __HIP_MEMORY_SCOPE_AGENT) < helpers_here) {
+          __builtin_amdgcn_s_sleep(1);
+          if (++spins > (1 << 20)) { ok = false; break; }
+        }
+        if (ok) {
+          if (__hip_atomic_fetch_add(done, 1, __ATOMIC_RELAXED, __HIP_MEMORY_SCOPE_AGENT) == readers - 1) {
+            __hip_atomic_store(arrive, 0, __ATOMIC_RELAXED, __HIP_MEMORY_SCOPE_AGENT);
+            __hip_atomic_store(done, 0, __ATOMIC_RELAXED, __HIP_MEMORY_SCOPE_AGENT);
+          }
+        } else __hip_atomic_store(sk_err, 1, __ATOMIC_RELAXED, __HIP_MEMORY_SCOPE_AGENT);
+      }
+    }
+    __syncthreads();
+    __builtin_amdgcn_fence(__ATOMIC_ACQUIRE, "workgroup");
+  }
+
   const float* partner = nullptr;
   const float* partner2 = nullptr;
   float* my_slot = nullptr;
@@ -337,6 +453,12 @@
         }
       }
     }
+    u32x2 li_tl = {0u, 0u};
+    if (li_tile) {
+      const int m = mb + (lane >> 2), pr = (lane & 3) * 2;
+      if (m >= li_r0 && m < li_r1 && pr < P.lora_r)
+        li_tl = __builtin_amdgcn_raw_buffer_load_b64(lx_make_rsrc(P.lora_t), (int)(((size_t)m * P.lora_ldt + pr) * 4), 0, PAIR_AUX_SC1);
+    }
     __builtin_amdgcn_wave_barrier();
     if constexpr (nx >= 0) { if (mw0 + nx * 16 < M) put(std::integral_constant<int, nx>{}); }
     __builtin_amdgcn_sched_barrier(0);
@@ -361,6 +483,34 @@
         }
         *(f32x4*)q_ = v0; *(f32x4*)(q_ + 4) = v1;
       }
+      __builtin_amdgcn_wave_barrier();
+    }
+    if (li_tile) {
+      *(u32x2*)(li_t + (lane >> 2) * 8 + (lane & 3) * 2) = li_tl;
+      __builtin_amdgcn_wave_barrier();
+      float* pw = patch + (i & 1) * (16 * G4_PLD);
+      const float* upc = li_up + wn * 128 + c4;
+      auto apply = [&](auto nr_) {
+        constexpr int NR = decltype(nr_)::value;
+        f32x4 u[NR];
+#pragma unroll
+        for (int r = 0; r < NR; ++r) u[r] = *(const f32x4*)(upc + r * 256);
+#pragma unroll
+        for (int t = 0; t < 8; ++t) {
+          const int row = t * 2 + (lane >> 5);
+          f32x4 tv[NR / 4];
+#pragma unroll
+          for (int q = 0; q < NR / 4; ++q) tv[q] = *(const f32x4*)(li_t + row * 8 + q * 4);
+          f32x4 v = *(const f32x4*)(pw + row * G4_PLD + c4);
+#pragma unroll
+          for (int r = 0; r < NR; ++r)
+#pragma unroll
+            for (int c_ = 0; c_ < 4; ++c_) v[c_] = __builtin_fmaf(tv[r >> 2][r & 3], u[r][c_], v[c_]);
+          *(f32x4*)(pw + row * G4_PLD + c4) = v;
+        }
+      };
+      if (P.lora_r <= 4) apply(std::integral_constant<int, 4>{});
+      else apply(std::integral_constant<int, 8>{});
       __builtin_amdgcn_wave_barrier();
     }
     if (qkv_tile) {
diff --git a/loongx_amd/csrc/gemm_common.h b/loongx_amd/csrc/gemm_common.h
--- a/loongx_amd/csrc/gemm_common.h
+++ b/loongx_amd/csrc/gemm_common.h
@@ -61,6 +61,22 @@
 constexpr int G4_THREADS = 256;
 constexpr int SK_SLOT_FLOATS = 256 * 256;
 
+constexpr int LI_HELPERS = 16;
+constexpr int LI_MAX_TROWS = 24;
+constexpr int LI_FLAGS_OFF = 256 + 8;
+static_assert(LI_FLAGS_OFF + 2 * LI_MAX_TROWS <= 256 + 64, "the counters live in the workspace's padding");
+
+__device__ __forceinline__ bool li_on(const lx_gemm_desc& p) { return p.lora_down != nullptr && !(p.epilogue & LX_EPI_QKV); }
+__device__ __forceinline__ int li_nblocks(const lx_gemm_desc& p) { return li_on(p) ? (p.lora_rows + 15) >> 4 : 0; }
+__device__ __forceinline__ void li_base(const GemmArgs& args, const int g, int& blocks, int& trows) {
+  blocks = 0; trows = 0;
+  for (int i = 0; i < g; ++i) {
+    blocks += li_nblocks(args.p[i]);
+    trows += (args.p[i].M + 255) >> 8;
+  }
+}
+__device__ __forceinline__ int li_per_helper(const int nblocks, const int helpers) { return ((nblocks + helpers - 1) / helpers + 3) & ~3; }
+
 }
 
 enum { LX_GV_BF16 = 0, LX_GV_F16 = 1, LX_GV_SPLIT = 2, LX_GV_FP8 = 3 };
diff --git a/loongx_amd/flux/engine.py b/loongx_amd/flux/engine.py
--- a/loongx_amd/flux/engine.py
+++ b/loongx_amd/flux/engine.py
@@ -8,6 +8,7 @@
 
 from .. import ops
 from ..ops import LX_EPI_GELU, LX_EPI_RESID_F32, LX_EPI_STORE_BF16, LX_EPI_STORE_F32
+from .._lib import LX_GEMM_PLAN_LORA_INLINE
 from .weights import FluxConfig, PackedWeights
 
 NEG_INF = float("-inf")
@@ -558,11 +559,13 @@
             return None
         return self.r_cond, self.M - self.r_cond
 
-    def _lora_t(self, A: torch.Tensor, name: str, include_txt: bool = False):
+    def _lora_t(self, A: torch.Tensor, name: str, include_txt: bool = False, launch: bool = True):
         lo = self.w.lora.get(name)
         if lo is None or (self.C == 0 and not self.latent_lora) or self.lora_scale == 0.0 or self._lora_rows(include_txt) is None:
             return None, None
         r0, n = self._lora_rows(include_txt)
+        if not launch:
+            return lo, r0
         t = self.TL[r0:r0 + n, : lo.down.shape[0]]
         ops.lora_down(self._op(A[r0:r0 + n]), self._down(name, lo), t, n_split=self.TL_SPLIT, split_stride=self.TLs.stride(0))
         if self.lora_scale != 1.0:
@@ -579,7 +582,12 @@
         if lora_ready is not None:
             (lo, lr0), nsplit = lora_ready, 1
         else:
-            lo, lr0 = self._lora_t(A, main, include_txt=txt is None) if lora_needed else (None, None)
+            inline = (lora_needed and qkv is None and lora_toff_max == 0 and self.lora_scale == 1.0 and not self.precise
+                      and self.gemm_ws() is not None)
+            lo, lr0 = self._lora_t(A, main, include_txt=txt is None, launch=not inline) if lora_needed else (None, None)
+            inline = inline and lo is not None
+        if lora_ready is not None:
+            inline = False
         probs = []
         for s, L in self._streams():
             if only is not None and s not in only:
@@ -614,7 +622,13 @@
                 if row0 >= lr0:
                     kw.update(lora_t=self.TL[row0:row0 + a.shape[0]], lora_up=lo.up[: W.shape[0]], lora_mod_cols=lora_mod_cols,
                               lora_toff_max=lora_toff_max, lora_nsplit=nsplit, lora_split_stride=self.TLs.stride(0))
+                    if inline:
+                        kw.update(lora_down=self._down(main, lo))
             probs.append(ops.gemm_desc(a, W, c, **kw))
+        if inline and not ops.gemm_plan_preview(probs, self.gemm_ws()) & LX_GEMM_PLAN_LORA_INLINE:
+            for d in probs:
+                ops.clear_lora_down(d)
+            self._lora_t(A, main, include_txt=txt is None)
         ops.gemm(probs, self.gemm_ws())
 
     def _rope_pairs(self, check: bool) -> None:
diff --git a/loongx_amd/ops.py b/loongx_amd/ops.py
--- a/loongx_amd/ops.py
+++ b/loongx_amd/ops.py
@@ -59,7 +59,8 @@
 def gemm_desc(A: torch.Tensor, W: torch.Tensor, C_: torch.Tensor, *, bias=None, epilogue=LX_EPI_STORE_BF16,
               gate=None, rows_per_batch=None, lora_t=None, lora_up=None, lora_mod_cols=0, lora_toff_max=0,
               gelu_col_start=0, M=None, N=None, K=None, lora_nsplit=1, lora_split_stride=0, k_segs=0, a_lo_off=0,
-              c_lo_off=0, fp8=False, col_scale=None, out_scale=0.0, qkv=None, f16=False, f16_ovf=None) -> GemmDesc:
+              c_lo_off=0, fp8=False, col_scale=None, out_scale=0.0, qkv=None, f16=False, f16_ovf=None, lora_down=None, lora_row0=0,
+              lora_rows=None) -> GemmDesc:
     if fp8:
         _req(A, torch.uint8, "A"); _req(W, torch.uint8, "W")
         epilogue |= LX_OPERANDS_FP8
@@ -87,6 +88,10 @@
         d.lora_r, d.lora_ldt = lora_up.shape[1], lora_t.stride(0)
     d.lora_mod_cols, d.lora_toff_max = lora_mod_cols, lora_toff_max
     d.lora_nsplit, d.lora_split_stride = lora_nsplit, lora_split_stride
+    if lora_down is not None:
+        assert lora_t is not None and qkv is None and lora_down.dtype == A.dtype and lora_down.stride(1) == 1
+        d.lora_down, d.lora_down_ld = lora_down.data_ptr(), lora_down.stride(0)
+        d.lora_row0, d.lora_rows = lora_row0, (d.M - lora_row0 if lora_rows is None else lora_rows)
     d.k_segs, d.a_lo_off, d.c_lo_off = k_segs, a_lo_off, c_lo_off
     if c_lo_off:
         epilogue |= LX_EPI_SPLIT_BF16
@@ -187,6 +192,20 @@
     call()
 
 
+def gemm_plan_preview(problems: Sequence[GemmDesc], workspace: Optional[torch.Tensor] = None) -> int:
+    n = len(problems)
+    arr = (GemmDesc * n)(*problems)
+    plan = lib.lx_gemm_plan_preview(arr, n, workspace.data_ptr() if workspace is not None else None, workspace.numel() if workspace is not None else 0)
+    if plan < 0:
+        check(plan, "lx_gemm_plan_preview")
+    return plan
+
+
+def clear_lora_down(d: GemmDesc) -> None:
+    if not d.epilogue & LX_EPI_QKV:
+        d.lora_down, d.lora_down_ld, d.lora_row0, d.lora_rows = None, 0, 0, 0
+
+
 def gemm_last_plan() -> int:
     return lib.lx_gemm_last_plan()
 
```
